# keio-bioinformatics/stem_kernel

Measured on AMD Instinct MI355X. Metric: sequence-pairs/sec (Gram entries/s) at L=200 nt, higher is better.
Workload: dtype f64

## Files before the change

include/stem_kernel.h:

```cpp
#ifndef STEM_KERNEL_H
#define STEM_KERNEL_H

#include <stddef.h>
#include <stdint.h>

#ifdef __cplusplus
extern "C" {
#endif

#define SK_ABI_VERSION 2

typedef enum {
  SK_OK = 0,
  SK_ERR_INVALID = -1,
  SK_ERR_HIP = -2,
  SK_ERR_NO_DEVICE = -3,
  SK_ERR_ALLOC = -4,
  SK_ERR_RANGE = -5,
  SK_ERR_UNSUPPORTED = -6
} sk_status;

typedef enum {
  SK_SU_STEM = 0,
  SK_SI_STEM = 1,
  SK_SU_STR = 2,
  SK_SI_STR = 3,
  SK_SU_STEM_STR = 4,
  SK_SI_STEM_STR = 5,
  SK_LSU_STEM = 6,
  SK_LSU_STEM_STR = 7,
  SK_NAIVE_STR = 8,
  SK_BPLA = 9,
  SK_LA = 10,
  SK_BPLA_SW = 11,
  SK_LA_SW = 12,
  SK_STEM4D = 13
} sk_kernel_kind;

typedef struct {
  int32_t kind;
  uint32_t len_band;
  double beta;
  double loop_gap;
  double stack;
  double covar;
  double alpha;
  double gap;
  double match;
  double mismatch;
  double ext;
  double score_table[16];
  double subst;
  double bp_bound;
  int32_t bp_model;
  uint32_t loop;
  double ali_bound;
  int32_t ali_zerop_fixed;
} sk_kernel_params;

void sk_kernel_params_default(sk_kernel_params *p, int32_t kind);

typedef struct sk_context sk_context;

int sk_open(int device, void *hip_stream, sk_context **ctx);
int sk_close(sk_context *ctx);
const char *sk_strerror(int status);
const char *sk_last_error(const sk_context *ctx);

typedef struct sk_dataset sk_dataset;

int sk_dataset_create(sk_dataset **ds);
int sk_dataset_free(sk_dataset *ds);

int sk_dataset_add(sk_dataset *ds, const char *label, int n_rows,
                   const char *const *rows, const double *const *bpp_rows,
                   float th, int use_bp);
int sk_dataset_add_synthetic(sk_dataset *ds, int32_t n, const char *const *seqs,
                             const char *const *labels, float th, int32_t n_threads);
int sk_dataset_add_synthetic_rows(sk_dataset *ds, int32_t n, int32_t n_rows,
                                  const char *const *rows, const char *const *labels,
                                  float th, int32_t n_threads);
int sk_dataset_add_copy(sk_dataset *dst, const sk_dataset *src, int32_t i);
int sk_dataset_size(const sk_dataset *ds);
int sk_dataset_export(const sk_dataset *ds, int32_t first, int32_t count, uint8_t *buf,
                      size_t cap, size_t *size);
int sk_dataset_import(sk_dataset *ds, const uint8_t *buf, size_t size);
int sk_dataset_pack_digest(sk_dataset *ds, uint64_t *y_hash, uint64_t *x_hash);
const char *sk_dataset_label(const sk_dataset *ds, int i);
int sk_dataset_shape(const sk_dataset *ds, int i, int32_t *n_nodes,
                     int32_t *n_edges, int32_t *n_bpfreq, int32_t *n_roots,
                     int32_t *seq_len);
int sk_dataset_row_traffic(const sk_dataset *ds, int i, int32_t *rows, int32_t *stored,
                           int32_t *slab_reads, int32_t *gamma_reads, int32_t *phi_reads,
                           int32_t *reg_reads, int32_t *y_slots);
int sk_dataset_dag(const sk_dataset *ds, int i, uint32_t *first, uint32_t *last,
                   uint32_t *n_edges, uint32_t *n_bpfreq, float *weight,
                   uint32_t *max_pa, uint32_t *edge_to, uint32_t *edge_gaps,
                   uint32_t *bp_code, float *bp_p, uint32_t *roots,
                   float *pos_weight);

int sk_dataset_profile(const sk_dataset *ds, int i, float *prof5, float *n_seqs);

int sk_dataset_bpla_weights(const sk_dataset *ds, int i, float *p_left,
                            float *p_right, float *p_unpair);

int sk_dataset_upload(sk_context *ctx, sk_dataset *ds);

int sk_gram(sk_context *ctx, sk_dataset *ds, const sk_kernel_params *kp,
            int normalize, double *out);

int sk_pairs_device(sk_context *ctx, sk_dataset *ds, const sk_kernel_params *kp,
                    const int32_t *x, const int32_t *y, int64_t n_pairs,
                    double *out_dev);
int sk_pairs(sk_context *ctx, sk_dataset *ds, const sk_kernel_params *kp,
             const int32_t *x, const int32_t *y, int64_t n_pairs, double *out);

int sk_test_row(sk_context *ctx, sk_dataset *test, int t, sk_dataset *train,
                const int32_t *sv_index, int32_t n_sv,
                const sk_kernel_params *kp, double *out, double *self);

int sk_diagonal(sk_context *ctx, sk_dataset *ds, const int32_t *sv_index,
                int32_t n_sv, const sk_kernel_params *kp, double *out);

int sk_test_matrix(sk_context *ctx, sk_dataset *test, sk_dataset *train,
                   const sk_kernel_params *kp, int norm_test, int normalize,
                   double *out, double *self_out);

int64_t sk_shard_count(int32_t n, int32_t rank, int32_t world);
int sk_shard_cells(int32_t n, int32_t rank, int32_t world, int32_t *x, int32_t *y);
int sk_shard_assemble(int32_t n, int32_t world, const double *gathered, int64_t per_rank,
                      int normalize, double *out);
int sk_comm_unique_id(uint8_t *id, size_t id_bytes);
int sk_comm_init(sk_context *ctx, const uint8_t *id, size_t id_bytes, int32_t rank, int32_t world);
int sk_comm_allgather(sk_context *ctx, const double *send_dev, int64_t count, double *recv_dev);
int sk_gram_sharded(sk_context *ctx, sk_dataset *ds, const sk_kernel_params *kp, int normalize,
                    double *out);

int sk_format_libsvm(const double *matrix, int32_t rows, int32_t cols,
                     const char *const *labels, char *buf, size_t buf_size,
                     size_t *needed);

int sk_fold_synthetic(const char *seq, int32_t n, int32_t no_gu, double *out);

#define SK_FOLD_NO_GU 1
#define SK_FOLD_NO_CLOSING_GU 2
#define SK_FOLD_NO_LONELY_PAIRS 4
int sk_fold_mccaskill(sk_context *ctx, int32_t n, const char *const *seqs, int32_t flags,
                      double *out, double *log_z);
int sk_fold_sample(sk_context *ctx, int32_t n, const char *const *seqs, int32_t flags,
                   int32_t n_samples, uint64_t seed, double *out_bpp, char *out_structs,
                   double *log_z);
double sk_fold_sample_uniform(uint64_t seed, int32_t seq, int32_t sample, int32_t draw);
int sk_fold_alignment(sk_context *ctx, int32_t n_aln, const int32_t *n_rows,
                      const char *const *rows, int32_t flags, double *out, double *log_z);
int sk_dataset_add_consensus(sk_dataset *ds, const char *label, int n_rows,
                             const char *const *rows, const double *bpp, float th);
int sk_dataset_add_alifolded(sk_context *ctx, sk_dataset *ds, int32_t n, int32_t n_rows,
                             const char *const *rows, const char *const *labels, float th,
                             int32_t fold_flags, int32_t n_threads);
int sk_dataset_add_batch(sk_dataset *ds, int32_t n, int32_t n_rows, const char *const *rows,
                         const double *const *bpp_rows, const char *const *labels, float th,
                         int32_t use_bp, int32_t n_threads);
int sk_dataset_add_folded(sk_context *ctx, sk_dataset *ds, int32_t n, int32_t n_rows,
                          const char *const *rows, const char *const *labels, float th,
                          int32_t fold_flags, int32_t n_threads);
int sk_dataset_add_sampled(sk_context *ctx, sk_dataset *ds, int32_t n, int32_t n_rows,
                           const char *const *rows, const char *const *labels, float th,
                           int32_t fold_flags, int32_t n_samples, uint64_t seed, int32_t n_threads);

int sk_bpla_gradients(sk_context *ctx, sk_dataset *xs, sk_dataset *ys, const sk_kernel_params *kp,
                      const int32_t *x, const int32_t *y, int64_t n_pairs, double *value,
                      double *grad);

typedef enum { SK_FMT_FASTA = 0, SK_FMT_CLUSTAL = 1, SK_FMT_MAF = 2 } sk_file_format;
typedef struct sk_seqfile sk_seqfile;
int sk_seqfile_read(const char *path, int32_t format, sk_seqfile **out);
int sk_seqfile_parse(const char *text, size_t len, int32_t format, sk_seqfile **out);
int sk_seqfile_free(sk_seqfile *f);
int64_t sk_seqfile_count(const sk_seqfile *f);
int32_t sk_seqfile_rows(const sk_seqfile *f, int64_t i);
const char *sk_seqfile_row(const sk_seqfile *f, int64_t i, int32_t r);
const char *sk_seqfile_last_error(void);
int sk_random_sequences(uint64_t *state, int32_t n_seqs, int32_t len, char *out);

typedef struct sk_svm_model sk_svm_model;
int sk_svm_model_load(const char *path, sk_svm_model **out);
void sk_svm_model_free(sk_svm_model *m);
int sk_svm_model_info(const sk_svm_model *m, int32_t *svm_type, int32_t *nr_class, int32_t *labels,
                      int32_t *has_probability);
int sk_svm_predict(const sk_svm_model *m, int32_t cnt, const double *row, int32_t n, int32_t probability,
                   double *label, double *values);
const char *sk_svm_last_error(void);

int sk_last_timing(const sk_context *ctx, double *stem_ms, double *string_ms,
                   double *cells, int32_t *launches);
int sk_last_launch_ms(const sk_context *ctx, double *ms_sum, int32_t *n_launches);
int sk_set_async(sk_context *ctx, int32_t on);
int sk_sync_timing(sk_context *ctx);
int sk_last_classes(const sk_context *ctx, uint32_t *stem_maxk_mask, uint32_t *stem4d_mask);
int sk_stem4d_col_shape(int32_t min_len, int32_t max_len, int32_t *nb, int32_t *waves, int32_t *pf);
void sk_ribosum_tables(float *s16, float *p256);
int sk_char2rna(int c);
int sk_experiments(void);

#ifdef __cplusplus
}
#endif
#endif
```

stem_kernel_amd/_lib.py:

```python
from __future__ import annotations

import ctypes as C
import os
import threading

_HERE = os.path.dirname(os.path.abspath(__file__))
LIB_PATH = os.environ.get("SK_LIB_PATH") or os.path.join(_HERE, "libstem_kernel_amd.so")

SK_OK = 0
STATUS = {
    0: "ok", -1: "invalid argument", -2: "HIP runtime error", -3: "no usable gfx950 device",
    -4: "allocation failed", -5: "index out of range", -6: "unsupported",
}

FMT_FASTA, FMT_CLUSTAL, FMT_MAF = range(3)
(SU_STEM, SI_STEM, SU_STR, SI_STR, SU_STEM_STR, SI_STEM_STR, LSU_STEM, LSU_STEM_STR, NAIVE_STR,
 BPLA, LA, BPLA_SW, LA_SW, STEM4D) = range(14)


class KernelParams(C.Structure):
    _fields_ = [
        ("kind", C.c_int32), ("len_band", C.c_uint32), ("beta", C.c_double),
        ("loop_gap", C.c_double), ("stack", C.c_double), ("covar", C.c_double),
        ("alpha", C.c_double), ("gap", C.c_double), ("match", C.c_double),
        ("mismatch", C.c_double), ("ext", C.c_double), ("score_table", C.c_double * 16),
        ("subst", C.c_double), ("bp_bound", C.c_double), ("bp_model", C.c_int32),
        ("loop", C.c_uint32), ("ali_bound", C.c_double), ("ali_zerop_fixed", C.c_int32),
    ]


_P = C.c_void_p
_I32P = C.POINTER(C.c_int32)
_U32P = C.POINTER(C.c_uint32)
_F32P = C.POINTER(C.c_float)
_F64P = C.POINTER(C.c_double)

SIGNATURES = {
    "sk_kernel_params_default": (None, [C.POINTER(KernelParams), C.c_int32]),
    "sk_open": (C.c_int, [C.c_int, _P, C.POINTER(_P)]),
    "sk_close": (C.c_int, [_P]),
    "sk_strerror": (C.c_char_p, [C.c_int]),
    "sk_last_error": (C.c_char_p, [_P]),
    "sk_dataset_create": (C.c_int, [C.POINTER(_P)]),
    "sk_dataset_free": (C.c_int, [_P]),
    "sk_dataset_add": (C.c_int, [_P, C.c_char_p, C.c_int, C.POINTER(C.c_char_p),
                                 C.POINTER(_F64P), C.c_float, C.c_int]),
    "sk_dataset_add_synthetic": (C.c_int, [_P, C.c_int32, C.POINTER(C.c_char_p),
                                           C.POINTER(C.c_char_p), C.c_float, C.c_int32]),
    "sk_dataset_add_synthetic_rows": (C.c_int, [_P, C.c_int32, C.c_int32, C.POINTER(C.c_char_p),
                                                C.POINTER(C.c_char_p), C.c_float, C.c_int32]),
    "sk_dataset_size": (C.c_int, [_P]),
    "sk_dataset_add_copy": (C.c_int, [_P, _P, C.c_int32]),
    "sk_dataset_export": (C.c_int, [_P, C.c_int32, C.c_int32, C.c_void_p, C.c_size_t,
                                    C.POINTER(C.c_size_t)]),
    "sk_dataset_import": (C.c_int, [_P, C.c_void_p, C.c_size_t]),
    "sk_dataset_pack_digest": (C.c_int, [_P, C.POINTER(C.c_uint64), C.POINTER(C.c_uint64)]),
    "sk_dataset_label": (C.c_char_p, [_P, C.c_int]),
    "sk_dataset_shape": (C.c_int, [_P, C.c_int, _I32P, _I32P, _I32P, _I32P, _I32P]),
    "sk_dataset_row_traffic": (C.c_int, [_P, C.c_int, _I32P, _I32P, _I32P, _I32P, _I32P, _I32P, _I32P]),
    "sk_dataset_dag": (C.c_int, [_P, C.c_int, _U32P, _U32P, _U32P, _U32P, _F32P, _U32P,
                                 _U32P, _U32P, _U32P, _F32P, _U32P, _F32P]),
    "sk_dataset_profile": (C.c_int, [_P, C.c_int, _F32P, _F32P]),
    "sk_dataset_bpla_weights": (C.c_int, [_P, C.c_int, _F32P, _F32P, _F32P]),
    "sk_dataset_upload": (C.c_int, [_P, _P]),
    "sk_gram": (C.c_int, [_P, _P, C.POINTER(KernelParams), C.c_int, _F64P]),
    "sk_pairs_device": (C.c_int, [_P, _P, C.POINTER(KernelParams), _I32P, _I32P, C.c_int64,
                                  C.c_void_p]),
    "sk_pairs": (C.c_int, [_P, _P, C.POINTER(KernelParams), _I32P, _I32P, C.c_int64, _F64P]),
    "sk_test_row": (C.c_int, [_P, _P, C.c_int, _P, _I32P, C.c_int32, C.POINTER(KernelParams),
                              _F64P, _F64P]),
    "sk_diagonal": (C.c_int, [_P, _P, _I32P, C.c_int32, C.POINTER(KernelParams), _F64P]),
    "sk_test_matrix": (C.c_int, [_P, _P, _P, C.POINTER(KernelParams), C.c_int, C.c_int, _F64P,
                                 _F64P]),
    "sk_format_libsvm": (C.c_int, [_F64P, C.c_int32, C.c_int32, C.POINTER(C.c_char_p),
                                   C.c_char_p, C.c_size_t, C.POINTER(C.c_size_t)]),
    "sk_fold_synthetic": (C.c_int, [C.c_char_p, C.c_int32, C.c_int32, _F64P]),
    "sk_fold_mccaskill": (C.c_int, [_P, C.c_int32, C.POINTER(C.c_char_p), C.c_int32, _F64P, _F64P]),
    "sk_fold_sample": (C.c_int, [_P, C.c_int32, C.POINTER(C.c_char_p), C.c_int32, C.c_int32, C.c_uint64,
                                 _F64P, C.c_void_p, _F64P]),
    "sk_fold_sample_uniform": (C.c_double, [C.c_uint64, C.c_int32, C.c_int32, C.c_int32]),
    "sk_fold_alignment": (C.c_int, [_P, C.c_int32, _I32P, C.POINTER(C.c_char_p), C.c_int32, _F64P, _F64P]),
    "sk_dataset_add_consensus": (C.c_int, [_P, C.c_char_p, C.c_int, C.POINTER(C.c_char_p), _F64P, C.c_float]),
    "sk_dataset_add_alifolded": (C.c_int, [_P, _P, C.c_int32, C.c_int32, C.POINTER(C.c_char_p),
                                           C.POINTER(C.c_char_p), C.c_float, C.c_int32, C.c_int32]),
    "sk_dataset_add_sampled": (C.c_int, [_P, _P, C.c_int32, C.c_int32, C.POINTER(C.c_char_p),
                                         C.POINTER(C.c_char_p), C.c_float, C.c_int32, C.c_int32,
                                         C.c_uint64, C.c_int32]),
    "sk_dataset_add_batch": (C.c_int, [_P, C.c_int32, C.c_int32, C.POINTER(C.c_char_p),
                                       C.POINTER(_F64P), C.POINTER(C.c_char_p), C.c_float,
                                       C.c_int32, C.c_int32]),
    "sk_dataset_add_folded": (C.c_int, [_P, _P, C.c_int32, C.c_int32, C.POINTER(C.c_char_p),
                                        C.POINTER(C.c_char_p), C.c_float, C.c_int32, C.c_int32]),
    "sk_random_sequences": (C.c_int, [C.POINTER(C.c_uint64), C.c_int32, C.c_int32, C.c_char_p]),
    "sk_last_timing": (C.c_int, [_P, _F64P, _F64P, _F64P, _I32P]),
    "sk_last_launch_ms": (C.c_int, [_P, _F64P, _I32P]),
    "sk_set_async": (C.c_int, [_P, C.c_int32]),
    "sk_sync_timing": (C.c_int, [_P]),
    "sk_shard_count": (C.c_int64, [C.c_int32, C.c_int32, C.c_int32]),
    "sk_shard_cells": (C.c_int, [C.c_int32, C.c_int32, C.c_int32, _I32P, _I32P]),
    "sk_shard_assemble": (C.c_int, [C.c_int32, C.c_int32, _F64P, C.c_int64, C.c_int, _F64P]),
    "sk_comm_unique_id": (C.c_int, [C.c_char_p, C.c_size_t]),
    "sk_comm_init": (C.c_int, [_P, C.c_char_p, C.c_size_t, C.c_int32, C.c_int32]),
    "sk_comm_allgather": (C.c_int, [_P, C.c_void_p, C.c_int64, C.c_void_p]),
    "sk_gram_sharded": (C.c_int, [_P, _P, C.POINTER(KernelParams), C.c_int, _F64P]),
    "sk_last_classes": (C.c_int, [_P, C.POINTER(C.c_uint32), C.POINTER(C.c_uint32)]),
    "sk_stem4d_col_shape": (C.c_int, [C.c_int32, C.c_int32, _I32P, _I32P, _I32P]),
    "sk_ribosum_tables": (None, [_F32P, _F32P]),
    "sk_char2rna": (C.c_int, [C.c_int]),
    "sk_experiments": (C.c_int, []),
    "sk_bpla_gradients": (C.c_int, [_P, _P, _P, C.POINTER(KernelParams), _I32P, _I32P, C.c_int64,
                                    _F64P, _F64P]),
    "sk_seqfile_read": (C.c_int, [C.c_char_p, C.c_int32, C.POINTER(_P)]),
    "sk_seqfile_parse": (C.c_int, [C.c_char_p, C.c_size_t, C.c_int32, C.POINTER(_P)]),
    "sk_seqfile_free": (C.c_int, [_P]),
    "sk_seqfile_count": (C.c_int64, [_P]),
    "sk_seqfile_rows": (C.c_int32, [_P, C.c_int64]),
    "sk_seqfile_row": (C.c_char_p, [_P, C.c_int64, C.c_int32]),
    "sk_seqfile_last_error": (C.c_char_p, []),
    "sk_svm_model_load": (C.c_int, [C.c_char_p, C.POINTER(_P)]),
    "sk_svm_model_free": (None, [_P]),
    "sk_svm_model_info": (C.c_int, [_P, C.POINTER(C.c_int32), C.POINTER(C.c_int32), C.POINTER(C.c_int32),
                                    C.POINTER(C.c_int32)]),
    "sk_svm_predict": (C.c_int, [_P, C.c_int32, C.POINTER(C.c_double), C.c_int32, C.c_int32,
                                 C.POINTER(C.c_double), C.POINTER(C.c_double)]),
    "sk_svm_last_error": (C.c_char_p, []),
}

_lock = threading.Lock()
_lib = None


class StemKernelError(RuntimeError):

    def __init__(self, code, msg=""):
        super().__init__(f"{STATUS.get(code, code)}{': ' + msg if msg else ''}")
        self.code = code


def lib():
    global _lib
    with _lock:
        if _lib is not None:
            return _lib
        if not os.path.exists(LIB_PATH):
            raise StemKernelError(-3, f"{LIB_PATH} not built; run `make` or __graft_entry__.build()")
        try:
            import torch
        except Exception:
            pass
        L = C.CDLL(LIB_PATH)
        for name, (res, args) in SIGNATURES.items():
            f = getattr(L, name)
            f.restype = res
            f.argtypes = args
        _lib = L
        return L


def check(rc, ctx=None):
    if rc != SK_OK:
        msg = ""
        if ctx:
            m = lib().sk_last_error(ctx)
            msg = m.decode() if m else ""
        raise StemKernelError(rc, msg)
    return rc


def default_params(kind=SU_STEM_STR, **over):
    p = KernelParams()
    lib().sk_kernel_params_default(C.byref(p), kind)
    for k, v in over.items():
        if k == "score_table":
            for i, t in enumerate(v):
                p.score_table[i] = float(t)
        else:
            setattr(p, k, v)
    return p
```

stem_kernel_amd/csrc/kernels/dag_stem.hip:

```cpp
#include <hip/hip_runtime.h>

#include <algorithm>

#include "device_set.h"
#include "launch.h"

namespace sk {

__global__ void sk_prep_kernel(DevSet s, DevParamNodes pn, const double* __restrict__ gpow,
                               double gap2) {
  const int e = blockIdx.x * blockDim.x + threadIdx.x;
  if (e >= s.n_examples) return;
  const int nl = s.ex_nl[e];
  const int nb = s.ex_node_base[e], eb = s.ex_edge_base[e];
  for (int k = 0; k < nl; ++k) {
    const uint32_t a = s.nd_a[nb + k];
    const int e0 = a & 0xffff, ne = (a >> 16) & 0xff;
    const double v_s = gap2 * (double)s.nd_w[nb + k];
    double L = 0.0, SL = 0.0;
    if (ne == 0) {
      L += 1.0 * v_s * gpow[s.nd_c[nb + k]];
    } else {
      for (int t = 0; t < ne; ++t) {
        const uint32_t ed = s.ed[eb + e0 + t].x;
// ... 437 lines not shown
          const bool two = na > h + 1;
          const uint32_t c0 = c[h], c1 = two ? c[h + 1] : c[h];
          const double eg0 = w[h], eg1 = two ? w[h + 1] : 0.0;
          add_rows2<MAXK>(S, row_rsrc(child_row(c0, slab, gamtab, phitab, stride), NLy),
                          row_rsrc(child_row(c1, slab, gamtab, phitab, stride), NLy), eg0, eg1, lane);
        }
      }
    }
#ifdef SK_STAMPS
    {
      int nl_ = 0;
      for (int j = 0; j < 4; ++j) nl_ += (j < xne && !(done >> j & 1u)) ? 1 : 0;
      cnt[0] += nl_ + (xne > 4 ? xne - 4 : 0);
    }
#endif
    for (int t = 4; t < xne; t += 2) {
      const uint32_t c0 = xch[chp_r + t];
      const bool two = t + 1 < xne;
      const uint32_t c1 = two ? xch[chp_r + t + 1] : c0;
      const double eg0 = xchw[chp_r + t], eg1 = two ? xchw[chp_r + t + 1] : 0.0;
      add_rows2<MAXK>(S, row_rsrc(child_row(c0, slab, gamtab, phitab, stride), NLy),
                      row_rsrc(child_row(c1, slab, gamtab, phitab, stride), NLy), eg0, eg1, lane);
    }
    STAMP(1);

    if (!combo) {
#pragma unroll
      for (int k = 0; k < MAXK; ++k) R[lane + 64 * k] = lane + 64 * k < qb ? S[k] : 0.0;
    }
    double rowk = 0.0;
    STAMP(2);
#ifdef SK_STAMPS
    cnt[3] += qb > qa ? qb - qa : 0;
#endif
    if (!combo && qa < qb) {
      constexpr int NW = 64 * PW;
      int top = qb - 1, q0 = max(top - NW + 1, qa);
      uint4 nd_n[PW];
      double Pq_n[PW];
#pragma unroll
      for (int j = 0; j < PW; ++j) {
        nd_n[j] = nd_first[j];
        Pq_n[j] = Pq_first[j];
      }
      for (;;) {
        uint4 nd[PW];
        double Pq[PW];
#pragma unroll
        for (int j = 0; j < PW; ++j) {
          nd[j] = nd_n[j];
          Pq[j] = Pq_n[j];
        }
        const int ntop = top - NW, nq0 = max(ntop - NW + 1, qa);
        if (ntop >= qa) {
#pragma unroll
          for (int j = 0; j < PW; ++j) {
            nd_n[j] = Y.nrg[min(nq0 + 64 * j + lane, ntop)];
            Pq_n[j] = yPg[min(nq0 + 64 * j + lane, ntop)];
          }
        }
        double co_v[PW], gl_v[PW];
#pragma unroll
        for (int j = 0; j < PW; ++j) {
          co_v[j] = co[xcode + ((nd[j].y >> 16) & 0xf)];
          gl_v[j] = gp[nd[j].y & 0xffff];
        }
        double Hq[PW];
#pragma unroll
        for (int j = 0; j < PW; ++j) Hq[j] = 0.0;
        if (!xloop) {
          const int ea = __builtin_amdgcn_readfirstlane(nd[0].x & 0xffff);
          const int jt = (top - q0) >> 6;
          uint32_t ndt = nd[0].x;
#pragma unroll
          for (int j = 1; j < PW; ++j) ndt = jt == j ? nd[j].x : ndt;
          const uint32_t at = __builtin_amdgcn_readlane(ndt, (top - q0) & 63);
          const int eb = (int)((at & 0xffff) + ((at >> 16) & 0xff));
          constexpr bool EG = edges_global<MAXK>();
          uint32_t en[SK_MU];
          if constexpr (EG) {
#pragma unroll
            for (int u = 0; u < SK_MU; ++u) en[u] = Y.ed2g[min(ea + 64 * u + lane, eb - 1)];
          }
          for (int f0 = ea; f0 < eb; f0 += 64 * SK_MU) {
            uint32_t e[SK_MU];
            if constexpr (EG) {
#pragma unroll
              for (int u = 0; u < SK_MU; ++u) {
                e[u] = en[u];
                en[u] = Y.ed2g[min(f0 + 64 * (SK_MU + u) + lane, eb - 1)];
              }
            } else {
#pragma unroll
              for (int u = 0; u < SK_MU; ++u) e[u] = Y.ed2[min(f0 + 64 * u + lane, eb - 1)];
            }
            double g[SK_MU], rv[SK_MU];
#pragma unroll
            for (int u = 0; u < SK_MU; ++u) {
              g[u] = gp[e[u] >> 22];
              rv[u] = R[e[u] & 0x7ff];
            }
#pragma unroll
            for (int u = 0; u < SK_MU; ++u) {
              const bool ok = f0 + 64 * u + lane < eb;
              const double w = g[u] * rv[u] * (ok ? 1.0 : 0.0);
              const int h = ok ? (int)((e[u] >> 11) & 0x7ff) - q0 : lane;
              if constexpr (SK_SEGSUM && MAXK <= SK_SEGSUM_MAXK) {
                const int key = ok ? h : -1 - lane;
                const int ql = lane & 3;
                double sw = w;
                {
                  const int ks = __builtin_amdgcn_mov_dpp(key, 0x90, 0xf, 0xf, false);
                  const double ws = __hiloint2double(
                      __builtin_amdgcn_mov_dpp(__double2hiint(sw), 0x90, 0xf, 0xf, false),
                      __builtin_amdgcn_mov_dpp(__double2loint(sw), 0x90, 0xf, 0xf, false));
                  sw += (ql >= 1 && ks == key) ? ws : 0.0;
                }
                {
                  const int ks = __builtin_amdgcn_mov_dpp(key, 0x40, 0xf, 0xf, false);
                  const double ws = __hiloint2double(
                      __builtin_amdgcn_mov_dpp(__double2hiint(sw), 0x40, 0xf, 0xf, false),
                      __builtin_amdgcn_mov_dpp(__double2loint(sw), 0x40, 0xf, 0xf, false));
                  sw += (ql >= 2 && ks == key) ? ws : 0.0;
                }
                const int kn = __builtin_amdgcn_mov_dpp(key, 0xF9, 0xf, 0xf, false);
                if (ok && (ql == 3 || kn != key))
                  __hip_atomic_fetch_add(&hb[h], sw, __ATOMIC_RELAXED, __HIP_MEMORY_SCOPE_WAVEFRONT);
              } else {
                __hip_atomic_fetch_add(&hb[h], w, __ATOMIC_RELAXED, __HIP_MEMORY_SCOPE_WAVEFRONT);
              }
            }
          }
#pragma unroll
          for (int j = 0; j < PW; ++j) {
            Hq[j] = hb[64 * j + lane];
            hb[64 * j + lane] = 0.0;
          }
        }
#pragma unroll
        for (int j = 0; j < PW; ++j) {
          const int q = q0 + 64 * j + lane;
          const bool on = q <= top;
          const uint32_t nda = nd[j].x, ndc = nd[j].y;
          double H = Hq[j];
          if (((nda >> 16) & 0xff) == 0)
            H = (xloop ? xeg0 : xSL) * gl_v[j];
          double vs;
          if (x_one && (ndc >> 24) != 0u) {
            vs = co_v[j] * xpf * (double)__uint_as_float(nd[j].w);
          } else {
            const int qq = on ? q : top;
            vs = H != 0.0 ? match_node_score(co, s, xbb, xb0, xnbf, ys, Y, ys.yn_b[Y.nb + qq] >> 16,
                                             nda >> 24, xwg, gap2 * (double)__uint_as_float(nd[j].z),
                                             x_nbp, (double)ys.yn_nbp[Y.nb + qq], x_nseq)
                          : 0.0;
          }
          const double M = vs * H;
          if (on) {
            R[q] = M;
            rowk += M * Pq[j];
          }
        }
#ifdef SK_STAMPS
        cnt[2] += 1;
#endif
        if (ntop < qa) break;
        top = ntop;
        q0 = nq0;
      }
    }
    STAMP(3);
#pragma unroll
    for (int k = 0; k < MAXK; ++k) {
      const int q = lane + 64 * k;
      if (!combo && 64 * k < qa && q < qa) R[q] = 0.0;
    }
    kacc += xP * rowk;
    wave_sync();
    STAMP(4);

    constexpr int NPF = MAXK == 17 ? SK_NPF17
                        : (MAXK == 16 && (SK_NPF16 == 0 || SK_M16 == 2)) ? 0
                        : ((MAXK <= 12 && SK_NPF12 == 2) || (MAXK == 16 && SK_NPF16 == 2) ||
                           (MAXK == 20 && SK_W20 == 8 && SK_NPF20 == 2)) ? 2 : 1;
    uint32_t nxt_done = 0;
    double egd = 0.0, egt0 = 0.0, egt1 = 0.0;
    double T0[MAXK], T1[MAXK];
#pragma unroll
    for (int k = 0; k < MAXK; ++k) T0[k] = T1[k] = 0.0;
    if (r + 1 < nlx) {
      const int nne = nx.a & 0xff;
      uint32_t pf0 = 0, pf1 = 0;
      int npf = 0;
#pragma unroll
      for (int j = 0; j < 4; ++j) {
        if (j < nne) {
          const uint32_t c = nch[j];
          const double g = ncw[j];
          if ((c & 0xffff) == pslot) {
            egd += g;
            nxt_done |= 1u << j;
          } else if (npf < NPF) {
            if (npf == 0) {
              pf0 = c;
              egt0 = g;
            } else {
              pf1 = c;
              egt1 = g;
            }
            ++npf;
            nxt_done |= 1u << j;
          }
        }
      }
      if (NPF >= 1 && npf >= 1) {
        const __amdgpu_buffer_rsrc_t r0 = row_rsrc(child_row(pf0, slab, gamtab, phitab, stride), NLy);
#pragma unroll
        for (int k = 0; k < MAXK; ++k) T0[k] = row_ld(r0, lane, k);
      }
      if (NPF >= 2 && npf >= 2) {
        const __amdgpu_buffer_rsrc_t r1 = row_rsrc(child_row(pf1, slab, gamtab, phitab, stride), NLy);
#pragma unroll
        for (int k = 0; k < MAXK; ++k) T1[k] = row_ld(r1, lane, k);
      }
    }

    int c0 = 0;
    if (band > 0) c0 = Y.ycs[min(max(xlen - band, 0), Y.lmax + 1)];
    c0 = __builtin_amdgcn_readfirstlane(c0);
#ifdef SK_STAMPS
    cnt[1] += Y.nch - c0;
#endif
    if (!combo && c0 < Y.nch && pslot != 0xffffu) {
      iy_sweep<node_weights<MAXK>(), node_weights_f32<MAXK>()>(Y, R, c0, lane);
      wave_sync();
    }
    STAMP(5);

    constexpr int HD = (MAXK > SK_HALF_D || (m16_wide<MAXK>() && SK_M16_HALFD)) ? (MAXK + 1) / 2 : MAXK;
    if (pslot == 0xffffu) {
#pragma unroll
      for (int k = 0; k < MAXK; ++k) S[k] = egt0 * T0[k] + (NPF >= 2 ? egt1 * T1[k] : 0.0);
    } else if (pslot == 0xfffeu) {
      const double cw = combo ? 1.0 : xwg;
#pragma unroll
      for (int h0 = 0; h0 < MAXK; h0 += HD) {
        double g1[HD];
#pragma unroll
        for (int k = 0; k < HD; ++k) g1[k] = combo ? 0.0 : R[lane + 64 * (h0 + k)];
        SCHED_FENCE();
#pragma unroll
        for (int k = 0; k < HD; ++k)
          S[h0 + k] = egd * (g1[k] + cw * S[h0 + k]) + egt0 * T0[h0 + k] + (NPF >= 2 ? egt1 * T1[h0 + k] : 0.0);
      }
    } else {
#ifdef SK_FULL_STORE
      double* __restrict__ orow = slab + (size_t)pslot * stride + lane;
#else
      const __amdgpu_buffer_rsrc_t orsrc = row_rsrc(slab + (size_t)pslot * stride, NLy);
#endif
      const double cw = combo ? 1.0 : xwg;
#pragma unroll
      for (int h0 = 0; h0 < MAXK; h0 += HD) {
        double g1[HD];
#pragma unroll
        for (int k = 0; k < HD; ++k) g1[k] = combo ? 0.0 : R[lane + 64 * (h0 + k)];
        SCHED_FENCE();
#pragma unroll
        for (int k = 0; k < HD; ++k) {
          const double o = g1[k] + cw * S[h0 + k];
#ifndef SK_XNOSTORE
#ifdef SK_FULL_STORE
          orow[64 * (h0 + k)] = o;
#else
          __builtin_amdgcn_raw_buffer_store_b64(__builtin_bit_cast(u32x2, o), orsrc, lane * 8,
                                                (h0 + k) * 512, SK_ROW_ST_POL);
#endif
#endif
          S[h0 + k] = egd * o + egt0 * T0[h0 + k] + (NPF >= 2 ? egt1 * T1[h0 + k] : 0.0);
        }
      }
    }
    done = nxt_done;
    wave_sync();
    STAMP(6);
  }
#ifdef SK_STAMPS
  if (lane == 0 && P.stamps) {
    for (int i = 0; i < 8; ++i) atomicAdd(&P.stamps[i], tacc[i]);
    atomicAdd(&P.stamps[8], (unsigned long long)nlx);
    atomicAdd(&P.stamps[9], 1ull);
    for (int i = 0; i < 4; ++i) atomicAdd(&P.stamps[10 + i], cnt[i]);
  }
#endif
  for (int off = 32; off > 0; off >>= 1) kacc += __shfl_xor(kacc, off, 64);
  return kacc;
}

template <int MAXK>
struct StemWaves {
  static constexpr int value = MAXK <= 12 ? 12 : MAXK <= 17 ? (SK_M16 ? 12 : SK_W16) : MAXK <= 20 ? SK_W20 : 8;
};

template <int MAXK>
__global__ void __launch_bounds__(64 * StemWaves<MAXK>::value) sk_dag_stem_kernel(StemLaunch P) {
  extern __shared__ __attribute__((aligned(16))) unsigned char smem[];
  const DevSet& s = P.yset;
  const int lane = threadIdx.x & 63, wave = threadIdx.x >> 6;
  const int nwaves = blockDim.x >> 6;
  const int maxnl = P.lds_max_nl;
  constexpr int PW = pass_width<MAXK>();

  lds_f64* co = (lds_f64*)(smem);
  lds_f64* gp = co + 256;
  lds_f64* Rall = gp + P.n_gpow_pad;
  lds_f64* hball = Rall + (size_t)nwaves * maxnl;
  constexpr bool NW = node_weights<MAXK>();
  lds_f64* yew = hball + (size_t)nwaves * 64 * PW;
  lds_u32* ysc = (lds_u32*)(yew + (node_weights_f32<MAXK>() ? (size_t)maxnl / 2
                                   : NW ? (size_t)maxnl : (size_t)P.lds_max_nch * 64));
  lds_u32* yed2 = ysc + (size_t)P.lds_max_nch * 64;
  lds_i32* ylf = (lds_i32*)(yed2 + (edges_global<MAXK>() ? 0 : P.lds_max_edges));
  lds_i32* ycs = ylf + P.lds_max_len_pad;
  lds_i32* ctl = ycs + P.lds_max_len_pad;
  lds_f64* kap = (lds_f64*)(ctl + 4);

  for (int k = threadIdx.x; k < 256; k += blockDim.x) co[k] = P.co_subst[k];
  for (int k = threadIdx.x; k < P.n_gpow; k += blockDim.x) gp[k] = P.gpow[k];

  lds_f64* R = Rall + (size_t)wave * maxnl;
  lds_f64* hb = hball + (size_t)wave * 64 * PW;
  for (int j = 0; j < PW; ++j) hb[64 * j + lane] = 0.0;
  double* slab = P.scratch + (size_t)(blockIdx.x * nwaves + wave) * P.slab_doubles;
  double* gamtab = P.gam_on ? P.gam + (size_t)blockIdx.x * P.gam_doubles : nullptr;
  double* phitab = P.phi_on ? P.phi + (size_t)blockIdx.x * P.phi_doubles : nullptr;
  double* phikap = P.phi_on ? phitab + (size_t)P.xset.n_phi * (64 * MAXK) : nullptr;
  const double gap2 = P.gap2;
  const int band = (int)P.band;

  const int wave_u = __builtin_amdgcn_readfirstlane(wave);
  for (;;) {
    __syncthreads();
    if (threadIdx.x == 0) ctl[0] = atomicAdd(P.item_counter, 1);
    __syncthreads();
    const int it = __builtin_amdgcn_readfirstlane(ctl[0]);
    if (it >= P.n_items) break;
    const int4 item = P.items[it];
    const int y = item.x;
    YView Y;
    Y.nl = s.ex_nl[y];
    Y.nch = s.ex_nch[y];
    Y.nseqs = s.ex_nseqs[y];
    const int nb = s.ex_node_base[y], eb = s.ex_edge_base[y], bb = s.ex_bpf_base[y];
    Y.lmax = Y.nl ? (int)(s.yn_b[nb + Y.nl - 1] & 0xffff) : 0;
    {
      const int ne = s.ex_edge_base[y + 1] - eb;
      const int sb = s.ex_ysc_base[y] * 64, nrec = Y.nch * 64;
      const int nfree = max(maxnl - Y.nl, 1);
      for (int k = threadIdx.x; k < nrec + 128; k += blockDim.x) {
        uint32_t r = k < nrec ? s.ysc[sb + k] : 0u;
        const uint32_t ch = r & 0x7ff, pa = (r >> 11) & 0x7ff;
        const uint32_t zs = (uint32_t)(maxnl - 1 - (k & 63) % nfree);
        if (k >= nrec || ch == pa) r = zs | (zs << 11);
        ysc[k] = r;
        if (!NW) yew[k] = (k >= nrec || ch == pa) ? 0.0 : gap2 * (double)s.yn_w[nb + pa] * gp[r >> 22];
      }
      if (node_weights_f32<MAXK>())
        for (int q = threadIdx.x; q < maxnl; q += blockDim.x) ((lds_f32*)yew)[q] = q < Y.nl ? s.yn_w[nb + q] : 0.0f;
      else if (NW)
        for (int q = threadIdx.x; q < maxnl; q += blockDim.x) yew[q] = q < Y.nl ? gap2 * (double)s.yn_w[nb + q] : 0.0;
      if (!edges_global<MAXK>())
        for (int k = threadIdx.x; k < ne; k += blockDim.x) yed2[k] = s.ye2[eb + k];
      const int cb = s.ex_ycs_base[y];
      for (int v = threadIdx.x; v <= Y.lmax + 1; v += blockDim.x) ycs[v] = s.ycs[cb + v];
    }
    Y.nrg = s.yrec + nb;
    Y.sc = ysc; Y.ew = yew; Y.ed2 = yed2; Y.lfirst = ylf; Y.ycs = ycs; Y.gp = gp;
    Y.ewf = (const lds_f32*)yew; Y.gap2 = gap2;
    Y.ed2g = s.ye2 + eb;
    Y.nb = nb; Y.bb = bb;
    __syncthreads();
    for (int v = threadIdx.x; v <= Y.lmax + 1; v += blockDim.x) {
      int lo = 0, hi = Y.nl;
      while (lo < hi) {
        const int mid = (lo + hi) >> 1;
        if ((int)(s.yn_b[nb + mid] & 0xffff) < v) lo = mid + 1; else hi = mid;
      }
      ylf[v] = lo;
    }
    __syncthreads();

    const bool gam = P.gam_on && s.ex_gapless[y];
    if (gam) {
      const DevSet& xset = P.xset;
      for (int g = wave_u; g < xset.n_gam; g += nwaves) {
        const uint32_t key = xset.gam_key[g];
        const int gcode = (int)(key >> 16) * 16, glen = (int)(key & 0xffff);
        double kp = 0.0;
        for (int k = 0; k < MAXK; ++k) {
          const int q = lane + 64 * k;
          double M = 0.0;
          if (q < Y.nl) {
            const uint4 nd = Y.nrg[q];
            const int ylen = (int)(s.yn_b[nb + q] & 0xffff);
            if (((nd.x >> 16) & 0xff) == 0 && (band == 0 || abs(glen - ylen) <= band)) {
              double vs;
              if ((nd.y >> 24) != 0u) {
                vs = co[gcode + ((nd.y >> 16) & 0xf)] * (double)__uint_as_float(nd.w);
              } else {
                vs = 0.0;
                const int yb0 = (int)(s.yn_b[nb + q] >> 16), ynb = (int)(nd.x >> 24);
                for (int b = 0; b < ynb; ++b)
                  vs += co[gcode + s.bpf_code[bb + yb0 + b]] * (double)s.bpf_p[bb + yb0 + b];
              }
              M = vs * gp[nd.y & 0xffff];
              kp += M * s.yn_P[nb + q];
            }
          }
          R[q] = M;
        }
        for (int off = 32; off > 0; off >>= 1) kp += __shfl_xor(kp, off, 64);
        if (lane == 0) kap[g] = kp;
        wave_sync();
        int c0 = 0;
        if (band > 0) c0 = Y.ycs[min(max(glen - band, 0), Y.lmax + 1)];
        c0 = __builtin_amdgcn_readfirstlane(c0);
        if (c0 < Y.nch) iy_sweep<node_weights<MAXK>(), node_weights_f32<MAXK>()>(Y, R, c0, lane);
        double* grow = gamtab + (size_t)g * (64 * MAXK);
        for (int k = 0; k < MAXK; ++k)
          if (lane + 64 * k < Y.nl) grow[lane + 64 * k] = R[lane + 64 * k];
        wave_sync();
      }
      __syncthreads();

      if (P.phi_on) {
        const DevSet& xset = P.xset;
        const int pb = P.item_phi_off[it], pe = P.item_phi_off[it + 1];
        const int share = (pe - pb + nwaves - 1) / nwaves;
        const int t0 = pb + wave_u * share, t1 = min(pe, t0 + share);
        int gcur = -1;
        double Hr[MAXK];
#pragma unroll
        for (int k = 0; k < MAXK; ++k) Hr[k] = 0.0;
        for (int t = t0; t < t1; ++t) {
          const int idx = __builtin_amdgcn_readfirstlane(P.item_phi[t]);
          const int g = __builtin_amdgcn_readfirstlane((int)xset.phi_g[idx]);
          if (g != gcur) {
            gcur = g;
            const double* __restrict__ grow = gamtab + (size_t)g * (64 * MAXK);
#pragma unroll
            for (int k = 0; k < MAXK; ++k) R[lane + 64 * k] = grow[lane + 64 * k];
            wave_sync();
            for (int k = 0; k < MAXK; ++k) {
              const int q = lane + 64 * k;
              double H = 0.0;
              if (q < Y.nl) {
                const uint32_t na = Y.nrg[q].x;
                const int ne = (int)((na >> 16) & 0xff), e0 = (int)(na & 0xffff);
                for (int e = 0; e < ne; ++e) {
                  const uint32_t rec = edges_global<MAXK>() ? Y.ed2g[e0 + e] : Y.ed2[e0 + e];
                  H += gp[rec >> 22] * R[rec & 0x7ff];
                }
              }
              Hr[k] = H;
            }
            wave_sync();
          }
          const uint32_t al = xset.phi_al[idx];
          const int acode = (int)(al >> 16) * 16, alen = (int)(al & 0xffff);
          double kp = 0.0;
#pragma unroll
          for (int k = 0; k < MAXK; ++k) {
            const int q = lane + 64 * k;
            double M = 0.0;
            if (q < Y.nl) {
              const uint4 nd = Y.nrg[q];
              const int ylen = (int)(s.yn_b[nb + q] & 0xffff);
              if (Hr[k] != 0.0 && (band == 0 || abs(alen - ylen) <= band)) {
                double vs;
                if ((nd.y >> 24) != 0u) {
                  vs = co[acode + ((nd.y >> 16) & 0xf)] * (double)__uint_as_float(nd.w);
                } else {
                  vs = 0.0;
                  const int yb0 = (int)(s.yn_b[nb + q] >> 16), ynb = (int)(nd.x >> 24);
                  for (int b = 0; b < ynb; ++b)
                    vs += co[acode + s.bpf_code[bb + yb0 + b]] * (double)s.bpf_p[bb + yb0 + b];
                }
                M = vs * Hr[k];
                kp += M * s.yn_P[nb + q];
              }
            }
            R[q] = M;
          }
          for (int off = 32; off > 0; off >>= 1) kp += __shfl_xor(kp, off, 64);
          if (lane == 0) phikap[idx] = kp;
          wave_sync();
          int c0 = 0;
          if (band > 0) c0 = Y.ycs[min(max(alen - band, 0), Y.lmax + 1)];
          c0 = __builtin_amdgcn_readfirstlane(c0);
          if (c0 < Y.nch) iy_sweep<node_weights<MAXK>(), node_weights_f32<MAXK>()>(Y, R, c0, lane);
          double* prow = phitab + (size_t)idx * (64 * MAXK);
#pragma unroll
          for (int k = 0; k < MAXK; ++k)
            if (lane + 64 * k < Y.nl) prow[lane + 64 * k] = R[lane + 64 * k];
          wave_sync();
        }
        __syncthreads();
      }
    }

    if (threadIdx.x == 0) ctl[1] = nwaves;
    __syncthreads();
    for (int t = wave_u; t < item.z;) {
      const int x = P.xs[item.y + t];
      const double k = stem_pair<MAXK>(P, Y, R, hb, co, gp, slab, x, lane, gam, gamtab, kap, phitab, phikap);
      if (lane == 0) P.out[P.oidx[item.y + t]] = k;
      int nt = 0;
      if (lane == 0) nt = atomicAdd(reinterpret_cast<int*>(const_cast<int32_t*>((const int32_t*)ctl)) + 1, 1);
      t = __builtin_amdgcn_readlane(nt, 0);
    }
  }
}

hipError_t launch_prep(const DevSet& s, const DevParamNodes& pn, const double* gpow, double gap2,
                       hipStream_t st) {
  const int bs = 64;
  const int grid = (s.n_examples + bs - 1) / bs;
  if (grid == 0) return hipSuccess;
  hipLaunchKernelGGL(sk_prep_kernel, dim3(grid), dim3(bs), 0, st, s, pn, gpow, gap2);
  return hipGetLastError();
}

size_t stem_lds_bytes(const StemLaunch& P, int nwaves) {
  size_t b = 0;
  b += 256 * 8;
  b += (size_t)P.n_gpow_pad * 8;
  b += (size_t)nwaves * P.lds_max_nl * 8;
  b += (size_t)nwaves * 64 * pass_width_of(stem_maxk(P.lds_max_nl)) * 8;
  const int maxk = stem_maxk(P.lds_max_nl);
  if (node_weights_of(maxk))
    b += (size_t)P.lds_max_nch * 64 * 4 + (size_t)P.lds_max_nl * (maxk >= SK_NODEF_MIN ? 4 : 8);
  else
    b += (size_t)P.lds_max_nch * 64 * 12;
  if (stem_maxk(P.lds_max_nl) < SK_EDG_MIN) b += (size_t)P.lds_max_edges * 4;
  b += (size_t)P.lds_max_len_pad * 4 * 2 + 16;
  if (P.gam_on) b += (size_t)P.xset.n_gam * 8;
  return b;
}

#define SK_STEM_CLASSES(X) X(4) X(8) X(12) X(16) X(17) X(20) X(24) X(28) X(32)

static const void* stem_kernel_ptr(int maxk) {
  switch (maxk) {
#define SK_CASE(K) \
  case K: return reinterpret_cast<const void*>(sk_dag_stem_kernel<K>);
    SK_STEM_CLASSES(SK_CASE)
#undef SK_CASE
    default: return nullptr;
  }
}

int stem_maxk(int max_nl) {
  const int s = (std::max(max_nl, 1) + 63) / 64;
  if (SK_K17 && s == 17) return 17;
  const int k = (s + 3) & ~3;
  return k <= 32 ? k : -1;
}

hipError_t launch_stem(const StemLaunch& P, int grid, int nwaves, hipStream_t st) {
  const size_t lds = stem_lds_bytes(P, nwaves);
  const int maxk = stem_maxk(P.lds_max_nl);
  const void* fn = stem_kernel_ptr(maxk);
  if (!fn) return hipErrorInvalidValue;
  hipError_t e = hipFuncSetAttribute(fn, hipFuncAttributeMaxDynamicSharedMemorySize, (int)lds);
  if (e != hipSuccess) return e;
  switch (maxk) {
#define SK_CASE(K)                                                                          \
  case K:                                                                                  \
    hipLaunchKernelGGL(sk_dag_stem_kernel<K>, dim3(grid), dim3(64 * nwaves), lds, st, P); \
    break;
    SK_STEM_CLASSES(SK_CASE)
#undef SK_CASE
    default: return hipErrorInvalidValue;
  }
  return hipGetLastError();
}

hipError_t stem_kernel_attr(int max_nl, int* max_dyn_lds, int* vgprs, int* max_waves) {
  hipFuncAttributes attr;
  const int maxk = stem_maxk(max_nl);
  if (maxk < 0) return hipErrorInvalidValue;
  hipError_t e = hipFuncGetAttributes(&attr, stem_kernel_ptr(maxk));
  if (e != hipSuccess) return e;
  *max_dyn_lds = 163840 - (int)attr.sharedSizeBytes;
  *vgprs = attr.numRegs;
  *max_waves = std::max(1, attr.maxThreadsPerBlock / 64);
  return hipSuccess;
}

}
```

stem_kernel_amd/csrc/kernels/launch.h:

```cpp
#pragma once
#include <hip/hip_runtime.h>

#include <cstddef>
#include <cstdint>

#include "device_set.h"
#include "tri_index.h"

namespace sk {

struct StemLaunch {
  DevSet xset;
  DevSet yset;
  DevParamNodes pn;
  const double* co_subst = nullptr;
  const double* gpow = nullptr;
  int32_t n_gpow = 0, n_gpow_pad = 0;
  double gap2 = 0.0;
  uint32_t band = 0;
  int32_t lds_max_nl = 0, lds_max_edges = 0, lds_max_bpf = 0, lds_max_nch = 0;
  int32_t lds_max_len_pad = 0;
  const int4* items = nullptr;
  int32_t n_items = 0;
  const int32_t* xs = nullptr;
  const int64_t* oidx = nullptr;
  double* out = nullptr;
  int* item_counter = nullptr;
  double* scratch = nullptr;
  int64_t slab_doubles = 0;
  double* gam = nullptr;
  int64_t gam_doubles = 0;
  int32_t gam_on = 0;
  double* phi = nullptr;
  int64_t phi_doubles = 0;
  const int32_t* item_phi_off = nullptr;
  const int32_t* item_phi = nullptr;
  int32_t phi_on = 0;
  unsigned long long* stamps = nullptr;
};

struct StemBigLaunch {
  DevSet xset, yset;
  DevParamNodes pn;
  const double* co_subst = nullptr;
  const double* gpow = nullptr;
  int32_t n_gpow = 0;
  double gap2 = 0.0;
  uint32_t band = 0;
  const int32_t* xs = nullptr;
  const int32_t* ys = nullptr;
  const int64_t* oidx = nullptr;
  int64_t n_pairs = 0;
  double* out = nullptr;
  double* scratch = nullptr;
  int64_t stride = 0;
  int64_t wave_doubles = 0;
};
hipError_t launch_stem_big(const StemBigLaunch& P, int grid, hipStream_t st);
constexpr int kStemBigWaves = 4;

struct StrLaunch {
  DevSet xset, yset;
  const double* st = nullptr;
  const double* gpow = nullptr;
  double gap = 0.0;
  int32_t naive = 0;
  const int32_t* xs = nullptr;
  const int32_t* ys = nullptr;
  int64_t n_pairs = 0;
  double* out = nullptr;
  const int64_t* oidx = nullptr;
  unsigned long long* pair_counter = nullptr;
  int32_t lds_max_len = 0;
};

struct StrPos {
  double v[4];
};
struct StrCode {
  float w;
  int32_t code;
};
struct StrFastLaunch {
  DevSet xset, yset;
  const StrPos* xtab = nullptr;
  const StrPos* ytab = nullptr;
  const double* st = nullptr;
  int32_t onehot = 0;
  const double* gpow = nullptr;
  double gap = 0.0;
  const int32_t* xs = nullptr;
  const int32_t* ys = nullptr;
  const int64_t* oidx = nullptr;
  int64_t n_pairs = 0;
  double* out = nullptr;
  unsigned long long* pair_counter = nullptr;
  int32_t lds_max_len = 0;
};
__host__ __device__ inline size_t str_fast_wave_lds_bytes(int maxlen, bool onehot) {
  return ((size_t)maxlen * (onehot ? sizeof(StrCode) : sizeof(StrPos)) + (size_t)2 * (maxlen + 2) * 8 + 15) &
         ~(size_t)15;
}
constexpr size_t kStrFastLds0 = 16 * 8;
hipError_t launch_str_tab(const float4* prof, const float* pos_w, int64_t n, const double* st, StrPos* xrole,
                          StrPos* yrole, hipStream_t stream);
hipError_t launch_str_code_tab(const float4* prof, const float* pos_w, int64_t n, StrCode* tab,
                               hipStream_t stream);
hipError_t launch_str_fast(const StrFastLaunch& P, int grid, int nwaves, hipStream_t stream);

struct alignas(16) BplaPos {
  double v[4];
  float pr, pl, pu, dyadic;
};
static_assert(sizeof(BplaPos) == 48, "BplaPos is three 16-B loads");

struct BplaLaunch {
  DevSet xset, yset;
  const BplaPos* xtab = nullptr;
  const BplaPos* ytab = nullptr;
  const int64_t* oidx = nullptr;
  const int2* items = nullptr;
  int32_t n_items = 0;
  const double* table = nullptr;
  double alpha = 0.0, beta = 0.0, gap = 0.0, ext = 0.0;
  double beta_gap = 0.0, beta_ext = 0.0;
  int32_t sw = 0;
  int32_t bp = 0;
  const int32_t* xs = nullptr;
  const int32_t* ys = nullptr;
  int64_t n_pairs = 0;
  double* out = nullptr;
  unsigned long long* pair_counter = nullptr;
  int32_t lds_max_len = 0;
  int32_t chunk = 1;
};

struct BplaGradLaunch {
  DevSet xset, yset;
  const double* table = nullptr;
  double alpha = 0.0, beta = 0.0, gap = 0.0, ext = 0.0;
  double beta_gap = 0.0, beta_ext = 0.0;
  const int32_t* xs = nullptr;
  const int32_t* ys = nullptr;
  int64_t n_pairs = 0;
  int32_t n1 = 1, m1 = 1;
  double* scratch = nullptr;
  double* value = nullptr;
  double* grad = nullptr;
  const BplaPos* xtab = nullptr;
  const BplaPos* ytab = nullptr;
  unsigned long long* pair_counter = nullptr;
  const int64_t* oidx = nullptr;
  int32_t lds_max_len = 0;
  int64_t bt_doubles = 0;
};
size_t bpla_grad_pair_bytes(int n1, int m1);
hipError_t launch_bpla_grad(const BplaGradLaunch& P, hipStream_t st);
__host__ __device__ inline int bpla_steps(int lx, int ly) {
  const int lys = ly > 64 ? ly : 64;
  return lx <= 0 || ly <= 0 ? 0 : ((lx + 63) / 64 - 1) * lys + ((lx - 1) & 63) + ly;
}
__host__ __device__ inline size_t bpla_grad_wave_lds_bytes(int maxlen) {
  const size_t b = (size_t)maxlen * sizeof(BplaPos) + (size_t)3 * (maxlen + 2) * 8;
  return (b + 15) & ~(size_t)15;
}
hipError_t launch_bpla_grad_wave(const BplaGradLaunch& P, int grid, int nwaves, hipStream_t st);

__host__ __device__ inline size_t bpla_wave_lds_bytes(int maxlen) {
  const size_t b = (size_t)4 * (maxlen + 2) * 8 + (size_t)maxlen * 32;
  return (b + 15) & ~(size_t)15;
}

struct Stem4dPair {
  int32_t n = 0, m = 0;
  int64_t plane_doubles = 0;
  int64_t scratch_off = 0;
  int64_t x_bp = 0, y_bp = 0;
  int64_t x_chr = 0, y_chr = 0;
  int64_t out_index = 0;
  int64_t band_off = 0;
};

struct Stem4dLaunch {
  const Stem4dPair* pairs = nullptr;
  const int2* items = nullptr;
  int64_t n_items = 0;
  int32_t d1 = 0;
  double* scratch = nullptr;
  const float* bpdiag = nullptr;
  const uint8_t* chars = nullptr;
  const float* bpdiag_y = nullptr;
  const uint8_t* chars_y = nullptr;
  const double* gpow = nullptr;
  double gap = 0.0, stack = 0.0, subst = 0.0;
  float bp_bound = 0.0f;
  double* out = nullptr;
  const int32_t* band_lo = nullptr;
  const int32_t* band_hi = nullptr;
  double* kbound = nullptr;
  int64_t kbound_stride = 0;
  int32_t gsum = 0;
  int32_t col_f = 1;
};

int stem4d_cpl(int m);
hipError_t launch_stem4d(const Stem4dLaunch& P, int cpl, hipStream_t st);
int stem4d_col_w_max(int m);
int stem4d_col_max_n();
int stem4d_col_pf();
int stem4d_col_nb(int cpl);
size_t stem4d_col_lds_bytes(int cpl, int waves, int max_m, int max_n);
int stem4d_col_max_waves(int cpl);
hipError_t launch_stem4d_col(const Stem4dLaunch& P, int64_t n_pairs, int cpl, int waves, int max_m,
                             int max_n, hipStream_t st);

struct PhmmLaunch {
  const Stem4dPair* pairs = nullptr;
  int64_t n_pairs = 0;
  const uint8_t* chars = nullptr;
  const uint8_t* chars_y = nullptr;
  char* scratch = nullptr;
  size_t pair_bytes = 0;
  int32_t n1 = 1, m1 = 1;
  float ali_bound = 0.0f;
  uint32_t band = 0;
  int32_t zerop_fixed = 0;
  int32_t* band_lo = nullptr;
  int32_t* band_hi = nullptr;
};
size_t phmm_pair_bytes(int n1, int m1);
hipError_t launch_phmm(const PhmmLaunch& P, hipStream_t st);

struct FoldSeq {
  int64_t seq_off = 0;
  int64_t work_off = 0;
  int64_t out_off = 0;
  int64_t lp_off = 0;
  int32_t n = 0, n_rows = 1;
};
struct FoldLaunch {
  const FoldSeq* seqs = nullptr;
  const int8_t* codes = nullptr;
  const double* tab = nullptr;
  int32_t o_st = 0, o_hp = 0, o_bu = 0, o_in = 0, o_ni = 0, o_au = 0, o_ml = 0, o_scp = 0;
  double log_sc = 0.0;
  int32_t no_gu = 0, no_closing_gu = 0;
  const uint8_t* lp = nullptr;
  int32_t n_tab = 0, n_tab_pad = 0;
  int32_t n_small = 0;
  int32_t max_n = 0;
  double* work = nullptr;
  double* out = nullptr;
  double* log_z = nullptr;
  int32_t inside_only = 0;
  int32_t o_ali = 0;
  int32_t min_path = 0;
};

constexpr int kFoldTables = 6, kFoldAliTables = 10;
struct FoldWork {
  double* base;
  size_t n;
  int tables;
  __host__ __device__ static size_t doubles(int tables, size_t n) { return (size_t)tables * n * n + 2 * (n + 1); }
  __host__ __device__ double& at(int k, int d, int i) const { return (base + (size_t)k * n * n)[(size_t)d * n + i]; }
  __host__ __device__ double& qb(int d, int i) const { return at(0, d, i); }
  __host__ __device__ double& qm(int d, int i) const { return at(1, d, i); }
  __host__ __device__ double& qm1(int d, int i) const { return at(2, d, i); }
  __host__ __device__ double& hb(int d, int i) const { return at(3, d, i); }
  __host__ __device__ double& hm(int d, int i) const { return at(4, d, i); }
  __host__ __device__ double& hm1(int d, int i) const { return at(5, d, i); }
  __host__ __device__ double& cell(int k, int d, int i) const { return at(kFoldTables + k, d, i); }
  __host__ __device__ double* q5() const { return base + (size_t)tables * n * n; }
  __host__ __device__ double* h5() const { return q5() + n + 1; }
};
inline size_t fold_work_doubles(size_t n) { return FoldWork::doubles(kFoldTables, n); }
inline size_t fold_ali_work_doubles(size_t n) { return FoldWork::doubles(kFoldAliTables, n); }

constexpr int kFoldRingMaxN = 248;
constexpr size_t kFoldLdsMax = 163840 - 256;
enum FoldPath : int32_t { kFoldPathRing = 0, kFoldPathHbm = 1, kFoldPathGtab = 2 };
bool fold_ring(const FoldLaunch& P, int max_n);
bool fold_gtab(const FoldLaunch& P, int max_n);
inline const char* fold_path_name(FoldPath p) {
  return p == kFoldPathRing ? "ring" : p == kFoldPathHbm ? "hbm" : "gtab";
}
FoldPath fold_path(const FoldLaunch& P, int max_n);
size_t fold_lds_bytes(const FoldLaunch& P, int max_n);
hipError_t launch_fold(const FoldLaunch& P, int n_seqs, int max_n, hipStream_t st);

struct FoldSampleLaunch {
  FoldLaunch F;
  uint32_t* cnt = nullptr;
  char* structs = nullptr;
  int32_t* status = nullptr;
  int32_t n_samples = 0;
  int32_t seq_base = 0;
  uint64_t seed = 0;
};
constexpr int32_t kFoldSampleRunaway = 1;
constexpr int32_t kFoldSampleNoWeight = 2;
constexpr int32_t kFoldSampleStack = 3;
size_t fold_sample_lds_bytes(const FoldLaunch& P, int max_n);
hipError_t launch_fold_sample(const FoldSampleLaunch& P, int n_seqs, int max_n, hipStream_t st);

FoldPath fold_ali_path(const FoldLaunch& P, int max_n);
size_t fold_ali_lds_bytes(const FoldLaunch& P, int max_n);
hipError_t launch_fold_ali(const FoldLaunch& P, int n_alns, int max_n, hipStream_t st);

enum CombineMode : int32_t {
  kCombineStem = 0,
  kCombineStr = 1,
  kCombineAdd = 2,
  kCombineLogStem = 3,
  kCombineLogAdd = 4
};

hipError_t launch_prep(const DevSet& s, const DevParamNodes& pn, const double* gpow, double gap2,
                       hipStream_t st);
size_t stem_lds_bytes(const StemLaunch& P, int nwaves);
hipError_t launch_stem(const StemLaunch& P, int grid, int nwaves, hipStream_t st);
hipError_t stem_kernel_attr(int max_nl, int* max_dyn_lds, int* vgprs, int* max_waves);
int stem_maxk(int max_nl);

size_t str_lds_bytes(const StrLaunch& P, int nwaves);
hipError_t launch_str(const StrLaunch& P, int grid, int nwaves, hipStream_t st);

constexpr size_t kBplaExpLds = 1024 * 8;
constexpr int kBplaChunkMax = 16;
#ifndef SK_BPLA_ITEMS_WAVES
#define SK_BPLA_ITEMS_WAVES 12
#endif
constexpr int kBplaItemsWavesMax = SK_BPLA_ITEMS_WAVES;
constexpr size_t kBplaChunkLds = kBplaChunkMax * (16 + 8);
__host__ __device__ inline size_t bpla_items_lds_bytes(int maxlen, int nwaves) {
  return kBplaExpLds + 16 + (size_t)maxlen * sizeof(BplaPos) +
         (size_t)nwaves * (3 * (maxlen + 2) * 8 + kBplaChunkLds);
}
size_t bpla_lds_bytes(const BplaLaunch& P, int nwaves);
hipError_t launch_bpla(const BplaLaunch& P, int grid, int nwaves, hipStream_t st);
hipError_t launch_bpla_tab(const float4* prof, const float4* lru, int64_t n, const double* table,
                           double xscale, BplaPos* xrole, BplaPos* yrole, hipStream_t st);
__host__ __device__ inline size_t bpla_fast_wave_lds_bytes(int maxlen) {
  const size_t b = (size_t)maxlen * sizeof(BplaPos) + (size_t)3 * (maxlen + 2) * 8 + kBplaChunkLds;
  return (b + 15) & ~(size_t)15;
}
hipError_t launch_bpla_fast(const BplaLaunch& P, int grid, int nwaves, hipStream_t st);

hipError_t launch_combine(const double* stem, const double* str, double* out, int64_t n,
                          int32_t mode, double alpha, double beta, hipStream_t st);

}
```

stem_kernel_amd/csrc/sk_api.cpp:

```cpp
#include <hip/hip_runtime.h>

#include <algorithm>
#include <chrono>
#include <cmath>
#include <cstdio>
#include <cstring>
#include <cstdlib>
#include <functional>
#include <memory>
#include <mutex>
#include <new>
#include <numeric>
#include <queue>
#include <sstream>
#include <thread>
#include <type_traits>
#include <atomic>
#include <string>
#include <system_error>
#include <vector>

#include "../../include/stem_kernel.h"
#include "host/fold_host.h"
#include "kernels/fold_ali_model.h"
#include "kernels/fold_rng.h"
#include "host/sk_internal.h"
#include "kernels/device_set.h"
#include "kernels/launch.h"
#include "ribosum85_60.inc"

using sk::DevSet;
using sk::Example;

namespace {

struct DeviceBuffers {
  std::vector<void*> ptrs;
  size_t bytes = 0;
  ~DeviceBuffers() { release(); }
  void release() {
    for (void* p : ptrs) (void)hipFree(p);
    ptrs.clear();
  }
};

template <class V, class T = typename V::value_type>
hipError_t upload(DeviceBuffers& db, const V& v, const T** out) {
  void* p = nullptr;
  const size_t bytes = std::max<size_t>(v.size() * sizeof(T), 16);
  hipError_t e = hipMalloc(&p, bytes);
  if (e != hipSuccess) return e;
  db.ptrs.push_back(p);
  db.bytes += bytes;
  if (!v.empty()) e = hipMemcpy(p, v.data(), v.size() * sizeof(T), hipMemcpyHostToDevice);
  *out = static_cast<const T*>(p);
  return e;
}

float4 bpla_weight(const Example& X, int i) {
  if (!X.has_bp) return make_float4(0.f, 0.f, 1.f, 0.f);
  float pl = 0.0f, pr = 0.0f;
  for (int j = 0; j < i; ++j) pr = (float)((double)pr + X.bpp[sk::tri_index(X.len, j, i)]);
  for (int j = i + 1; j < X.len; ++j) pl = (float)((double)pl + X.bpp[sk::tri_index(X.len, i, j)]);
  float pu = (float)(1.0 - (double)(pl + pr));
  if (pu < 0.0f) pu = 0.0f;
  return make_float4(std::sqrt(pl), std::sqrt(pr), std::sqrt(pu), 0.f);
}

void bpla_weights(const Example& X, std::vector<float4>& out) {
  const int L = X.len;
  const size_t base = out.size();
  out.resize(base + (size_t)std::max(L, 0));
  if (!X.has_bp) {
    for (int i = 0; i < L; ++i) out[base + i] = make_float4(0.f, 0.f, 1.f, 0.f);
    return;
  }
  std::vector<float> pr((size_t)L, 0.0f);
  for (int i = 0; i < L; ++i) {
    float pl = 0.0f;
    if (i + 1 < L) {
      const double* row = X.bpp.data() + sk::tri_index(L, i, i + 1);
      for (int j = i + 1; j < L; ++j) {
        const double b = row[j - i - 1];
        pl = (float)((double)pl + b);
        pr[j] = (float)((double)pr[j] + b);
      }
    }
    float pu = (float)(1.0 - (double)(pl + pr[i]));
    if (pu < 0.0f) pu = 0.0f;
    out[base + i] = make_float4(std::sqrt(pl), std::sqrt(pr[i]), std::sqrt(pu), 0.f);
  }
}

template <class T>
struct NoInitAlloc : std::allocator<T> {
  template <class U>
  struct rebind {
    using other = NoInitAlloc<U>;
  };
  NoInitAlloc() = default;
  template <class U>
  NoInitAlloc(const NoInitAlloc<U>&) noexcept {}
  template <class U>
  void construct(U* p) noexcept {
    ::new ((void*)p) U;
  }
  template <class U, class... A>
  void construct(U* p, A&&... a) {
    ::new ((void*)p) U(std::forward<A>(a)...);
  }
};
template <class T>
using pvec = std::vector<T, NoInitAlloc<T>>;

struct HostPack {
  std::vector<int32_t> ex_nl, ex_node_base, ex_edge_base, ex_bpf_base, ex_lvl_base, ex_nlev,
      ex_len, ex_pos_base, ex_has_w;
  std::vector<uint8_t> ex_dyadic;
  std::vector<uint8_t> ex_str_fast, ex_onehot;
  std::vector<uint8_t> ex_big;
  std::vector<float> ex_nseqs;
  pvec<uint32_t> nd_a, nd_b, nd_c;
  pvec<float> nd_w, nd_nbp;
  pvec<double> nd_P;
  pvec<uint2> ed;
  pvec<uint32_t> bpf_code;
  pvec<float> bpf_p;
  pvec<int32_t> lvl;
  pvec<float4> pos_prof;
  pvec<float> pos_w;
  pvec<uint8_t> pos_chr;
  pvec<float4> pos_lru;
  std::vector<int32_t> ex_nslots, ex_xch_base;
  pvec<sk::XRow> xrow;
  pvec<uint32_t> yn_a, yn_b, yn_c, ye2, ysc;
  pvec<uint4> yrec;
  pvec<float> yn_w, yn_nbp, yn_p0;
  pvec<double> yn_P;
  pvec<int32_t> ycs;
  std::vector<int32_t> ex_ysc_base, ex_nch, ex_ycs_base;
  pvec<uint32_t> xr_node, xr_ch;
  pvec<sk::XRow> xgrow;
  std::vector<uint32_t> gam_key;
  pvec<uint32_t> xg_node, xg_ch, xg_clg, gr_info;
  pvec<float> xg_cpf, gr_pf;
  pvec<double> gr_P;
  std::vector<int32_t> ex_xg_base, ex_nlxg, ex_xgch_base, ex_gr_base, ex_gapless;
  pvec<uint8_t> xg_cty;
  std::vector<uint32_t> phi_al, phi_g;
  pvec<uint32_t> gra_gidx, gra_row, phk_idx;
  std::vector<int32_t> ex_gra_base, ex_phk_base;
  pvec<uint64_t> ex_phi_bits;
  int32_t max_nl = 0, max_edges = 0, max_bpf = 0, max_nlev = 0, max_len = 0, max_slots = 0;
  int32_t max_nch = 0;
};
#define SK_PACK_Y_ARRAYS(X) X(yn_a) X(yn_b) X(yn_c) X(ye2) X(ysc) X(yrec) X(yn_w) X(yn_nbp) X(yn_p0) X(yn_P) \
  X(ycs) X(ex_ysc_base) X(ex_nch) X(ex_ycs_base)
#define SK_PACK_X_ARRAYS(X) X(nd_a) X(nd_b) X(nd_c) X(nd_w) X(nd_nbp) X(nd_P) X(ed) X(bpf_code) X(bpf_p)     \
  X(lvl) X(xr_ch) X(xrow) X(xr_node) X(gr_info) X(gr_pf) X(gr_P) X(xg_ch) X(xg_clg) X(xg_cpf) X(xg_cty)     \
  X(phk_idx) X(gra_gidx) X(gra_row) X(xgrow) X(xg_node) X(pos_prof) X(pos_w) X(pos_chr) X(pos_lru)          \
  X(ex_phi_bits) X(ex_nl) X(ex_node_base) X(ex_edge_base) X(ex_bpf_base) X(ex_lvl_base) X(ex_nlev) X(ex_len) \
  X(ex_pos_base) X(ex_has_w) X(ex_dyadic) X(ex_str_fast) X(ex_onehot) X(ex_big) X(ex_nseqs) X(ex_nslots)    \
  X(ex_xch_base) X(gam_key) X(ex_xg_base) X(ex_nlxg) X(ex_xgch_base) X(ex_gr_base) X(ex_gapless) X(phi_al)   \
  X(phi_g) X(ex_gra_base) X(ex_phk_base)

}

struct Stem4dTables {
  Stem4dTables() = default;
  Stem4dTables(const Stem4dTables&) = delete;
  Stem4dTables& operator=(const Stem4dTables&) = delete;
  ~Stem4dTables() {
    if (device < 0 || buf.ptrs.empty()) return;
    int cur = -1;
    if (hipGetDevice(&cur) != hipSuccess) cur = -1;
    if (hipSetDevice(device) == hipSuccess) (void)hipDeviceSynchronize();
    buf.release();
    if (cur >= 0) (void)hipSetDevice(cur);
  }
  DeviceBuffers buf;
  int device = -1, model = -1;
  unsigned loop = 0;
  size_t n_ex = 0;
  const float* bp = nullptr;
  const uint8_t* ch = nullptr;
  std::vector<int64_t> bp_off, ch_off;
  std::vector<uint8_t> why, acgu;
};

struct sk_dataset {
  std::vector<Example> ex;
  std::vector<std::string> labels;
  int device = -1;
  bool uploaded = false;
  DevSet dev;
  DeviceBuffers buf;
  HostPack pack;
  std::string err;
  double* prep = nullptr;
  double prep_loop_gap = -1.0;
  std::mutex s4_mu;
  std::vector<std::shared_ptr<Stem4dTables>> s4;
};
constexpr size_t kS4Sets = 4;

struct Stem4dBatch {
  sk::Stem4dPair* pairs = nullptr;
  int2* items = nullptr;
  int32_t* band = nullptr;
  size_t cap_pairs = 0, cap_items = 0, cap_band = 0;
};

struct sk_context {
  Stem4dBatch s4d;
  int device = 0;
  hipStream_t stream = nullptr;
  bool own_stream = false;
  int n_cu = 0;
  std::string err;
  double* scratch = nullptr;
  size_t scratch_bytes = 0;
  void* work = nullptr;
  size_t work_bytes = 0;
  hipEvent_t ev0 = nullptr, ev1 = nullptr, ev2 = nullptr, ev3 = nullptr;
  hipStream_t side = nullptr;
  hipEvent_t evf = nullptr, evj = nullptr;
  hipStream_t cls = nullptr;
  hipEvent_t evk = nullptr, evx = nullptr;
  hipStream_t aux = nullptr;
  hipEvent_t eva = nullptr;
  struct TSet {
    hipEvent_t ev[4] = {nullptr, nullptr, nullptr, nullptr};
    std::vector<hipEvent_t> lev;
    size_t lev_used = 0;
    bool pending = false, stem = false, str = false;
    double cells = 0.0;
    int32_t launches = 0;
  };
  static constexpr int kTSets = 4;
  TSet tset[kTSets];
  int tk = 0;
  bool async = false;
  double acc_stem_ms = 0.0, acc_str_ms = 0.0, acc_cells = 0.0, acc_launch_ms = 0.0;
  int32_t acc_launch_n = 0, acc_launches = 0;
  struct Stage {
    std::vector<std::pair<char*, size_t>> blocks;
    size_t blk = 0, off = 0;
    hipEvent_t ev = nullptr;
    bool recorded = false;
    char* dbuf = nullptr;
    size_t dcap = 0;
    hipEvent_t uev = nullptr;
  };
  Stage stage[2];
  hipStream_t cps = nullptr;
  uint64_t ncalls = 0;
  double last_launch_ms_sum = 0.0;
  int32_t last_launch_n = 0;
  double last_stem_ms = 0.0, last_str_ms = 0.0, last_cells = 0.0;
  int32_t last_launches = 0;
  uint32_t last_stem_classes = 0, last_s4d_classes = 0;
  void* comm = nullptr;
};

template <class F>
void run_slices(int n, F&& f) {
  std::vector<std::thread> th;
  std::vector<int> here;
  for (int t = 1; t < n; ++t) {
    try {
      th.emplace_back(f, t);
    } catch (const std::system_error&) {
      here.push_back(t);
    }
  }
  f(0);
  for (int t : here) f(t);
  for (auto& x : th) x.join();
}
int plan_threads(int want) {
  return std::max(1, std::min({want, 16, (int)std::max(1u, std::thread::hardware_concurrency())}));
}
template <class F>
void run_pool(int n, F&& work) {
  std::vector<std::thread> th;
  for (int t = 1; t < n; ++t) {
    try {
      th.emplace_back(work);
    } catch (const std::system_error&) {
      break;
    }
  }
  work();
  for (auto& x : th) x.join();
}

namespace sk {
hipStream_t ctx_stream(sk_context* ctx) { return ctx->stream; }

hipError_t lev_mark(sk_context* ctx, hipStream_t s) {
  sk_context::TSet& T = ctx->tset[ctx->tk];
  if (T.lev_used == T.lev.size()) {
    hipEvent_t e = nullptr;
    const hipError_t r = hipEventCreate(&e);
    if (r != hipSuccess) return r;
    T.lev.push_back(e);
  }
  return hipEventRecord(T.lev[T.lev_used++], s);
}

hipError_t lev_collect(sk_context* ctx) {
  sk_context::TSet& T = ctx->tset[ctx->tk];
  for (size_t i = 0; i + 1 < T.lev_used; i += 2) {
    float ms = 0.f;
    const hipError_t r = hipEventElapsedTime(&ms, T.lev[i], T.lev[i + 1]);
    if (r != hipSuccess) return r;
    ctx->last_launch_ms_sum += ms;
    ++ctx->last_launch_n;
  }
  T.lev_used = 0;
  return hipSuccess;
}

hipError_t tset_resolve(sk_context* ctx, int k) {
  sk_context::TSet& T = ctx->tset[k];
  if (!T.pending) return hipSuccess;
  T.pending = false;
  float ms = 0.f;
  hipError_t r;
  if (T.stem) {
    if ((r = hipEventSynchronize(T.ev[1])) != hipSuccess) return r;
    if ((r = hipEventElapsedTime(&ms, T.ev[0], T.ev[1])) != hipSuccess) return r;
    ctx->acc_stem_ms += ms;
  }
  if (T.str) {
    if ((r = hipEventSynchronize(T.ev[3])) != hipSuccess) return r;
    if ((r = hipEventElapsedTime(&ms, T.ev[2], T.ev[3])) != hipSuccess) return r;
    ctx->acc_str_ms += ms;
  }
  for (size_t i = 0; i + 1 < T.lev_used; i += 2) {
    if ((r = hipEventSynchronize(T.lev[i + 1])) != hipSuccess) return r;
    if ((r = hipEventElapsedTime(&ms, T.lev[i], T.lev[i + 1])) != hipSuccess) return r;
    ctx->acc_launch_ms += ms;
    ++ctx->acc_launch_n;
  }
  T.lev_used = 0;
  ctx->acc_cells += T.cells;
  ctx->acc_launches += T.launches;
  return hipSuccess;
}

hipError_t call_begin(sk_context* ctx) {
  hipError_t r;
  if (ctx->async) {
    const int k = (ctx->tk + 1) % sk_context::kTSets;
    if ((r = tset_resolve(ctx, k)) != hipSuccess) return r;
    ctx->tk = k;
    sk_context::Stage& G = ctx->stage[ctx->ncalls++ & 1];
    if (G.recorded) {
      if ((r = hipEventSynchronize(G.ev)) != hipSuccess) return r;
    } else if (G.blk || G.off) {
      if ((r = hipStreamSynchronize(ctx->stream)) != hipSuccess) return r;
      if (ctx->cps && (r = hipStreamSynchronize(ctx->cps)) != hipSuccess) return r;
    }
    G.recorded = false;
    G.blk = G.off = 0;
  } else {
    ctx->tk = 0;
  }
  sk_context::TSet& T = ctx->tset[ctx->tk];
  for (int i = 0; i < 4; ++i)
    if (!T.ev[i] && (r = hipEventCreate(&T.ev[i])) != hipSuccess) return r;
  T.lev_used = 0;
  T.pending = false;
  ctx->ev0 = T.ev[0];
  ctx->ev1 = T.ev[1];
  ctx->ev2 = T.ev[2];
  ctx->ev3 = T.ev[3];
  return hipSuccess;
}

hipError_t h2d(sk_context* ctx, void* dst, const void* src, size_t bytes, hipStream_t s) {
  if (bytes == 0) return hipSuccess;
  if (!ctx->async) return hipMemcpyAsync(dst, src, bytes, hipMemcpyHostToDevice, s);
  sk_context::Stage& G = ctx->stage[(ctx->ncalls - 1) & 1];
  const size_t need = (bytes + 255) & ~(size_t)255;
  while (G.blk < G.blocks.size() && G.off + need > G.blocks[G.blk].second) {
    ++G.blk;
    G.off = 0;
  }
  if (G.blk == G.blocks.size()) {
    const size_t cap = std::max(need, (size_t)8 << 20);
    void* p = nullptr;
    const hipError_t r = hipHostMalloc(&p, cap, hipHostMallocDefault);
    if (r != hipSuccess) return r;
    G.blocks.push_back({static_cast<char*>(p), cap});
    G.off = 0;
  }
  char* p = G.blocks[G.blk].first + G.off;
  G.off += need;
  std::memcpy(p, src, bytes);
  return hipMemcpyAsync(dst, p, bytes, hipMemcpyHostToDevice, s);
}

hipError_t up_reserve(sk_context* ctx, size_t bytes, char** dst) {
  sk_context::Stage& G = ctx->stage[(ctx->ncalls - 1) & 1];
  hipError_t r;
  if (G.dcap < bytes) {
    if (G.dbuf && (r = hipFree(G.dbuf)) != hipSuccess) return r;
    G.dbuf = nullptr;
    G.dcap = 0;
    const size_t cap = bytes + bytes / 4 + 4096;
    void* p = nullptr;
    if ((r = hipMalloc(&p, cap)) != hipSuccess) return r;
    G.dbuf = static_cast<char*>(p);
    G.dcap = cap;
  }
  *dst = G.dbuf;
  return hipSuccess;
}

hipError_t up_copy(sk_context* ctx, const void* src, size_t bytes, hipStream_t s) {
  sk_context::Stage& G = ctx->stage[(ctx->ncalls - 1) & 1];
  hipError_t r;
  if (!ctx->cps && (r = hipStreamCreateWithFlags(&ctx->cps, hipStreamNonBlocking)) != hipSuccess) return r;
  if (!G.uev && (r = hipEventCreateWithFlags(&G.uev, hipEventDisableTiming)) != hipSuccess) return r;
  if ((r = h2d(ctx, G.dbuf, src, bytes, ctx->cps)) != hipSuccess) return r;
  if ((r = hipEventRecord(G.uev, ctx->cps)) != hipSuccess) return r;
  return hipStreamWaitEvent(s, G.uev, 0);
}

hipError_t call_finish(sk_context* ctx, hipStream_t s, bool stem, bool str) {
  sk_context::TSet& T = ctx->tset[ctx->tk];
  T.stem = stem;
  T.str = str;
  T.cells = ctx->last_cells;
  T.launches = ctx->last_launches;
  hipError_t r;
  if (ctx->async) {
    sk_context::Stage& G = ctx->stage[(ctx->ncalls - 1) & 1];
    if ((r = hipEventRecord(G.ev, s)) != hipSuccess) return r;
    G.recorded = true;
    T.pending = true;
    return hipSuccess;
  }
  if ((r = hipStreamSynchronize(s)) != hipSuccess) return r;
  float ms = 0.f;
  if (stem) {
    if ((r = hipEventElapsedTime(&ms, T.ev[0], T.ev[1])) != hipSuccess) return r;
    ctx->last_stem_ms = ms;
  }
  if (str) {
    if ((r = hipEventElapsedTime(&ms, T.ev[2], T.ev[3])) != hipSuccess) return r;
    ctx->last_str_ms = ms;
  }
  return lev_collect(ctx);
}

void lev_reset(sk_context* ctx) {
  ctx->last_launch_ms_sum = 0.0;
  ctx->last_launch_n = 0;
}
int ctx_device(sk_context* ctx) { return ctx->device; }
void*& ctx_comm(sk_context* ctx) { return ctx->comm; }
void comm_destroy(void* comm);
}

namespace {

int fail(sk_context* ctx, int code, const std::string& msg) {
  if (ctx) ctx->err = msg;
  return code;
}


static void assign_sweep_lanes(const std::vector<int>& take, const std::vector<uint32_t>& er, int nl,
                               uint32_t lanes[64]) {
  const int n = (int)take.size();
  thread_local uint8_t npar[2048];
  int cntp[64];
  for (int i = 0; i < n; ++i) ++npar[(er[take[i]] >> 11) & 0x7ff];
  for (int i = 0; i < n; ++i) cntp[i] = npar[(er[take[i]] >> 11) & 0x7ff];
  for (int i = 0; i < n; ++i) npar[(er[take[i]] >> 11) & 0x7ff] = 0;
  int ord[64];
  {
    int cstart[66] = {0};
    for (int i = 0; i < n; ++i) ++cstart[64 - cntp[i] + 1];
    for (int k = 0; k < 65; ++k) cstart[k + 1] += cstart[k];
    for (int i = 0; i < n; ++i) ord[cstart[64 - cntp[i]]++] = i;
  }
  int fill[4] = {0, 0, 0, 0};
  int at[4][16];
  uint32_t rd[2][32][4];
  int rdn[2][32];
  std::memset(at, 0, sizeof(at));
  std::memset(rdn, 0, sizeof(rdn));
  auto child_load = [&](int h, uint32_t c) {
    const int sl = c & 31;
    for (int t = 0; t < std::min(rdn[h][sl], 4); ++t)
      if (rd[h][sl][t] == c) return rdn[h][sl];
    return rdn[h][sl] + 1;
  };
  auto put = [&](int g, uint32_t r) {
    const uint32_t c = r & 0x7ff, q = (r >> 11) & 0x7ff;
    const int h = g >> 1, sl = c & 31;
    bool seen = false;
    for (int t = 0; t < std::min(rdn[h][sl], 4); ++t) seen |= rd[h][sl][t] == c;
    if (!seen) {
      if (rdn[h][sl] < 4) rd[h][sl][rdn[h][sl]] = c;
      ++rdn[h][sl];
    }
    at[g][q & 15]++;
    lanes[16 * g + fill[g]++] = r;
  };
  for (int oi = 0; oi < n; ++oi) {
    const int i = ord[oi];
    const uint32_t r = er[take[i]];
    const uint32_t c = r & 0x7ff, q = (r >> 11) & 0x7ff;
    int best = -1, bc = 1 << 30;
    for (int g = 0; g < 4; ++g) {
      if (fill[g] == 16) continue;
      const int cost = 4 * (child_load(g >> 1, c) + at[g][q & 15] + 1) + fill[g];
      if (cost < bc) {
        bc = cost;
        best = g;
      }
    }
    put(best, r);
  }
  const int nl1 = std::max(nl, 1);
  for (int g = 0; g < 4; ++g) {
    while (fill[g] < 16) {
      int bs = 0, bc = 1 << 30;
      for (int sl = 0; sl < 32 && sl < nl1; ++sl) {
        const int cost = rdn[g >> 1][sl] + at[g][sl & 15];
        if (cost < bc) {
          bc = cost;
          bs = sl;
        }
      }
      const uint32_t d = (uint32_t)(bs % nl1);
      put(g, d | (d << 11));
    }
  }
}

#define SK_HIP(ctx, expr)                                                              \
  do {                                                                                 \
    hipError_t _e = (expr);                                                            \
    if (_e != hipSuccess)                                                              \
      return fail((ctx), SK_ERR_HIP, std::string(#expr) + ": " + hipGetErrorString(_e)); \
  } while (0)

int pack_dataset(sk_dataset* ds, std::string& err, const std::function<void()>* after_x = nullptr) {
  HostPack& P = ds->pack;
  const bool tstats = std::getenv("SK_HOST_STATS") != nullptr;
  auto tnow = [] { return std::chrono::duration<double, std::milli>(std::chrono::steady_clock::now().time_since_epoch()).count(); };
  const double tp0 = tnow();
  const char* lanes_env = SK_KNOB("SK_SWEEP_LANES");
  const bool sweep_lanes_greedy = !lanes_env || std::atoi(lanes_env) != 0;
  P = HostPack();
  const int n = (int)ds->ex.size();
  auto is_gamma = [&](const Example& X, int v) {
    const uint32_t e0 = X.edge_off[v], e1 = X.edge_off[v + 1];
// ... 1223 lines not shown

static int col_waves(int cpl, int min_m, int max_m, int max_n) {
  static const int w_env = SK_KNOB("SK4C_W") ? std::max(1, std::atoi(SK_KNOB("SK4C_W"))) : 0;
  int W = std::min(w_env ? w_env : sk::stem4d_col_max_waves(cpl), sk::stem4d_col_max_waves(cpl));
  if (min_m != INT32_MAX) W = std::min(W, sk::stem4d_col_w_max(min_m));
  W = std::max(W, 1);
  while (W > 1 && sk::stem4d_col_lds_bytes(cpl, W, max_m, max_n) > 160 * 1024) --W;
  return W;
}

int run_stem4d(sk_context* ctx, sk_dataset* xs_, sk_dataset* ys_, const sk_kernel_params* kp,
               const int32_t* x, const int32_t* y, int64_t n, double* out_dev) {
  if (kp->bp_model < 0 || kp->bp_model > 2 || !(kp->bp_bound >= 0.0))
    return fail(ctx, SK_ERR_INVALID, "4-D stem kernel: bp_model 0..2 and bp_bound >= 0");
  const float ali_bound = (float)kp->ali_bound;
  const bool ali = ali_bound > 0.0f;
  const bool ali_phmm = ali && kp->ali_zerop_fixed;
  std::shared_ptr<const Stem4dTables> tx, ty;
  int rc = stem4d_dataset_tables(ctx, xs_, kp, &tx);
  if (rc) return rc;
  if (ys_ == xs_) ty = tx;
  else if ((rc = stem4d_dataset_tables(ctx, ys_, kp, &ty))) return rc;
  const Stem4dTables& TX = *tx;
  const Stem4dTables& TY = *ty;
  auto usable = [&](const Stem4dTables& T, int e) -> int {
    if (T.why[e] == 1) return fail(ctx, SK_ERR_INVALID, "4-D stem kernel takes single sequences");
    if (T.why[e] == 2) return fail(ctx, SK_ERR_INVALID, "4-D stem kernel with bp_model 0 needs base pairs");
    if (ali && !T.acgu[e])
      return fail(ctx, SK_ERR_INVALID, "4-D stem kernel: alignment constraints need A/C/G/U sequences");
    return SK_OK;
  };
  int max_m = 0, max_n = 0;
  double cells = 0.0;
  for (int64_t k = 0; k < n; ++k) {
    if ((rc = usable(TX, x[k])) || (rc = usable(TY, y[k]))) return rc;
    const double a = xs_->ex[x[k]].len, b = ys_->ex[y[k]].len;
    max_m = std::max(max_m, (int)b);
    max_n = std::max(max_n, (int)a);
    cells += (a + 1) * (a + 2) / 2 * (b + 1) * (b + 2) / 2;
  }
  ctx->last_cells = cells;
  size_t free_b = 0, total_b = 0;
  SK_HIP(ctx, hipMemGetInfo(&free_b, &total_b));
  const double budget = std::min(128e9, 0.5 * (double)free_b);
  std::vector<int64_t> order(n);
  std::iota(order.begin(), order.end(), 0);
  const std::vector<double> gp = gap_powers(kp->gap, std::max(max_m, max_n) + 2);
  rc = ensure_work(ctx, gp.size() * 8 + 4096);
  if (rc) return rc;
  Arena A{static_cast<char*>(ctx->work), 0, ctx->work_bytes};
  double* d_gp = A.take<double>(gp.size());
  hipStream_t S = ctx->stream;
  SK_HIP(ctx, hipMemcpyAsync(d_gp, gp.data(), gp.size() * 8, hipMemcpyHostToDevice, S));
  const int cpl = sk::stem4d_cpl(max_m);
  const bool ktiles = max_m + 1 > 64 * cpl;
  const int64_t kb_stride = ktiles ? 4 * (int64_t)(max_m + 1) : 0;
  const bool banded = ali_phmm || (!ali && kp->len_band > 0);
  const bool gsum = !banded && !SK_KNOB("SK4_NO_GSUM");
  const size_t nst = gsum ? 2 : 4;
  const bool colk_call = gsum && !ktiles && !SK_KNOB("SK4_SPAN") && !SK_KNOB("SK4_NO_PRE");
  const int col_nb = colk_call ? sk::stem4d_col_nb(cpl) : 0;
  auto col_ok = [&](int64_t q) {
    const int m = ys_->ex[y[q]].len;
    return colk_call && xs_->ex[x[q]].len <= sk::stem4d_col_max_n() &&
           (m <= 1 || sk::stem4d_col_w_max(m) >= 1);
  };
  std::stable_sort(order.begin(), order.end(), [&](int64_t a, int64_t b) {
    const bool ca = col_ok(a), cb = col_ok(b);
    if (ca != cb) return ca;
    return xs_->ex[x[a]].len > xs_->ex[x[b]].len;
  });
  double total_ms = 0.0;
  int launches = 0;
  Stem4dBatch& Bt = ctx->s4d;
  for (int64_t b0 = 0; b0 < n;) {
    std::vector<sk::Stem4dPair> prs;
    double bytes = 0.0;
    size_t ring_bytes = 0;
    int64_t b1 = b0;
    int maxn = 0;
    const bool colk = col_ok(order[b0]);
    while (b1 < n && prs.size() < 4096 && col_ok(order[b1]) == colk) {
      const int64_t q = order[b1];
      sk::Stem4dPair p;
      p.n = xs_->ex[x[q]].len;
      p.m = ys_->ex[y[q]].len;
      p.plane_doubles = stem4d_plane_doubles(p.m);
      const size_t rb = colk ? ((size_t)(p.n + col_nb) * (size_t)p.plane_doubles * 8 + 255) & ~(size_t)255
                             : ((size_t)3 * (p.n + 1) * nst * (size_t)p.plane_doubles * 8 +
                                (gsum ? (size_t)(p.n + 1) * 8 : 0) + 255) & ~(size_t)255;
      const double pb = (double)rb + (double)(p.n + 1) * (double)kb_stride * 8.0;
      if (!prs.empty() && bytes + pb > budget) break;
      p.scratch_off = (int64_t)(ring_bytes / 8);
      bytes += pb;
      ring_bytes += rb;
      p.x_bp = TX.bp_off[x[q]];
      p.x_chr = TX.ch_off[x[q]];
      p.y_bp = TY.bp_off[y[q]];
      p.y_chr = TY.ch_off[y[q]];
      p.out_index = q;
      maxn = std::max(maxn, p.n);
      prs.push_back(p);
      ++b1;
    }
    if (colk) {
      int min_m = INT32_MAX;
      for (const auto& p : prs)
        if (p.m >= 2) min_m = std::min(min_m, p.m);
      const int W = col_waves(cpl, min_m, max_m, maxn);
      rc = ensure_scratch(ctx, ring_bytes + 64);
      if (rc) return rc;
      if (Bt.cap_pairs < prs.size()) {
        if (Bt.pairs) {
          SK_HIP(ctx, hipStreamSynchronize(S));
          (void)hipFree(Bt.pairs);
        }
        Bt.cap_pairs = std::max<size_t>(prs.size(), 64);
        SK_HIP(ctx, hipMalloc(&Bt.pairs, Bt.cap_pairs * sizeof(sk::Stem4dPair)));
      }
      SK_HIP(ctx, hipMemcpyAsync(Bt.pairs, prs.data(), prs.size() * sizeof(sk::Stem4dPair),
                                 hipMemcpyHostToDevice, S));
      sk::Stem4dLaunch L;
      L.pairs = Bt.pairs;
      L.scratch = ctx->scratch;
      L.bpdiag = TX.bp;
      L.chars = TX.ch;
      L.bpdiag_y = TY.bp;
      L.chars_y = TY.ch;
      L.gpow = d_gp;
      L.gap = kp->gap;
      L.stack = kp->stack;
      L.subst = kp->subst;
      L.bp_bound = (float)kp->bp_bound;
      L.out = out_dev;
      L.gsum = 3;
      SK_HIP(ctx, hipEventRecord(ctx->ev0, S));
      SK_HIP(ctx, sk::lev_mark(ctx, S));
      SK_HIP(ctx, sk::launch_stem4d_col(L, (int64_t)prs.size(), cpl, W, max_m, maxn, S));
      SK_HIP(ctx, sk::lev_mark(ctx, S));
      ctx->last_s4d_classes |= 1u << ((cpl == 1 ? 0 : cpl == 2 ? 1 : cpl == 4 ? 2 : 3) + 8);
      ++launches;
      SK_HIP(ctx, hipEventRecord(ctx->ev1, S));
      SK_HIP(ctx, hipStreamSynchronize(S));
      SK_HIP(ctx, sk::lev_collect(ctx));
      float ms = 0.f;
      SK_HIP(ctx, hipEventElapsedTime(&ms, ctx->ev0, ctx->ev1));
      total_ms += ms;
      b0 = b1;
      continue;
    }
    std::vector<int32_t> blo, bhi;
    size_t n_band = 0;
    int max_n1 = 1, max_m1 = 1;
    if (ali_phmm) {
      for (auto& p : prs) {
        p.band_off = (int64_t)n_band;
        n_band += (size_t)p.n + 1;
        max_n1 = std::max(max_n1, p.n + 1);
        max_m1 = std::max(max_m1, p.m + 1);
      }
    } else if (!ali && kp->len_band > 0) {
      for (auto& p : prs) {
        p.band_off = (int64_t)blo.size();
        for (int i = 0; i <= p.n; ++i) {
          const unsigned jj = p.n ? (unsigned)((double)i / p.n * p.m + 0.5) : 0u;
          blo.push_back((int32_t)(jj < kp->len_band ? 0u : jj - kp->len_band));
          bhi.push_back((int32_t)(jj + kp->len_band > (unsigned)p.m ? (unsigned)p.m : jj + kp->len_band));
        }
      }
    }
    int nh = SK_KNOB("SK4_STREAMS") ? std::atoi(SK_KNOB("SK4_STREAMS")) : 4;
    if (SK_KNOB("SK_SERIAL_CLASSES") || ktiles) nh = 1;
    nh = std::max(1, std::min({nh, 4, (int)prs.size()}));
    const hipStream_t hs[4] = {S, ctx->cls, ctx->side, ctx->aux};
    std::vector<int2> items;
    std::vector<int64_t> ioff((size_t)(maxn + 1) * nh + 1, 0);
    for (int d1 = 0; d1 <= maxn; ++d1)
      for (int h = 0; h < nh; ++h) {
        ioff[(size_t)d1 * nh + h] = (int64_t)items.size();
        for (size_t p = h; p < prs.size(); p += nh)
          for (int i = 0; i + d1 <= prs[p].n; ++i) items.push_back(make_int2((int)p, i));
      }
    ioff.back() = (int64_t)items.size();
    if (!ali_phmm) n_band = blo.size();
    const size_t phmm_bytes =
        ali_phmm ? prs.size() * sk::phmm_pair_bytes(max_n1, max_m1) : 0;
    const size_t kb_bytes = ktiles ? (size_t)(ioff[nh] - ioff[0]) * (size_t)kb_stride * 8 : 0;
    rc = ensure_scratch(ctx, std::max(ring_bytes + kb_bytes + 64, phmm_bytes));
    if (rc) return rc;
    if (Bt.cap_pairs < prs.size() || Bt.cap_items < items.size()) {
      if (Bt.pairs) (void)hipFree(Bt.pairs);
      if (Bt.items) (void)hipFree(Bt.items);
      Bt.cap_pairs = std::max<size_t>(prs.size(), 64);
      Bt.cap_items = std::max<size_t>(items.size(), 4096);
      SK_HIP(ctx, hipMalloc(&Bt.pairs, Bt.cap_pairs * sizeof(sk::Stem4dPair)));
      SK_HIP(ctx, hipMalloc(&Bt.items, Bt.cap_items * sizeof(int2)));
    }
    SK_HIP(ctx, hipMemcpyAsync(Bt.pairs, prs.data(), prs.size() * sizeof(sk::Stem4dPair),
                               hipMemcpyHostToDevice, S));
    SK_HIP(ctx, hipMemcpyAsync(Bt.items, items.data(), items.size() * sizeof(int2),
                               hipMemcpyHostToDevice, S));
    if (n_band) {
      if (Bt.cap_band < n_band) {
        if (Bt.band) {
          SK_HIP(ctx, hipStreamSynchronize(S));
          (void)hipFree(Bt.band);
        }
        Bt.cap_band = std::max<size_t>(n_band, 4096);
        SK_HIP(ctx, hipMalloc(&Bt.band, 2 * Bt.cap_band * sizeof(int32_t)));
      }
      if (!blo.empty()) {
        SK_HIP(ctx, hipMemcpyAsync(Bt.band, blo.data(), blo.size() * 4, hipMemcpyHostToDevice, S));
        SK_HIP(ctx, hipMemcpyAsync(Bt.band + Bt.cap_band, bhi.data(), bhi.size() * 4,
                                   hipMemcpyHostToDevice, S));
      }
    }
    sk::Stem4dLaunch L;
    L.pairs = Bt.pairs;
    L.scratch = ctx->scratch;
    L.bpdiag = TX.bp;
    L.chars = TX.ch;
    L.bpdiag_y = TY.bp;
    L.chars_y = TY.ch;
    L.gpow = d_gp;
    L.gap = kp->gap;
    L.stack = kp->stack;
    L.subst = kp->subst;
    L.bp_bound = (float)kp->bp_bound;
    L.out = out_dev;
    L.band_lo = n_band ? Bt.band : nullptr;
    L.band_hi = n_band ? Bt.band + Bt.cap_band : nullptr;
    L.kbound = ktiles ? ctx->scratch + ring_bytes / 8 : nullptr;
    L.kbound_stride = kb_stride;
    const bool no_pre = SK_KNOB("SK4_NO_PRE") != nullptr;
    L.gsum = gsum ? (!ktiles && !no_pre ? 2 : 1) : 0;
    SK_HIP(ctx, hipEventRecord(ctx->ev0, S));
    if (ali_phmm) {
      sk::PhmmLaunch H;
      H.pairs = Bt.pairs;
      H.n_pairs = (int64_t)prs.size();
      H.chars = TX.ch;
      H.chars_y = TY.ch;
      H.scratch = reinterpret_cast<char*>(ctx->scratch);
      H.n1 = max_n1;
      H.m1 = max_m1;
      H.pair_bytes = sk::phmm_pair_bytes(max_n1, max_m1);
      H.ali_bound = ali_bound;
      H.band = kp->len_band;
      H.zerop_fixed = kp->ali_zerop_fixed ? 1 : 0;
      H.band_lo = Bt.band;
      H.band_hi = Bt.band + Bt.cap_band;
      SK_HIP(ctx, sk::launch_phmm(H, S));
    }
    if (nh > 1) {
      SK_HIP(ctx, hipEventRecord(ctx->evk, S));
      for (int h = 1; h < nh; ++h) SK_HIP(ctx, hipStreamWaitEvent(hs[h], ctx->evk, 0));
    }
    for (int d1 = 0; d1 <= maxn; ++d1)
      for (int h = 0; h < nh; ++h) {
        const size_t q = (size_t)d1 * nh + h;
        L.d1 = d1;
        L.items = Bt.items + ioff[q];
        L.n_items = ioff[q + 1] - ioff[q];
        if (!L.n_items) continue;
        SK_HIP(ctx, sk::lev_mark(ctx, hs[h]));
        SK_HIP(ctx, sk::launch_stem4d(L, cpl, hs[h]));
        SK_HIP(ctx, sk::lev_mark(ctx, hs[h]));
        ctx->last_s4d_classes |= 1u << ((cpl == 1 ? 0 : cpl == 2 ? 1 : cpl == 4 ? 2 : 3) +
                                        (L.band_lo ? 4 : 0));
        ++launches;
      }
    for (int h = 1; h < nh; ++h) {
      hipEvent_t e = h == 1 ? ctx->evx : h == 2 ? ctx->evj : ctx->eva;
      SK_HIP(ctx, hipEventRecord(e, hs[h]));
      SK_HIP(ctx, hipStreamWaitEvent(S, e, 0));
    }
    SK_HIP(ctx, hipEventRecord(ctx->ev1, S));
    SK_HIP(ctx, hipStreamSynchronize(S));
    SK_HIP(ctx, sk::lev_collect(ctx));
    float ms = 0.f;
    SK_HIP(ctx, hipEventElapsedTime(&ms, ctx->ev0, ctx->ev1));
    total_ms += ms;
    b0 = b1;
  }
  ctx->last_stem_ms = total_ms;
  ctx->last_launches = launches;
  return SK_OK;
}

int run_pairs(sk_context* ctx, sk_dataset* xs_, sk_dataset* ys_, const sk_kernel_params* kp,
              const int32_t* x, const int32_t* y, int64_t n, double* out_dev) {
  if (!ctx || !kp) return fail(ctx, SK_ERR_INVALID, "null argument");
  int rc = check_set(ctx, xs_);
  if (rc) return rc;
  rc = check_set(ctx, ys_);
  if (rc) return rc;
  if (n < 0) return fail(ctx, SK_ERR_INVALID, "negative pair count");
  if (kp->kind < SK_SU_STEM || kp->kind > SK_STEM4D)
    return fail(ctx, SK_ERR_UNSUPPORTED, "unknown kernel kind");
  ctx->last_stem_ms = ctx->last_str_ms = ctx->last_cells = 0.0;
  ctx->last_launches = 0;
  sk::lev_reset(ctx);
  ctx->last_stem_classes = ctx->last_s4d_classes = 0;
  if (n == 0) return SK_OK;
  const int nx = (int)xs_->ex.size(), ny = (int)ys_->ex.size();
  for (int64_t k = 0; k < n; ++k)
    if (x[k] < 0 || x[k] >= nx || y[k] < 0 || y[k] >= ny)
      return fail(ctx, SK_ERR_RANGE, "pair index out of range");
  SK_HIP(ctx, sk::call_begin(ctx));
  if (kind_is_bpla(kp->kind)) return run_bpla(ctx, xs_, ys_, kp, x, y, n, out_dev);
  if (kp->kind == SK_STEM4D) {
    rc = run_stem4d(ctx, xs_, ys_, kp, x, y, n, out_dev);
    if (rc == SK_OK && ctx->async) {
      ctx->acc_stem_ms += ctx->last_stem_ms;
      ctx->acc_cells += ctx->last_cells;
      ctx->acc_launches += ctx->last_launches;
      ctx->acc_launch_ms += ctx->last_launch_ms_sum;
      ctx->acc_launch_n += ctx->last_launch_n;
    }
    return rc;
  }

  const bool stem = kind_has_stem(kp->kind), str = kind_has_str(kp->kind);
  const HostPack& PX = xs_->pack;
  const HostPack& PY = ys_->pack;
  const bool host_stats = std::getenv("SK_HOST_STATS") != nullptr;
  auto now_ms = [] {
    return std::chrono::duration<double, std::milli>(std::chrono::steady_clock::now().time_since_epoch()).count();
  };
  const double th0 = host_stats ? now_ms() : 0.0;
  double th1 = th0, th2 = th0;

  struct StemClass {
    int maxk = 0;
    int max_nl = 0, max_edges = 0, max_bpf = 0, max_nch = 0;
    int nwaves = 1, grid = 1;
    size_t item_off = 0, n_items = 0;
  };
  std::vector<StemClass> classes;
  std::vector<int4> items;
  std::vector<int32_t> ixs;
  std::vector<int64_t> ioidx;
  std::vector<int32_t> big_x, big_y;
  std::vector<int64_t> big_o;
  int big_max_nl = 0;
  const int max_len = std::max(PX.max_len, PY.max_len);
  if (stem) {
    std::vector<int64_t> cnt(ny + 1, 0);
    for (int64_t k = 0; k < n; ++k) cnt[y[k] + 1]++;
    for (int j = 0; j < ny; ++j) cnt[j + 1] += cnt[j];
    std::vector<int64_t> byy(n);
    {
      std::vector<int64_t> pos(cnt.begin(), cnt.end() - 1);
      for (int64_t k = 0; k < n; ++k) byy[pos[y[k]]++] = k;
    }
    {
      std::atomic<int> nextj{0};
      auto work = [&]() {
        std::vector<uint64_t> key;
        std::vector<int64_t> tmp;
        for (int j = nextj.fetch_add(1); j < ny; j = nextj.fetch_add(1)) {
          const int64_t b = cnt[j], e = cnt[j + 1];
          if (e - b < 2) continue;
          key.resize(e - b);
          for (int64_t t = b; t < e; ++t)
            key[t - b] = ((uint64_t)(0xffffffffu - (uint32_t)PX.ex_nl[x[byy[t]]]) << 32) | (uint32_t)(t - b);
          std::sort(key.begin(), key.end());
          tmp.assign(byy.begin() + b, byy.begin() + e);
          for (int64_t t = b; t < e; ++t) byy[t] = tmp[(uint32_t)key[t - b]];
        }
      };
      run_pool(plan_threads(n / 65536 + 1), work);
    }
    ixs.resize(n);
    ioidx.resize(n);
    for (int64_t t = 0; t < n; ++t) {
      ixs[t] = x[byy[t]];
      ioidx[t] = byy[t];
    }
    const bool force_big = [] {
      const char* e = SK_KNOB("SK_FORCE_BIG_Y");
      return e && std::atoi(e) != 0;
    }();
    std::vector<uint8_t> ybig(ny, 0);
    for (int j = 0; j < ny; ++j) ybig[j] = force_big || PY.ex_big[j] ? 1 : 0;
    auto in_class = [&](int j, int maxk) {
      return !ybig[j] && sk::stem_maxk(PY.ex_nl[j] + 1) == maxk;
    };
    {
      std::vector<int64_t> bk;
      for (int j = 0; j < ny; ++j) {
        if (!ybig[j] || cnt[j + 1] == cnt[j]) continue;
        big_max_nl = std::max(big_max_nl, PY.ex_nl[j]);
        for (int64_t t = cnt[j]; t < cnt[j + 1]; ++t) bk.push_back(byy[t]);
      }
      std::stable_sort(bk.begin(), bk.end(), [&](int64_t a, int64_t b) {
        return (double)PX.ex_nl[x[a]] * PY.ex_nl[y[a]] > (double)PX.ex_nl[x[b]] * PY.ex_nl[y[b]];
      });
      for (int64_t k : bk) {
        big_x.push_back(x[k]);
        big_y.push_back(y[k]);
        big_o.push_back(k);
      }
    }
    for (int maxk : {32, 28, 24, 20, 17, 16, 12, 8, 4}) {
      StemClass C;
      C.maxk = maxk;
      bool any = false;
      for (int j = 0; j < ny; ++j) {
        if (cnt[j + 1] == cnt[j] || !in_class(j, maxk)) continue;
        any = true;
        C.max_nl = std::max(C.max_nl, PY.ex_nl[j]);
        C.max_edges = std::max(C.max_edges, PY.ex_edge_base[j + 1] - PY.ex_edge_base[j]);
        C.max_bpf = std::max(C.max_bpf, PY.ex_bpf_base[j + 1] - PY.ex_bpf_base[j]);
        C.max_nch = std::max(C.max_nch, PY.ex_nch[j]);
      }
      if (!any) continue;
      sk::StemLaunch L;
      L.lds_max_nl = 64 * maxk;
      L.lds_max_edges = (C.max_edges + 3) & ~3;
      L.lds_max_bpf = (C.max_bpf + 1 + 3) & ~3;
      L.lds_max_nch = C.max_nch + 2;
      L.lds_max_len_pad = (max_len + 2 + 3) & ~3;
      L.n_gpow = max_len + 2;
      L.n_gpow_pad = (L.n_gpow + 1) & ~1;
      L.xset.n_gam = (int32_t)PX.gam_key.size();
      L.gam_on = L.xset.n_gam > 0;
      int max_dyn = 0, vgprs = 0, max_w = 8;
      SK_HIP(ctx, sk::stem_kernel_attr(L.lds_max_nl, &max_dyn, &vgprs, &max_w));
      const int valloc = ((std::max(vgprs, 1) + 7) / 8) * 8;
      const int waves_cu_vgpr = 4 * std::min(8, 512 / valloc);
      int best = 0, per_cu = 1;
      for (int w = max_w; w >= 1; --w) {
        const size_t lds = sk::stem_lds_bytes(L, w);
        if (lds > (size_t)max_dyn) continue;
        const int pc = std::min<int>((int)(163840 / lds), std::min(32, waves_cu_vgpr) / w);
        if (pc * w > best) {
          best = pc * w;
          C.nwaves = w;
          per_cu = pc;
        }
      }
      if (best == 0) return fail(ctx, SK_ERR_UNSUPPORTED, "y example too large for LDS");
#ifdef SK_STAMPS
      if (const char* fw = SK_KNOB("SK_FORCE_WAVES")) {
        int w = 0, pc = 0;
        if (std::sscanf(fw, "%d,%d", &w, &pc) == 2 && w >= 1 && w <= C.nwaves && pc >= 1) {
          C.nwaves = w;
          per_cu = pc;
        }
      }
#endif
      C.grid = ctx->n_cu * per_cu;
      std::vector<int> ysel;
      double class_cost = 0.0;
      for (int j = 0; j < ny; ++j) {
        if (cnt[j + 1] == cnt[j] || !in_class(j, maxk)) continue;
        ysel.push_back(j);
        for (int64_t t = cnt[j]; t < cnt[j + 1]; ++t)
          class_cost += (double)PX.ex_nl[x[byy[t]]] * (double)PY.ex_nl[j];
      }
      std::stable_sort(ysel.begin(), ysel.end(), [&](int a, int b) {
        return cnt[a + 1] - cnt[a] > cnt[b + 1] - cnt[b];
      });
      double gss_k = 1.5;
      if (const char* e = SK_KNOB("SK_GSS_K")) gss_k = std::max(0.25, std::atof(e));
      const double share = 1.0 / (gss_k * (double)C.grid);
      double remaining = class_cost;
      C.item_off = items.size();
      for (int j : ysel) {
        const double yw = (double)PY.ex_nl[j];
        int64_t b = cnt[j];
        while (b < cnt[j + 1]) {
          const double target = remaining * share;
          int64_t e = b;
          double cost = 0.0;
          while (e < cnt[j + 1] && (e - b < C.nwaves || cost < target)) {
            const int64_t re = std::min<int64_t>(cnt[j + 1], e + C.nwaves);
            for (int64_t t = e; t < re; ++t) cost += (double)PX.ex_nl[x[byy[t]]] * yw;
            e = re;
          }
          items.push_back(make_int4(j, (int)b, (int)(e - b), 0));
          remaining -= cost;
          b = e;
        }
      }
      C.n_items = items.size() - C.item_off;
      C.grid = (int)std::min<int64_t>(C.grid, std::max<int64_t>(1, (int64_t)C.n_items));
      classes.push_back(C);
    }
    double cells = 0.0;
    for (int64_t k = 0; k < n; ++k) cells += (double)PX.ex_nl[x[k]] * (double)PY.ex_nl[y[k]];
    ctx->last_cells = cells;
  }

  if (host_stats) th1 = now_ms();
  std::vector<int32_t> item_phi_off, item_phi;
  const bool phi_on = stem && !PX.phi_al.empty() && !PX.gam_key.empty();
  if (phi_on) {
    const size_t W = (PX.phi_al.size() + 63) / 64;
    const size_t ni = items.size();
    const int T = plan_threads((int)(ni / 512 + 1));
    std::vector<std::vector<int32_t>> tkeys(T), tcnt(T);
    run_slices(T, [&](int t) {
      std::vector<uint64_t> acc(W);
      for (size_t i = ni * t / T; i < ni * (t + 1) / T; ++i) {
        const int4 it = items[i];
        const size_t k0 = tkeys[t].size();
        if (PY.ex_gapless[it.x]) {
          std::fill(acc.begin(), acc.end(), 0ull);
          for (int u = it.y; u < it.y + it.z; ++u) {
            const uint64_t* b = PX.ex_phi_bits.data() + (size_t)ixs[u] * W;
            for (size_t w = 0; w < W; ++w) acc[w] |= b[w];
          }
          for (size_t w = 0; w < W; ++w)
            for (uint64_t m = acc[w]; m; m &= m - 1) tkeys[t].push_back((int32_t)(w * 64 + __builtin_ctzll(m)));
        }
        tcnt[t].push_back((int32_t)(tkeys[t].size() - k0));
      }
    });
    item_phi_off.assign(1, 0);
    for (int t = 0; t < T; ++t) {
      item_phi.insert(item_phi.end(), tkeys[t].begin(), tkeys[t].end());
      for (int32_t c : tcnt[t]) item_phi_off.push_back(item_phi_off.back() + c);
    }
    if (std::getenv("SK_PHI_STATS"))
      std::fprintf(stderr, "[phi] keys=%zu items=%zu item keys=%zu pairs=%lld phi components=%zu rows=%zu\n",
                   PX.phi_al.size(), items.size(), item_phi.size(), (long long)n, PX.phk_idx.size(),
                   PX.xgrow.size());
  }

  if (host_stats) th2 = now_ms();
  std::vector<int32_t> spx, spy;
  std::vector<int64_t> soidx;
  int64_t n_soh = 0, n_sfast = 0;
  const int str_lds_len = (std::max(PY.max_len, 64) + 1) & ~1;
  if (str && kp->kind != SK_NAIVE_STR && !SK_KNOB("SK_STR_GENERAL") &&
      sk::str_fast_wave_lds_bytes(str_lds_len, false) + sk::kStrFastLds0 <= 163840) {
    auto cat = [&](int64_t k) {
      const int a = x[k], b = y[k];
      if (PX.ex_has_w[a] != PY.ex_has_w[b]) return 2;
      if (PX.ex_onehot[a] && PY.ex_onehot[b]) return 0;
      return PX.ex_str_fast[a] && PY.ex_str_fast[b] ? 1 : 2;
    };
    int64_t cnt3[3] = {0, 0, 0};
    for (int64_t k = 0; k < n; ++k) ++cnt3[cat(k)];
    n_soh = cnt3[0];
    n_sfast = cnt3[0] + cnt3[1];
    if (cnt3[0] != n && cnt3[1] != n && cnt3[2] != n) {
      spx.reserve(n);
      spy.reserve(n);
      soidx.reserve(n);
      for (int c = 0; c < 3; ++c)
        for (int64_t k = 0; k < n; ++k)
          if (cat(k) == c) {
            spx.push_back(x[k]);
            spy.push_back(y[k]);
            soidx.push_back(k);
          }
    }
  }
  const size_t n_str_pos = n_sfast ? PX.pos_prof.size() + (ys_ == xs_ ? 0 : PY.pos_prof.size()) : 0;

  const size_t nb = (size_t)n;
  size_t need = 0;
  need += soidx.size() * 8 + n_str_pos * (2 * sizeof(sk::StrPos) + sizeof(sk::StrCode)) + 1024;
  need += (item_phi_off.size() + item_phi.size()) * 4 + 512;
  need += 256 * 8 + 16 * 8 + (size_t)(max_len + 4) * 8 * 2;
  need += 1024;
  need += items.size() * sizeof(int4) + nb * (4 + 8) + nb * 8 * 2 + nb * 4 * 2 + 64 + 8 * 256;
  need += big_x.size() * (4 + 4 + 8) + 3 * 256;
  need += 16 * 256;
  rc = ensure_work(ctx, need);
  if (rc) return rc;
  Arena A{static_cast<char*>(ctx->work), 0, ctx->work_bytes};
  double* d_co = A.take<double>(256);
  double* d_gp_loop = A.take<double>(max_len + 4);
  double* d_st = A.take<double>(16);
  double* d_gp_str = A.take<double>(max_len + 4);
  int4* d_items = A.take<int4>(std::max<size_t>(items.size(), 1));
  int32_t* d_ixs = A.take<int32_t>(std::max<size_t>(nb, 1));
  int64_t* d_oidx = A.take<int64_t>(std::max<size_t>(nb, 1));
  double* d_stem = A.take<double>(nb);
  double* d_str = A.take<double>(nb);
  int32_t* d_px = A.take<int32_t>(nb);
  int32_t* d_py = A.take<int32_t>(nb);
  int* d_ctr = A.take<int>(64);
  int32_t* d_bx = A.take<int32_t>(std::max<size_t>(big_x.size(), 1));
  int32_t* d_by = A.take<int32_t>(std::max<size_t>(big_x.size(), 1));
  int64_t* d_bo = A.take<int64_t>(std::max<size_t>(big_x.size(), 1));
  int32_t* d_iphi_off = A.take<int32_t>(std::max<size_t>(item_phi_off.size(), 1));
  int32_t* d_iphi = A.take<int32_t>(std::max<size_t>(item_phi.size(), 1));
  int64_t* d_soidx = soidx.empty() ? nullptr : A.take<int64_t>(soidx.size());
  sk::StrPos* d_stab = (n_sfast > n_soh) ? A.take<sk::StrPos>(2 * n_str_pos) : nullptr;
  sk::StrCode* d_ctab = n_soh ? A.take<sk::StrCode>(n_str_pos) : nullptr;

  std::vector<double> co(256), st(16);
  const bool subst = kind_subst(kp->kind);
  for (int k = 0; k < 256; ++k)
    co[k] = subst ? std::exp(SK_RIBOSUM_P[k] * kp->beta)
                  : ((k >> 4) == (k & 15) ? kp->stack : kp->covar);
  for (int k = 0; k < 16; ++k)
    st[k] = subst ? std::exp(SK_RIBOSUM_S[k] * kp->alpha)
                  : ((k >> 2) == (k & 3) ? kp->match : kp->mismatch);
  const std::vector<double> gl = gap_powers(kp->loop_gap, max_len + 4);
  const std::vector<double> gs = gap_powers(kp->gap, max_len + 4);
  hipStream_t S = ctx->stream;
  SK_HIP(ctx, sk::h2d(ctx, d_co, co.data(), 256 * 8, S));
  SK_HIP(ctx, sk::h2d(ctx, d_st, st.data(), 16 * 8, S));
  SK_HIP(ctx, sk::h2d(ctx, d_gp_loop, gl.data(), gl.size() * 8, S));
  SK_HIP(ctx, sk::h2d(ctx, d_gp_str, gs.data(), gs.size() * 8, S));
  SK_HIP(ctx, hipMemsetAsync(d_ctr, 0, 64 * sizeof(int), S));

  double* stem_out = (combine_mode(kp->kind) == sk::kCombineStem) ? out_dev : d_stem;
  double* str_out = (combine_mode(kp->kind) == sk::kCombineStr) ? out_dev : d_str;

  const bool side = stem && str;
  if (str) {
    SK_HIP(ctx, sk::h2d(ctx, d_px, spx.empty() ? x : spx.data(), nb * 4, S));
    SK_HIP(ctx, sk::h2d(ctx, d_py, spy.empty() ? y : spy.data(), nb * 4, S));
    if (d_soidx)
      SK_HIP(ctx, sk::h2d(ctx, d_soidx, soidx.data(), soidx.size() * 8, S));
    if (side) {
      SK_HIP(ctx, hipEventRecord(ctx->evf, S));
      SK_HIP(ctx, hipStreamWaitEvent(ctx->side, ctx->evf, 0));
    }
  }
  if (stem) {
    SK_HIP(ctx, sk::h2d(ctx, d_items, items.data(), items.size() * sizeof(int4), S));
    SK_HIP(ctx, sk::h2d(ctx, d_ixs, ixs.data(), nb * 4, S));
    SK_HIP(ctx, sk::h2d(ctx, d_oidx, ioidx.data(), nb * 8, S));
    if (phi_on) {
      SK_HIP(ctx, sk::h2d(ctx, d_iphi_off, item_phi_off.data(), item_phi_off.size() * 4, S));
      if (!item_phi.empty())
        SK_HIP(ctx, sk::h2d(ctx, d_iphi, item_phi.data(), item_phi.size() * 4, S));
    }
    const double gap2 = kp->loop_gap * kp->loop_gap;
    const size_t nnd = std::max<size_t>(PX.nd_a.size(), 1);
    const size_t nxc = std::max<size_t>(PX.xr_ch.size(), 1), nxg = std::max<size_t>(PX.xgrow.size(), 1),
                 nxgc = std::max<size_t>(PX.xg_ch.size(), 1),
                 ngh = std::max<size_t>(PX.ex_nl.size() * PX.gam_key.size(), 1),
                 nphk = std::max<size_t>(PX.phk_idx.size(), 1);
    if (!xs_->prep) {
      void* p = nullptr;
      SK_HIP(ctx, hipMalloc(&p, (3 * nnd + nxc + nxg + nxgc + ngh + nphk) * sizeof(double)));
      xs_->prep = static_cast<double*>(p);
      xs_->buf.ptrs.push_back(p);
      xs_->prep_loop_gap = -1.0;
    }
    sk::DevParamNodes pn;
    pn.nd_L = xs_->prep;
    pn.nd_SL = xs_->prep + nnd;
    pn.xr_SL = xs_->prep + 2 * nnd;
    pn.xr_chw = xs_->prep + 3 * nnd;
    pn.xg_SL = pn.xr_chw + nxc;
    pn.xg_chw = pn.xg_SL + nxg;
    pn.gam_h = pn.xg_chw + nxgc;
    pn.phk_w = pn.gam_h + ngh;
    if (!(xs_->prep_loop_gap == kp->loop_gap)) {
      SK_HIP(ctx, sk::launch_prep(xs_->dev, pn, d_gp_loop, gap2, S));
      xs_->prep_loop_gap = kp->loop_gap;
    }
    const bool two_streams = classes.size() > 1 && !SK_KNOB("SK_SERIAL_CLASSES");
    size_t scratch_need = 0, scratch_x = 0;
    for (size_t c = 0; c < classes.size(); ++c) {
      const StemClass& C = classes[c];
      const int64_t slab = (int64_t)(PX.max_slots + 1) * 64 * C.maxk;
      const int64_t gtab = (int64_t)PX.gam_key.size() * 64 * C.maxk;
      const int64_t ptab = phi_on ? (int64_t)PX.phi_al.size() * (64 * C.maxk + 1) : 0;
      const size_t b = (size_t)C.grid * (C.nwaves * slab + gtab + ptab) * sizeof(double);
      size_t& r = (two_streams && (c & 1)) ? scratch_x : scratch_need;
      r = std::max(r, b);
    }
    const int64_t big_stride = ((int64_t)std::max(big_max_nl, 1) + 63) / 64 * 64;
    const int64_t big_wave = (int64_t)(PX.max_slots + 2) * big_stride;
    int big_grid = 0;
    if (!big_x.empty()) {
      size_t free_b = 0, total_b = 0;
      SK_HIP(ctx, hipMemGetInfo(&free_b, &total_b));
      const size_t budget = std::max<size_t>(std::min<size_t>(free_b / 2, (size_t)32 << 30),
                                             (size_t)big_wave * 8 * sk::kStemBigWaves);
      const int64_t by_mem = (int64_t)(budget / ((size_t)big_wave * 8 * sk::kStemBigWaves));
      const int64_t by_pairs = ((int64_t)big_x.size() + sk::kStemBigWaves - 1) / sk::kStemBigWaves;
      big_grid = (int)std::max<int64_t>(1, std::min<int64_t>({by_mem, by_pairs, (int64_t)ctx->n_cu * 8}));
      scratch_need = std::max(scratch_need,
                              (size_t)big_grid * sk::kStemBigWaves * (size_t)big_wave * sizeof(double));
    }
    scratch_need = (scratch_need + 255) / 256 * 256;
    rc = ensure_scratch(ctx, std::max<size_t>(scratch_need + scratch_x, 64));
    if (rc) return rc;
    double* scratch_cls = ctx->scratch + scratch_need / sizeof(double);
#ifdef SK_STAMPS
    unsigned long long* d_stamps = nullptr;
    SK_HIP(ctx, hipMalloc(&d_stamps, 16 * sizeof(unsigned long long)));
    SK_HIP(ctx, hipMemsetAsync(d_stamps, 0, 16 * sizeof(unsigned long long), S));
#endif
    if (host_stats)
      std::fprintf(stderr, "[host] pairs=%lld plan %.2f ms, phi keys %.2f ms, uploads+prep %.2f ms\n",
                   (long long)n, th1 - th0, th2 - th1, now_ms() - th2);
    SK_HIP(ctx, hipEventRecord(ctx->ev0, S));
    if (two_streams) {
      SK_HIP(ctx, hipEventRecord(ctx->evk, S));
      SK_HIP(ctx, hipStreamWaitEvent(ctx->cls, ctx->evk, 0));
    }
    for (size_t c = 0; c < classes.size(); ++c) {
      const StemClass& C = classes[c];
      const bool on_cls = two_streams && (c & 1);
      sk::StemLaunch SL;
      SL.xset = xs_->dev;
      SL.yset = ys_->dev;
      SL.pn = pn;
      SL.co_subst = d_co;
      SL.gpow = d_gp_loop;
      SL.n_gpow = max_len + 2;
      SL.n_gpow_pad = (SL.n_gpow + 1) & ~1;
      SL.gap2 = gap2;
      SL.band = kp->len_band;
      SL.lds_max_nl = 64 * C.maxk;
      SL.lds_max_edges = (C.max_edges + 3) & ~3;
      SL.lds_max_bpf = (C.max_bpf + 1 + 3) & ~3;
      SL.lds_max_nch = C.max_nch + 2;
      SL.lds_max_len_pad = (max_len + 2 + 3) & ~3;
      SL.items = d_items + C.item_off;
      SL.n_items = (int32_t)C.n_items;
      SL.xs = d_ixs;
      SL.oidx = d_oidx;
      SL.out = stem_out;
      SL.item_counter = d_ctr + 16 + (int)c;
      SL.slab_doubles = (int64_t)(PX.max_slots + 1) * SL.lds_max_nl;
      SL.scratch = on_cls ? scratch_cls : ctx->scratch;
      SL.gam_on = !PX.gam_key.empty();
      SL.gam_doubles = (int64_t)PX.gam_key.size() * SL.lds_max_nl;
      SL.gam = SL.scratch + (size_t)C.grid * C.nwaves * SL.slab_doubles;
      SL.phi_on = phi_on ? 1 : 0;
      SL.phi_doubles = phi_on ? (int64_t)PX.phi_al.size() * (SL.lds_max_nl + 1) : 0;
      SL.phi = SL.gam + (size_t)C.grid * SL.gam_doubles;
      SL.item_phi_off = d_iphi_off + C.item_off;
      SL.item_phi = d_iphi;
#ifdef SK_STAMPS
      SL.stamps = d_stamps;
#endif
      SK_HIP(ctx, sk::lev_mark(ctx, on_cls ? ctx->cls : S));
      SK_HIP(ctx, sk::launch_stem(SL, C.grid, C.nwaves, on_cls ? ctx->cls : S));
      SK_HIP(ctx, sk::lev_mark(ctx, on_cls ? ctx->cls : S));
      ctx->last_stem_classes |= 1u << (C.maxk % 4 ? C.maxk : C.maxk / 4);
    }
    if (two_streams) {
      SK_HIP(ctx, hipEventRecord(ctx->evx, ctx->cls));
      SK_HIP(ctx, hipStreamWaitEvent(S, ctx->evx, 0));
    }
    if (!big_x.empty()) {
      const size_t nbig = big_x.size();
      SK_HIP(ctx, sk::h2d(ctx, d_bx, big_x.data(), nbig * 4, S));
      SK_HIP(ctx, sk::h2d(ctx, d_by, big_y.data(), nbig * 4, S));
      SK_HIP(ctx, sk::h2d(ctx, d_bo, big_o.data(), nbig * 8, S));
      sk::StemBigLaunch BL;
      BL.xset = xs_->dev;
      BL.yset = ys_->dev;
      BL.pn = pn;
      BL.co_subst = d_co;
      BL.gpow = d_gp_loop;
      BL.n_gpow = max_len + 2;
      BL.gap2 = gap2;
      BL.band = kp->len_band;
      BL.xs = d_bx;
      BL.ys = d_by;
      BL.oidx = d_bo;
      BL.n_pairs = (int64_t)nbig;
      BL.out = stem_out;
      BL.scratch = ctx->scratch;
      BL.stride = big_stride;
      BL.wave_doubles = big_wave;
      SK_HIP(ctx, sk::lev_mark(ctx, S));
      SK_HIP(ctx, sk::launch_stem_big(BL, big_grid, S));
      SK_HIP(ctx, sk::lev_mark(ctx, S));
      ctx->last_stem_classes |= 1u;
    }
    SK_HIP(ctx, hipEventRecord(ctx->ev1, S));
#ifdef SK_STAMPS
    {
      unsigned long long h[16];
      SK_HIP(ctx, hipMemcpyAsync(h, d_stamps, sizeof(h), hipMemcpyDeviceToHost, S));
      SK_HIP(ctx, hipStreamSynchronize(S));
      (void)hipFree(d_stamps);
      const double rows = (double)h[8];
      std::fprintf(stderr, "[stamps] classes=%zu pairs=%llu rows=%.0f cycles/row:", classes.size(),
                   h[9], rows);
      const char* nm[7] = {"hdr", "A", "Rfill", "passes", "zero", "sweep", "store"};
      for (int i = 0; i < 7; ++i) std::fprintf(stderr, " %s=%.0f", nm[i], h[i] / rows);
      std::fprintf(stderr, "\n[stamps] per row: A-loaded rows=%.3f swept chunks=%.2f match passes=%.2f band nodes=%.1f\n",
                   h[10] / rows, h[11] / rows, h[12] / rows, h[13] / rows);
      for (const StemClass& C : classes)
        std::fprintf(stderr, "[stamps] class maxk=%d max_nl=%d max_edges=%d max_nch=%d waves/wg=%d grid=%d items=%zu\n",
                     C.maxk, C.max_nl, C.max_edges, C.max_nch, C.nwaves, C.grid, C.n_items);
    }
#endif
    ctx->last_launches = (int32_t)classes.size() + (big_x.empty() ? 0 : 1);
  }
  if (str) {
    const hipStream_t SS = side ? ctx->side : S;
    sk::StrLaunch T;
    T.xset = xs_->dev;
    T.yset = ys_->dev;
    T.st = d_st;
    T.gpow = d_gp_str;
    T.gap = kp->gap;
    T.naive = kp->kind == SK_NAIVE_STR ? 1 : 0;
    T.xs = d_px + n_sfast;
    T.ys = d_py + n_sfast;
    T.oidx = d_soidx ? d_soidx + n_sfast : nullptr;
    T.n_pairs = n - n_sfast;
    T.out = str_out;
    T.pair_counter = reinterpret_cast<unsigned long long*>(d_ctr + 8);
    T.lds_max_len = (std::max(PY.max_len, 1) + 1) & ~1;
    int w = 4;
    while (w > 1 && sk::str_lds_bytes(T, w) > 65536) w /= 2;
    const size_t lds = sk::str_lds_bytes(T, w);
    if (lds > 163840) return fail(ctx, SK_ERR_UNSUPPORTED, "sequence too long for string kernel LDS");
    const int per_cu = std::max(1, std::min<int>((int)(163840 / lds), 8));
    const int64_t g = std::max<int64_t>(1, std::min<int64_t>((int64_t)ctx->n_cu * per_cu, (n - n_sfast + w - 1) / w));
    SK_HIP(ctx, hipEventRecord(ctx->ev2, SS));
    for (int oh = 1; oh >= 0; --oh) {
      const int64_t b = oh ? 0 : n_soh, e = oh ? n_soh : n_sfast;
      if (e <= b) continue;
      const size_t npx = PX.pos_prof.size(), npy = PY.pos_prof.size();
      const void *tx, *ty;
      if (oh) {
        SK_HIP(ctx, sk::launch_str_code_tab(xs_->dev.pos_prof, xs_->dev.pos_w, (int64_t)npx, d_ctab, SS));
        if (ys_ != xs_)
          SK_HIP(ctx, sk::launch_str_code_tab(ys_->dev.pos_prof, ys_->dev.pos_w, (int64_t)npy, d_ctab + npx, SS));
        tx = d_ctab;
        ty = ys_ != xs_ ? d_ctab + npx : d_ctab;
      } else {
        SK_HIP(ctx, sk::launch_str_tab(xs_->dev.pos_prof, xs_->dev.pos_w, (int64_t)npx, d_st, d_stab,
                                       d_stab + npx, SS));
        tx = d_stab;
        ty = d_stab + npx;
        if (ys_ != xs_) {
          SK_HIP(ctx, sk::launch_str_tab(ys_->dev.pos_prof, ys_->dev.pos_w, (int64_t)npy, d_st, d_stab + 2 * npx,
                                         d_stab + 2 * npx + npy, SS));
          ty = d_stab + 2 * npx + npy;
        }
      }
      sk::StrFastLaunch F;
      F.xset = xs_->dev;
      F.yset = ys_->dev;
      F.xtab = static_cast<const sk::StrPos*>(tx);
      F.ytab = static_cast<const sk::StrPos*>(ty);
      F.st = d_st;
      F.onehot = oh;
      F.gpow = d_gp_str;
      F.gap = kp->gap;
      F.xs = d_px + b;
      F.ys = d_py + b;
      F.oidx = d_soidx ? d_soidx + b : nullptr;
      F.n_pairs = e - b;
      F.out = str_out;
      F.lds_max_len = (std::max(PY.max_len, 64) + 1) & ~1;
      const size_t wl = sk::str_fast_wave_lds_bytes(F.lds_max_len, oh != 0);
      if (wl + sk::kStrFastLds0 > 163840) return fail(ctx, SK_ERR_UNSUPPORTED, "sequence too long for string kernel LDS");
      const int per_cu_w = (int)std::max<size_t>(1, std::min<size_t>(16, (163840 - sk::kStrFastLds0) / wl));
      const int fw = std::min(4, per_cu_w);
      const int64_t fg = std::min<int64_t>((int64_t)ctx->n_cu * std::max(1, per_cu_w / fw), (e - b + fw - 1) / fw);
      SK_HIP(ctx, sk::launch_str_fast(F, (int)fg, fw, SS));
    }
    if (n_sfast < n) SK_HIP(ctx, sk::launch_str(T, (int)g, w, SS));
    SK_HIP(ctx, hipEventRecord(ctx->ev3, SS));
    if (side) {
      SK_HIP(ctx, hipEventRecord(ctx->evj, ctx->side));
      SK_HIP(ctx, hipStreamWaitEvent(S, ctx->evj, 0));
    }
  }
  const int32_t mode = combine_mode(kp->kind);
  if (mode != sk::kCombineStem && mode != sk::kCombineStr)
    SK_HIP(ctx, sk::launch_combine(d_stem, d_str, out_dev, n, mode, kp->alpha, kp->beta, S));
  SK_HIP(ctx, sk::call_finish(ctx, S, stem, str));
  return SK_OK;
}

int bpla_gradients(sk_context* ctx, sk_dataset* xs_, sk_dataset* ys_, const sk_kernel_params* kp,
                   const int32_t* x, const int32_t* y, int64_t n, double* value, double* grad) {
  if (!ctx || !xs_ || !ys_ || !kp || (n > 0 && (!x || !y || !value || !grad)))
    return fail(ctx, SK_ERR_INVALID, "null argument");
  int rc = check_set(ctx, xs_);
  if (rc) return rc;
  rc = check_set(ctx, ys_);
  if (rc) return rc;
  if (n <= 0) return n < 0 ? fail(ctx, SK_ERR_INVALID, "negative pair count") : SK_OK;
  SK_HIP(ctx, sk::call_begin(ctx));
  for (int64_t k = 0; k < n; ++k) {
    if (x[k] < 0 || x[k] >= (int)xs_->ex.size() || y[k] < 0 || y[k] >= (int)ys_->ex.size())
      return fail(ctx, SK_ERR_INVALID, "pair index out of range");
    if (!xs_->ex[x[k]].has_bp || !ys_->ex[y[k]].has_bp)
      return fail(ctx, SK_ERR_INVALID, "BPLA gradients need examples built with use_bp");
  }
  size_t free_b = 0, total_b = 0;
  SK_HIP(ctx, hipMemGetInfo(&free_b, &total_b));
  const double budget = std::min(96e9, 0.6 * (double)free_b);
  rc = ensure_work(ctx, 16 * 8 + 4096);
  if (rc) return rc;
  double* d_tb = static_cast<double*>(ctx->work);
  hipStream_t S = ctx->stream;
  SK_HIP(ctx, hipMemcpyAsync(d_tb, kp->score_table, 16 * 8, hipMemcpyHostToDevice, S));
  struct DevBuf {
    void* p = nullptr;
    ~DevBuf() {
      if (p) (void)hipFree(p);
    }
  } xy_buf, out_buf;
  SK_HIP(ctx, hipMalloc(&xy_buf.p, (size_t)2 * n * sizeof(int32_t)));
  SK_HIP(ctx, hipMalloc(&out_buf.p, (size_t)10 * n * sizeof(double)));
  int32_t* d_xy = static_cast<int32_t*>(xy_buf.p);
  double* d_out = static_cast<double*>(out_buf.p);
  SK_HIP(ctx, hipMemcpyAsync(d_xy, x, (size_t)n * 4, hipMemcpyHostToDevice, S));
  SK_HIP(ctx, hipMemcpyAsync(d_xy + n, y, (size_t)n * 4, hipMemcpyHostToDevice, S));
  double total_ms = 0.0;
  const HostPack& PX = xs_->pack;
  const HostPack& PY = ys_->pack;
  std::vector<int32_t> wx, wy, gx, gy;
  std::vector<int64_t> wo, go;
  const bool general_only = SK_KNOB("SK_BPLA_GENERAL") != nullptr;
  for (int64_t k = 0; k < n; ++k) {
    if (!general_only && PX.ex_dyadic[x[k]] && PY.ex_dyadic[y[k]]) {
      wx.push_back(x[k]);
      wy.push_back(y[k]);
      wo.push_back(k);
    } else {
      gx.push_back(x[k]);
      gy.push_back(y[k]);
      go.push_back(k);
    }
  }
  if (!wx.empty()) {
    const size_t nw = wx.size();
    const size_t npx = PX.pos_prof.size(), npy = ys_ == xs_ ? 0 : PY.pos_prof.size();
    const size_t ntab = 2 * (npx + npy);
    int tmax = 1, maxlen = 64;
    for (size_t k = 0; k < nw; ++k) {
      tmax = std::max(tmax, sk::bpla_steps(xs_->ex[wx[k]].len, ys_->ex[wy[k]].len));
      maxlen = std::max(maxlen, ys_->ex[wy[k]].len);
    }
    maxlen = (maxlen + 1) & ~1;
    const size_t wl = sk::bpla_grad_wave_lds_bytes(maxlen);
    if (wl + sk::kBplaExpLds > 163840)
      return fail(ctx, SK_ERR_UNSUPPORTED, "sequence too long for the BPLA gradient kernel LDS");
    const int per_cu_w = (int)std::max<size_t>(1, std::min<size_t>(16, (163840 - 2 * sk::kBplaExpLds) / wl));
    const int wpb = std::min(4, per_cu_w);
    const int64_t bt = (int64_t)3 * 64 * tmax;
    int64_t grid = (int64_t)ctx->n_cu * std::max(1, per_cu_w / wpb);
    grid = std::min<int64_t>(grid, std::max<int64_t>(1, ((int64_t)nw + wpb - 1) / wpb));
    grid = std::min<int64_t>(grid, std::max<int64_t>(1, (int64_t)(budget / (8.0 * bt * wpb))));
    DevBuf tab_buf, idx_buf;
    SK_HIP(ctx, hipMalloc(&tab_buf.p, ntab * sizeof(sk::BplaPos) + 64));
    SK_HIP(ctx, hipMalloc(&idx_buf.p, nw * (4 + 4 + 8) + 64));
    int32_t* d_wx = static_cast<int32_t*>(idx_buf.p);
    int32_t* d_wy = d_wx + nw;
    int64_t* d_wo = reinterpret_cast<int64_t*>(static_cast<char*>(idx_buf.p) + ((nw * 8 + 15) & ~size_t(15)));
    unsigned long long* d_cnt = reinterpret_cast<unsigned long long*>(d_tb + 16);
    SK_HIP(ctx, hipMemcpyAsync(d_wx, wx.data(), nw * 4, hipMemcpyHostToDevice, S));
    SK_HIP(ctx, hipMemcpyAsync(d_wy, wy.data(), nw * 4, hipMemcpyHostToDevice, S));
    SK_HIP(ctx, hipMemcpyAsync(d_wo, wo.data(), nw * 8, hipMemcpyHostToDevice, S));
    SK_HIP(ctx, hipMemsetAsync(d_cnt, 0, 8, S));
    sk::BplaPos* tabs = static_cast<sk::BplaPos*>(tab_buf.p);
    sk::BplaPos* tx = tabs;
    sk::BplaPos* ty = tabs + npx;
    SK_HIP(ctx, sk::launch_bpla_tab(xs_->dev.pos_prof, xs_->dev.pos_lru, (int64_t)npx, d_tb, 1.0, tx,
                                    tabs + npx, S));
    if (npy) {
      ty = tabs + 2 * npx + npy;
      SK_HIP(ctx, sk::launch_bpla_tab(ys_->dev.pos_prof, ys_->dev.pos_lru, (int64_t)npy, d_tb, 1.0,
                                      tabs + 2 * npx, ty, S));
    }
    rc = ensure_scratch(ctx, (size_t)grid * wpb * (size_t)bt * 8 + 64);
    if (rc) return rc;
    sk::BplaGradLaunch W;
    W.xset = xs_->dev;
    W.yset = ys_->dev;
    W.table = d_tb;
    W.alpha = kp->alpha;
    W.beta = kp->beta;
    W.gap = kp->gap;
    W.ext = kp->ext;
    W.beta_gap = std::exp(kp->beta * kp->gap);
    W.beta_ext = std::exp(kp->beta * kp->ext);
    W.xs = d_wx;
    W.ys = d_wy;
    W.n_pairs = (int64_t)nw;
    W.scratch = ctx->scratch;
    W.value = d_out;
    W.grad = d_out + n;
    W.xtab = tx;
    W.ytab = ty;
    W.pair_counter = d_cnt;
    W.oidx = d_wo;
    W.lds_max_len = maxlen;
    W.bt_doubles = bt;
    SK_HIP(ctx, hipEventRecord(ctx->ev0, S));
    SK_HIP(ctx, sk::launch_bpla_grad_wave(W, (int)grid, wpb, S));
    SK_HIP(ctx, hipEventRecord(ctx->ev1, S));
    SK_HIP(ctx, hipStreamSynchronize(S));
    float ms = 0.f;
    SK_HIP(ctx, hipEventElapsedTime(&ms, ctx->ev0, ctx->ev1));
    total_ms += ms;
  }
  if (!wx.empty() && !gx.empty()) {
    SK_HIP(ctx, hipMemcpyAsync(d_xy, gx.data(), gx.size() * 4, hipMemcpyHostToDevice, S));
    SK_HIP(ctx, hipMemcpyAsync(d_xy + n, gy.data(), gy.size() * 4, hipMemcpyHostToDevice, S));
  }
  const int64_t ng = wx.empty() ? n : (int64_t)gx.size();
  const int32_t* hx = wx.empty() ? x : gx.data();
  const int32_t* hy = wx.empty() ? y : gy.data();
  double* g_out = wx.empty() ? d_out : d_out + 5 * n;
  for (int64_t b0 = 0; b0 < ng && rc == SK_OK;) {
    int n1 = 1, m1 = 1;
    int64_t b1 = b0;
    while (b1 < ng) {
      const int a1 = std::max(n1, xs_->ex[hx[b1]].len + 1), c1 = std::max(m1, ys_->ex[hy[b1]].len + 1);
      if (b1 > b0 && (double)(b1 - b0 + 1) * sk::bpla_grad_pair_bytes(a1, c1) > budget) break;
      n1 = a1, m1 = c1, ++b1;
    }
    const int64_t cnt = b1 - b0;
    rc = ensure_scratch(ctx, (size_t)cnt * sk::bpla_grad_pair_bytes(n1, m1) + 64);
    if (rc) break;
    sk::BplaGradLaunch G;
    G.xset = xs_->dev;
    G.yset = ys_->dev;
    G.table = d_tb;
    G.alpha = kp->alpha;
    G.beta = kp->beta;
    G.gap = kp->gap;
    G.ext = kp->ext;
    G.beta_gap = std::exp(kp->beta * kp->gap);
    G.beta_ext = std::exp(kp->beta * kp->ext);
    G.xs = d_xy + b0;
    G.ys = d_xy + n + b0;
    G.n_pairs = cnt;
    G.n1 = n1;
    G.m1 = m1;
    G.scratch = ctx->scratch;
    G.value = g_out + b0;
    G.grad = g_out + ng + 4 * b0;
    SK_HIP(ctx, hipEventRecord(ctx->ev0, S));
    SK_HIP(ctx, sk::launch_bpla_grad(G, S));
    SK_HIP(ctx, hipEventRecord(ctx->ev1, S));
    SK_HIP(ctx, hipStreamSynchronize(S));
    float ms = 0.f;
    SK_HIP(ctx, hipEventElapsedTime(&ms, ctx->ev0, ctx->ev1));
// ... 975 lines not shown
    const size_t need = sq.size() * sizeof(sk::FoldSeq) + codes.size() + lp.size() + tab.size() * 8 +
                        (outn + nb) * 8 + strn + 10 * 256;
    int rc = ensure_work(ctx, need);
    if (rc) return rc;
    rc = ensure_scratch(ctx, std::max<size_t>(work * 8, 64));
    if (rc) return rc;
    Arena A{static_cast<char*>(ctx->work), 0, ctx->work_bytes};
    sk::FoldSeq* d_sq = A.take<sk::FoldSeq>(sq.size());
    int8_t* d_codes = A.take<int8_t>(std::max<size_t>(codes.size(), 1));
    double* d_tab = A.take<double>(tab.size());
    double* d_out = A.take<double>(std::max<size_t>(outn, 1));
    double* d_lz = A.take<double>(nb);
    uint8_t* d_lp = no_lp ? A.take<uint8_t>(std::max<size_t>(lp.size(), 1)) : nullptr;
    if (no_lp && !lp.empty())
      SK_HIP(ctx, hipMemcpyAsync(d_lp, lp.data(), lp.size(), hipMemcpyHostToDevice, S));
    SK_HIP(ctx, hipMemcpyAsync(d_sq, sq.data(), sq.size() * sizeof(sk::FoldSeq), hipMemcpyHostToDevice, S));
    if (!codes.empty())
      SK_HIP(ctx, hipMemcpyAsync(d_codes, codes.data(), codes.size(), hipMemcpyHostToDevice, S));
    SK_HIP(ctx, hipMemcpyAsync(d_tab, tab.data(), tab.size() * 8, hipMemcpyHostToDevice, S));
    SK_HIP(ctx, hipMemsetAsync(ctx->scratch, 0, work * 8, S));
    SK_HIP(ctx, hipMemsetAsync(d_out, 0, std::max<size_t>(outn, 1) * 8, S));
    char* d_str = want_str ? A.take<char>(std::max<size_t>(strn, 1)) : nullptr;
    int32_t* d_status = sm ? A.take<int32_t>(1) : nullptr;
    if (want_str && strn) SK_HIP(ctx, hipMemsetAsync(d_str, '.', strn, S));
    if (sm) SK_HIP(ctx, hipMemsetAsync(d_status, 0, sizeof(int32_t), S));
    L.seqs = d_sq;
    L.codes = d_codes;
    L.tab = d_tab;
    L.lp = d_lp;
    L.work = ctx->scratch;
    L.out = d_out;
    L.log_z = d_lz;
    if (stats)
      std::fprintf(stderr, "[sk] fold batch: %d items, longest %d, path %s\n", nb, bmax,
                   sk::fold_path_name(K.path(L, bmax)));
    SK_HIP(ctx, K.launch(L, nb, bmax, S));
    std::vector<double> lz(nb);
    std::vector<uint32_t> cnt;
    int32_t status = 0;
    if (sm) {
      sk::FoldSampleLaunch SL;
      SL.F = L;
      SL.cnt = reinterpret_cast<uint32_t*>(d_out);
      SL.structs = d_str;
      SL.status = d_status;
      SL.n_samples = sm->n_samples;
      SL.seq_base = b0;
      SL.seed = sm->seed;
      SK_HIP(ctx, sk::launch_fold_sample(SL, nb, bmax, S));
      if (out && outn) {
        cnt.resize(outn);
        SK_HIP(ctx, hipMemcpyAsync(cnt.data(), d_out, outn * 4, hipMemcpyDeviceToHost, S));
      }
      if (strn) SK_HIP(ctx, hipMemcpyAsync(sm->structs + str_host, d_str, strn, hipMemcpyDeviceToHost, S));
      SK_HIP(ctx, hipMemcpyAsync(&status, d_status, sizeof(int32_t), hipMemcpyDeviceToHost, S));
    } else if (outn) {
      SK_HIP(ctx, hipMemcpyAsync(out + out_host, d_out, outn * 8, hipMemcpyDeviceToHost, S));
    }
    SK_HIP(ctx, hipMemcpyAsync(lz.data(), d_lz, nb * 8, hipMemcpyDeviceToHost, S));
    SK_HIP(ctx, hipStreamSynchronize(S));
    for (int k = 0; k < nb; ++k) {
      if (!std::isfinite(lz[k])) return fail(ctx, SK_ERR_UNSUPPORTED, K.out_of_range);
      if (log_z) log_z[b0 + k] = lz[k];
    }
    if (status == sk::kFoldSampleRunaway)
      return fail(ctx, SK_ERR_HIP, "fold sampling: a walk made more than 2 n + 2 decisions");
    if (status == sk::kFoldSampleNoWeight)
      return fail(ctx, SK_ERR_HIP, "fold sampling: a decision's candidates sum to 0 or a non-finite value");
    if (status != 0) return fail(ctx, SK_ERR_HIP, "fold sampling: more open segments than the stack holds");
    for (size_t a = 0; a < cnt.size(); ++a) out[out_host + a] = (double)cnt[a] / (double)ns;
    out_host += outn;
    str_host += strn;
    b0 = b1;
  }
  if (stats) std::fprintf(stderr, "[sk] fold: %d items in %d batches\n", (int)n, n_batches);
  return SK_OK;
}

}

int sk_fold_mccaskill(sk_context* ctx, int32_t n, const char* const* seqs, int32_t flags,
                      double* out, double* log_z) {
  if (!ctx || n < 0 || (n > 0 && (!seqs || !out))) return fail(ctx, SK_ERR_INVALID, "null argument");
  if (flags & ~(SK_FOLD_NO_GU | SK_FOLD_NO_CLOSING_GU | SK_FOLD_NO_LONELY_PAIRS))
    return fail(ctx, SK_ERR_UNSUPPORTED, "fold: unknown flag");
  return fold_batches(ctx, kFoldPlain, n, nullptr, seqs, flags, out, log_z, nullptr);
}

int sk_fold_sample(sk_context* ctx, int32_t n, const char* const* seqs, int32_t flags,
                   int32_t n_samples, uint64_t seed, double* out_bpp, char* out_structs, double* log_z) {
  if (!ctx || n < 0 || (n > 0 && !seqs)) return fail(ctx, SK_ERR_INVALID, "null argument");
  if (n_samples < 1) return fail(ctx, SK_ERR_INVALID, "fold sampling: n_samples must be at least 1");
  if (!out_bpp && !out_structs) return fail(ctx, SK_ERR_INVALID, "fold sampling: no output asked for");
  if (flags & ~(SK_FOLD_NO_GU | SK_FOLD_NO_CLOSING_GU | SK_FOLD_NO_LONELY_PAIRS))
    return fail(ctx, SK_ERR_UNSUPPORTED, "fold: unknown flag");
  FoldSampling sm;
  sm.n_samples = n_samples;
  sm.seed = seed;
  sm.structs = out_structs;
  return fold_batches(ctx, kFoldPlain, n, nullptr, seqs, flags, out_bpp, log_z, &sm);
}

double sk_fold_sample_uniform(uint64_t seed, int32_t seq, int32_t sample, int32_t draw) {
  return sk::rng_uniform(sk::rng_stream(seed, seq, sample), draw);
}

int sk_fold_alignment(sk_context* ctx, int32_t n_aln, const int32_t* n_rows, const char* const* rows,
                      int32_t flags, double* out, double* log_z) {
  if (!ctx || n_aln < 0 || (n_aln > 0 && (!n_rows || !rows || !out))) return fail(ctx, SK_ERR_INVALID, "null argument");
  if (flags & ~(SK_FOLD_NO_GU | SK_FOLD_NO_CLOSING_GU | SK_FOLD_NO_LONELY_PAIRS))
    return fail(ctx, SK_ERR_UNSUPPORTED, "fold: unknown flag");
  if (flags & SK_FOLD_NO_CLOSING_GU)
    return fail(ctx, SK_ERR_UNSUPPORTED,
                "consensus fold: --noClosingGU has no per-column meaning when the rows differ");
  size_t r = 0;
  for (int32_t k = 0, len = 0; k < n_aln; ++k) {
    if (n_rows[k] < 1) return fail(ctx, SK_ERR_INVALID, "consensus fold: an alignment needs at least one row");
    if (n_rows[k] > sk::kAliMaxRows) return fail(ctx, SK_ERR_UNSUPPORTED, "consensus fold: too many rows");
    for (int32_t a = 0; a < n_rows[k]; ++a, ++r) {
      if (!rows[r]) return fail(ctx, SK_ERR_INVALID, "null row");
      const int m = (int)std::strlen(rows[r]);
      if (a == 0) len = m;
      else if (m != len) return fail(ctx, SK_ERR_INVALID, "consensus fold: rows of unequal length");
    }
  }
  return fold_batches(ctx, kFoldAli, n_aln, n_rows, rows, flags, out, log_z, nullptr);
}

namespace {
int add_examples_threaded(sk_dataset* ds, int32_t n, int32_t n_rows, const char* const* rows,
                          const double* const* bpp_rows, const char* const* labels, float th,
                          int use_bp, int32_t n_threads, bool consensus = false) {
  const size_t base = ds->ex.size();
  try {
    ds->ex.resize(base + n);
    for (int32_t i = 0; i < n; ++i) ds->labels.emplace_back(labels && labels[i] ? labels[i] : "+1");
  } catch (const std::bad_alloc&) {
    return SK_ERR_ALLOC;
  }
  int nt = n_threads > 0 ? n_threads : (int)std::thread::hardware_concurrency();
  nt = std::max(1, std::min(nt, std::max<int32_t>(n, 1)));
  std::atomic<int32_t> next(0), status(SK_OK);
  auto work = [&]() {
    for (;;) {
      const int32_t i = next.fetch_add(1);
      if (i >= n || status.load() != SK_OK) return;
      try {
        sk::build_example(ds->ex[base + i], n_rows, rows + (size_t)i * n_rows,
                          use_bp ? bpp_rows + (size_t)i * (consensus ? 1 : n_rows) : nullptr, th, use_bp != 0,
                          consensus);
      } catch (...) {
        status.store(SK_ERR_INVALID);
      }
    }
  };
  run_pool(nt, work);
  if (status.load() != SK_OK) {
    ds->ex.resize(base);
    ds->labels.resize(base);
  }
  return status.load();
}
}

int sk_dataset_add_batch(sk_dataset* ds, int32_t n, int32_t n_rows, const char* const* rows,
                         const double* const* bpp_rows, const char* const* labels, float th,
                         int32_t use_bp, int32_t n_threads) {
  if (!ds || n < 0 || n_rows < 1 || (n > 0 && (!rows || (use_bp && !bpp_rows)))) return SK_ERR_INVALID;
  if (ds->uploaded) return SK_ERR_INVALID;
  return add_examples_threaded(ds, n, n_rows, rows, bpp_rows, labels, th, use_bp, n_threads);
}

namespace {
int add_folded(sk_context* ctx, sk_dataset* ds, int32_t n, int32_t n_rows, const char* const* rows,
               const char* const* labels, float th, int32_t fold_flags, int32_t n_samples, uint64_t seed,
               int32_t n_threads) {
  if (!ctx || !ds || n < 0 || n_rows < 1 || (n > 0 && !rows)) return fail(ctx, SK_ERR_INVALID, "null argument");
  if (ds->uploaded) return fail(ctx, SK_ERR_INVALID, "dataset already uploaded");
  const size_t nr = (size_t)n * n_rows;
  std::vector<std::string> erased(nr);
  std::vector<const char*> eptr(nr);
  std::vector<size_t> off(nr + 1, 0);
  for (size_t r = 0; r < nr; ++r) {
    if (!rows[r]) return fail(ctx, SK_ERR_INVALID, "null row");
    for (const char* p = rows[r]; *p; ++p)
      if (*p != '-') erased[r].push_back((char)std::tolower((unsigned char)*p));
    eptr[r] = erased[r].c_str();
    const size_t m = erased[r].size();
    off[r + 1] = off[r] + (m > 1 ? m * (m - 1) / 2 : 0);
  }
  std::vector<double> bpp(std::max<size_t>(off[nr], 1));
  int rc = n_samples > 0 ? sk_fold_sample(ctx, (int32_t)nr, eptr.data(), fold_flags, n_samples, seed, bpp.data(),
                                          nullptr, nullptr)
                         : sk_fold_mccaskill(ctx, (int32_t)nr, eptr.data(), fold_flags, bpp.data(), nullptr);
  if (rc) return rc;
  std::vector<const double*> bptr(nr);
  for (size_t r = 0; r < nr; ++r) bptr[r] = bpp.data() + off[r];
  rc = add_examples_threaded(ds, n, n_rows, rows, bptr.data(), labels, th, 1, n_threads);
  return rc ? fail(ctx, rc, "example build failed") : SK_OK;
}
}

int sk_dataset_add_folded(sk_context* ctx, sk_dataset* ds, int32_t n, int32_t n_rows,
                          const char* const* rows, const char* const* labels, float th,
                          int32_t fold_flags, int32_t n_threads) {
  return add_folded(ctx, ds, n, n_rows, rows, labels, th, fold_flags, 0, 0, n_threads);
}

int sk_dataset_add_sampled(sk_context* ctx, sk_dataset* ds, int32_t n, int32_t n_rows,
                           const char* const* rows, const char* const* labels, float th,
                           int32_t fold_flags, int32_t n_samples, uint64_t seed, int32_t n_threads) {
  if (n_samples < 1) return fail(ctx, SK_ERR_INVALID, "fold sampling: n_samples must be at least 1");
  return add_folded(ctx, ds, n, n_rows, rows, labels, th, fold_flags, n_samples, seed, n_threads);
}

int sk_dataset_add_alifolded(sk_context* ctx, sk_dataset* ds, int32_t n, int32_t n_rows,
                             const char* const* rows, const char* const* labels, float th,
                             int32_t fold_flags, int32_t n_threads) {
  if (!ctx || !ds || n < 0 || n_rows < 1 || (n > 0 && !rows)) return fail(ctx, SK_ERR_INVALID, "null argument");
  if (ds->uploaded) return fail(ctx, SK_ERR_INVALID, "dataset already uploaded");
  std::vector<size_t> off((size_t)n + 1, 0);
  for (int32_t i = 0; i < n; ++i) {
    if (!rows[(size_t)i * n_rows]) return fail(ctx, SK_ERR_INVALID, "null row");
    const size_t m = std::strlen(rows[(size_t)i * n_rows]);
    off[i + 1] = off[i] + (m > 1 ? m * (m - 1) / 2 : 0);
  }
  std::vector<double> bpp(std::max<size_t>(off[n], 1));
  const std::vector<int32_t> nr((size_t)n, n_rows);
  int rc = sk_fold_alignment(ctx, n, nr.data(), rows, fold_flags, bpp.data(), nullptr);
  if (rc) return rc;
  std::vector<const double*> bptr((size_t)n);
  for (int32_t i = 0; i < n; ++i) bptr[i] = bpp.data() + off[i];
  rc = add_examples_threaded(ds, n, n_rows, rows, bptr.data(), labels, th, 1, n_threads, true);
  return rc ? fail(ctx, rc, "example build failed") : SK_OK;
}

int sk_random_sequences(uint64_t* state, int32_t n_seqs, int32_t len, char* out) {
  if (!state || !out || n_seqs < 0 || len < 0) return SK_ERR_INVALID;
  for (int32_t s = 0; s < n_seqs; ++s) sk::random_sequence(*state, len, out + (size_t)s * (len + 1));
  return SK_OK;
}

int sk_last_timing(const sk_context* ctx, double* stem_ms, double* string_ms, double* cells,
                   int32_t* launches) {
  if (!ctx) return SK_ERR_INVALID;
  if (stem_ms) *stem_ms = ctx->last_stem_ms;
  if (string_ms) *string_ms = ctx->last_str_ms;
  if (cells) *cells = ctx->last_cells;
  if (launches) *launches = ctx->last_launches;
  return SK_OK;
}

int sk_set_async(sk_context* ctx, int32_t on) {
  if (!ctx) return SK_ERR_INVALID;
  if (ctx->async && !on) {
    const int rc = sk_sync_timing(ctx);
    if (rc) return rc;
  }
  ctx->async = on != 0;
  return SK_OK;
}

int sk_sync_timing(sk_context* ctx) {
  if (!ctx) return SK_ERR_INVALID;
  if (!ctx->async) return SK_OK;
  for (int k = 0; k < sk_context::kTSets; ++k)
    if (sk::tset_resolve(ctx, k) != hipSuccess) return fail(ctx, SK_ERR_HIP, "sk_sync_timing: event");
  ctx->last_stem_ms = ctx->acc_stem_ms;
  ctx->last_str_ms = ctx->acc_str_ms;
  ctx->last_cells = ctx->acc_cells;
  ctx->last_launches = ctx->acc_launches;
  ctx->last_launch_ms_sum = ctx->acc_launch_ms;
  ctx->last_launch_n = ctx->acc_launch_n;
  ctx->acc_stem_ms = ctx->acc_str_ms = ctx->acc_cells = ctx->acc_launch_ms = 0.0;
  ctx->acc_launch_n = ctx->acc_launches = 0;
  return SK_OK;
}

int sk_last_launch_ms(const sk_context* ctx, double* ms_sum, int32_t* n_launches) {
  if (!ctx) return SK_ERR_INVALID;
  if (ms_sum) *ms_sum = ctx->last_launch_ms_sum;
  if (n_launches) *n_launches = ctx->last_launch_n;
  return SK_OK;
}

int sk_stem4d_col_shape(int32_t min_len, int32_t max_len, int32_t* nb, int32_t* waves, int32_t* pf) {
  if (max_len < 0 || min_len > max_len) return SK_ERR_INVALID;
  const int cpl = sk::stem4d_cpl(max_len);
  const bool runs = max_len + 1 <= 64 * cpl && max_len <= sk::stem4d_col_max_n() &&
                    (min_len <= 1 || sk::stem4d_col_w_max(min_len) >= 1);
  if (nb) *nb = sk::stem4d_col_nb(cpl);
  if (waves) *waves = runs ? col_waves(cpl, min_len >= 2 ? min_len : INT32_MAX, max_len, max_len) : 0;
  if (pf) *pf = sk::stem4d_col_pf();
  return SK_OK;
}

int sk_last_classes(const sk_context* ctx, uint32_t* stem_maxk_mask, uint32_t* stem4d_mask) {
  if (!ctx) return SK_ERR_INVALID;
  if (stem_maxk_mask) *stem_maxk_mask = ctx->last_stem_classes;
  if (stem4d_mask) *stem4d_mask = ctx->last_s4d_classes;
  return SK_OK;
}

void sk_ribosum_tables(float* s16, float* p256) {
  if (s16) std::memcpy(s16, SK_RIBOSUM_S, sizeof(SK_RIBOSUM_S));
  if (p256) std::memcpy(p256, SK_RIBOSUM_P, sizeof(SK_RIBOSUM_P));
}

int sk_char2rna(int c) { return sk::char2rna(c); }

int sk_experiments(void) {
#ifdef SK_EXPERIMENTS
  return 1;
#else
  return 0;
#endif
}

}
```

stem_kernel_amd/kernel_matrix.py:

```python
from __future__ import annotations

import ctypes as C
import sys
from typing import Iterable, List, Optional, Sequence

import numpy as np

from . import _lib
from ._lib import SK_OK, KernelParams, StemKernelError, check, lib

__all__ = [
    "fold", "random_sequences", "Dataset", "Context", "KernelMatrix",
    "SuStemKernel", "SiStemKernel", "StringKernel", "SuStemStrKernel", "StemStrKernel",
    "SiStemStrKernel", "LSuStemKernel", "LSuStemStrKernel", "NaiveStringKernel",
    "StemKernelError", "SVMModel",
]


_FORMATS = {"fa": _lib.FMT_FASTA, "fasta": _lib.FMT_FASTA, "aln": _lib.FMT_CLUSTAL,
            "clustal": _lib.FMT_CLUSTAL, "maf": _lib.FMT_MAF}


def _seqfile_rows(h) -> List[List[str]]:
    L = lib()
# ... 279 lines not shown
            ctx._chk(lib().sk_dataset_add_sampled(ctx.handle, ds._h, n, nr, rarr, larr, C.c_float(th),
                                                  flags, n_samples, seed, threads))
        elif consensus:
            ctx._chk(lib().sk_dataset_add_alifolded(ctx.handle, ds._h, n, nr, rarr, larr, C.c_float(th),
                                                    flags, threads))
        else:
            ctx._chk(lib().sk_dataset_add_folded(ctx.handle, ds._h, n, nr, rarr, larr, C.c_float(th),
                                                 flags, threads))
        return ds

    def __len__(self):
        return lib().sk_dataset_size(self._h)

    def export(self, first: int = 0, count: Optional[int] = None) -> bytearray:
        count = len(self) - first if count is None else count
        need = C.c_size_t()
        check(lib().sk_dataset_export(self._h, first, count, None, 0, C.byref(need)))
        out = bytearray(need.value)
        buf = (C.c_char * max(need.value, 1)).from_buffer(out) if need.value else None
        check(lib().sk_dataset_export(self._h, first, count, buf, need.value, C.byref(need)))
        return out

    def import_bytes(self, data) -> "Dataset":
        n = len(data)
        if isinstance(data, bytearray) and n:
            data = (C.c_char * n).from_buffer(data)
        check(lib().sk_dataset_import(self._h, data, n))
        return self

    def pack_digest(self):
        hy, hx = C.c_uint64(), C.c_uint64()
        check(lib().sk_dataset_pack_digest(self._h, C.byref(hy), C.byref(hx)))
        return hy.value, hx.value

    def profile(self, i: int):
        L = self.shape(i)[4]
        out = np.zeros((max(L, 1), 5), np.float32)
        ns = C.c_float()
        check(lib().sk_dataset_profile(self._h, i, out.ctypes.data_as(C.POINTER(C.c_float)),
                                       C.byref(ns)))
        return out[:L], ns.value

    def bpla_weights(self, i: int):
        L = self.shape(i)[4]
        a = [np.zeros(max(L, 1), np.float32) for _ in range(3)]
        check(lib().sk_dataset_bpla_weights(self._h, i, *(v.ctypes.data_as(C.POINTER(C.c_float))
                                                           for v in a)))
        return [v[:L] for v in a]

    def label(self, i: int) -> str:
        return lib().sk_dataset_label(self._h, i).decode()

    def shape(self, i: int):
        v = [C.c_int32() for _ in range(5)]
        check(lib().sk_dataset_shape(self._h, i, *[C.byref(a) for a in v]))
        return tuple(a.value for a in v)

    def row_traffic(self, i: int) -> dict:
        v = [C.c_int32() for _ in range(7)]
        check(lib().sk_dataset_row_traffic(self._h, i, *[C.byref(a) for a in v]))
        return dict(zip(("rows", "stored", "slab_reads", "gamma_reads", "phi_reads", "reg_reads",
                         "y_slots"), (a.value for a in v)))

    def dag(self, i: int) -> dict:
        nn, ne, nb, nr, L = self.shape(i)
        u = lambda k: np.zeros(max(k, 1), np.uint32)
        f = lambda k: np.zeros(max(k, 1), np.float32)
        d = dict(first=u(nn), last=u(nn), n_edges=u(nn), n_bpfreq=u(nn), weight=f(nn),
                 max_pa=u(nn), edge_to=u(ne), edge_gaps=u(ne), bp_code=u(nb), bp_p=f(nb),
                 roots=u(nr), pos_weight=f(L))
        ptr = lambda a: a.ctypes.data_as(C.POINTER(C.c_uint32 if a.dtype == np.uint32 else C.c_float))
        check(lib().sk_dataset_dag(self._h, i, *[ptr(d[k]) for k in
                                                 ("first", "last", "n_edges", "n_bpfreq", "weight",
                                                  "max_pa", "edge_to", "edge_gaps", "bp_code",
                                                  "bp_p", "roots", "pos_weight")]))
        sizes = dict(first=nn, last=nn, n_edges=nn, n_bpfreq=nn, weight=nn, max_pa=nn,
                     edge_to=ne, edge_gaps=ne, bp_code=nb, bp_p=nb, roots=nr, pos_weight=L)
        return {k: v[: sizes[k]] for k, v in d.items()}


class Context:

    def __init__(self, device: int = 0, stream: Optional[int] = None):
        self._h = C.c_void_p()
        check(lib().sk_open(device, C.c_void_p(stream) if stream else None, C.byref(self._h)))
        self.device = device

    def close(self):
        if self._h is not None and self._h.value:
            lib().sk_close(self._h)
            self._h = None

    def __del__(self):
        try:
            self.close()
        except Exception:
            pass

    @property
    def handle(self):
        return self._h

    def _chk(self, rc):
        return check(rc, self._h)

    def fold(self, seqs: Sequence[str], no_gu: bool = False, no_closing_gu: bool = False,
             log_z: bool = False, no_lonely_pairs: bool = False):
        seqs = list(seqs)
        n = len(seqs)
        sizes = [len(s) * (len(s) - 1) // 2 for s in seqs]
        out = np.zeros(max(sum(sizes), 1))
        lz = np.zeros(max(n, 1))
        sarr = (C.c_char_p * max(n, 1))(*[s.encode() for s in seqs])
        flags = (1 if no_gu else 0) | (2 if no_closing_gu else 0) | (4 if no_lonely_pairs else 0)
        self._chk(lib().sk_fold_mccaskill(self._h, n, sarr, flags,
                                          out.ctypes.data_as(C.POINTER(C.c_double)),
                                          lz.ctypes.data_as(C.POINTER(C.c_double))))
        res, o = [], 0
        for z in sizes:
            res.append(out[o:o + z].copy())
            o += z
        return (res, lz[:n]) if log_z else res

    def fold_alignment(self, alns: Sequence[Sequence[str]], no_gu: bool = False,
                       no_lonely_pairs: bool = False, with_log_z: bool = False):
        alns = [[a] if isinstance(a, str) else list(a) for a in alns]
        n = len(alns)
        sizes = [len(a[0]) * (len(a[0]) - 1) // 2 if a else 0 for a in alns]
        out = np.zeros(max(sum(sizes), 1))
        lz = np.zeros(max(n, 1))
        flat = [r.encode() for a in alns for r in a]
        rarr = (C.c_char_p * max(len(flat), 1))(*flat)
        nrow = np.array([len(a) for a in alns] or [0], dtype=np.int32)
        flags = (1 if no_gu else 0) | (4 if no_lonely_pairs else 0)
        self._chk(lib().sk_fold_alignment(self._h, n, nrow.ctypes.data_as(C.POINTER(C.c_int32)), rarr, flags,
                                          out.ctypes.data_as(C.POINTER(C.c_double)),
                                          lz.ctypes.data_as(C.POINTER(C.c_double))))
        res, o = [], 0
        for z in sizes:
            res.append(out[o:o + z].copy())
            o += z
        return (res, lz[:n]) if with_log_z else res

    def fold_sample(self, seqs: Sequence[str], n_samples: int, seed: int = 0, no_gu: bool = False,
                    no_closing_gu: bool = False, no_lonely_pairs: bool = False,
                    structures: bool = False, log_z: bool = False):
        seqs = list(seqs)
        n = len(seqs)
        sizes = [len(s) * (len(s) - 1) // 2 for s in seqs]
        out = np.zeros(max(sum(sizes), 1))
        lz = np.zeros(max(n, 1))
        sarr = (C.c_char_p * max(n, 1))(*[s.encode() for s in seqs])
        flags = (1 if no_gu else 0) | (2 if no_closing_gu else 0) | (4 if no_lonely_pairs else 0)
        sbuf = None
        if structures:
            sbuf = np.zeros(max(sum(len(s) for s in seqs) * max(n_samples, 0), 1), np.uint8)
        self._chk(lib().sk_fold_sample(self._h, n, sarr, flags, n_samples, seed,
                                       out.ctypes.data_as(C.POINTER(C.c_double)),
                                       sbuf.ctypes.data if structures else None,
                                       lz.ctypes.data_as(C.POINTER(C.c_double))))
        res, o = [], 0
        for z in sizes:
            res.append(out[o:o + z].copy())
            o += z
        ret = [res]
        if structures:
            raw, strs, o = sbuf.tobytes(), [], 0
            for s in seqs:
                m = len(s)
                strs.append([raw[o + k * m:o + (k + 1) * m].decode("ascii") for k in range(n_samples)])
                o += m * n_samples
            ret.append(strs)
        if log_z:
            ret.append(lz[:n])
        return ret[0] if len(ret) == 1 else tuple(ret)

    def upload(self, ds: Dataset):
        self._chk(lib().sk_dataset_upload(self._h, ds.handle))

    def gram(self, ds: Dataset, kernel: _Kernel, normalize: bool = False) -> np.ndarray:
        self.upload(ds)
        n = len(ds)
        out = np.zeros((n, n), dtype=np.float64)
        self._chk(lib().sk_gram(self._h, ds.handle, C.byref(kernel.params), int(normalize),
                                out.ctypes.data_as(C.POINTER(C.c_double))))
        return out

    def pairs(self, ds: Dataset, kernel: _Kernel, x, y) -> np.ndarray:
        self.upload(ds)
        x = np.ascontiguousarray(x, dtype=np.int32)
        y = np.ascontiguousarray(y, dtype=np.int32)
        out = np.zeros(x.size, dtype=np.float64)
        self._chk(lib().sk_pairs(self._h, ds.handle, C.byref(kernel.params),
                                 x.ctypes.data_as(C.POINTER(C.c_int32)),
                                 y.ctypes.data_as(C.POINTER(C.c_int32)), x.size,
                                 out.ctypes.data_as(C.POINTER(C.c_double))))
        return out

    def bpla_gradients(self, ds: Dataset, kernel: "BPLAKernel", x, y, ys: Optional[Dataset] = None):
        ys = ds if ys is None else ys
        self.upload(ds)
        self.upload(ys)
        x = np.ascontiguousarray(x, dtype=np.int32)
        y = np.ascontiguousarray(y, dtype=np.int32)
        val = np.zeros(x.size, dtype=np.float64)
        grad = np.zeros((x.size, 4), dtype=np.float64)
        self._chk(lib().sk_bpla_gradients(self._h, ds.handle, ys.handle, C.byref(kernel.params),
                                          x.ctypes.data_as(C.POINTER(C.c_int32)),
                                          y.ctypes.data_as(C.POINTER(C.c_int32)), x.size,
                                          val.ctypes.data_as(C.POINTER(C.c_double)),
                                          grad.ctypes.data_as(C.POINTER(C.c_double))))
        return val, grad

    def bpla_gradient_gram(self, ds: Dataset, kernel: "BPLAKernel", normalize: bool = False):
        from .shard import assemble_gradients
        n = len(ds)
        iu, ju = np.triu_indices(n)
        val, grad = self.bpla_gradients(ds, kernel, iu, ju)
        return assemble_gradients(iu, ju, val, grad, n, normalize)

    def comm_init(self, uid: bytes, rank: int, world: int) -> None:
        self._chk(lib().sk_comm_init(self._h, uid, len(uid), rank, world))

    def allgather(self, send_ptr: int, count: int, recv_ptr: int) -> None:
        self._chk(lib().sk_comm_allgather(self._h, send_ptr, count, recv_ptr))

    def gram_sharded(self, ds: Dataset, kernel: _Kernel, normalize: bool = False) -> np.ndarray:
        self.upload(ds)
        n = len(ds)
        out = np.zeros((n, n), dtype=np.float64)
        self._chk(lib().sk_gram_sharded(self._h, ds.handle, C.byref(kernel.params),
                                        int(normalize), out.ctypes.data_as(C.POINTER(C.c_double))))
        return out

    def pairs_device(self, ds: Dataset, kernel: _Kernel, x, y, out_ptr: int) -> None:
        self.upload(ds)
        x = np.ascontiguousarray(x, dtype=np.int32)
        y = np.ascontiguousarray(y, dtype=np.int32)
        self._chk(lib().sk_pairs_device(self._h, ds.handle, C.byref(kernel.params),
                                        x.ctypes.data_as(C.POINTER(C.c_int32)),
                                        y.ctypes.data_as(C.POINTER(C.c_int32)), x.size,
                                        C.c_void_p(out_ptr)))

    def test_row(self, test: Dataset, t: int, train: Dataset, kernel: _Kernel,
                 sv_index=None, self_value: bool = False):
        self.upload(test)
        self.upload(train)
        out = np.zeros(len(train), dtype=np.float64)
        sv = None if sv_index is None else np.ascontiguousarray(sv_index, dtype=np.int32)
        sf = C.c_double(0.0)
        self._chk(lib().sk_test_row(self._h, test.handle, t, train.handle,
                                    None if sv is None else sv.ctypes.data_as(C.POINTER(C.c_int32)),
                                    0 if sv is None else sv.size, C.byref(kernel.params),
                                    out.ctypes.data_as(C.POINTER(C.c_double)),
                                    C.byref(sf) if self_value else None))
        return (out, sf.value) if self_value else out

    def diagonal(self, ds: Dataset, kernel: _Kernel, sv_index=None) -> np.ndarray:
        self.upload(ds)
        out = np.zeros(len(ds), dtype=np.float64)
        sv = None if sv_index is None else np.ascontiguousarray(sv_index, dtype=np.int32)
        self._chk(lib().sk_diagonal(self._h, ds.handle,
                                    None if sv is None else sv.ctypes.data_as(C.POINTER(C.c_int32)),
                                    0 if sv is None else sv.size, C.byref(kernel.params),
                                    out.ctypes.data_as(C.POINTER(C.c_double))))
        return out

    def test_matrix(self, test: Dataset, train: Dataset, kernel: _Kernel, norm_test=False,
                    normalize=False):
        self.upload(test)
        self.upload(train)
        out = np.zeros((len(test), len(train)), dtype=np.float64)
        self_ = np.zeros(len(test), dtype=np.float64)
        self._chk(lib().sk_test_matrix(self._h, test.handle, train.handle, C.byref(kernel.params),
                                       int(norm_test), int(normalize),
                                       out.ctypes.data_as(C.POINTER(C.c_double)),
                                       self_.ctypes.data_as(C.POINTER(C.c_double))))
        return out, self_

    def last_timing(self):
        a, b, c, d = C.c_double(), C.c_double(), C.c_double(), C.c_int32()
        self._chk(lib().sk_last_timing(self._h, C.byref(a), C.byref(b), C.byref(c), C.byref(d)))
        return dict(stem_ms=a.value, string_ms=b.value, cells=c.value, launches=d.value)

    def set_async(self, on: bool = True) -> None:
        self._chk(lib().sk_set_async(self._h, 1 if on else 0))

    def sync_timing(self) -> None:
        self._chk(lib().sk_sync_timing(self._h))

    def last_launch_ms(self):
        a, b = C.c_double(), C.c_int32()
        self._chk(lib().sk_last_launch_ms(self._h, C.byref(a), C.byref(b)))
        return dict(ms_sum=a.value, launches=b.value)

    def last_classes(self):
        a, b = C.c_uint32(), C.c_uint32()
        self._chk(lib().sk_last_classes(self._h, C.byref(a), C.byref(b)))
        maxk = sorted((4 * k if k <= 8 else k) for k in range(32) if a.value >> k & 1)
        s4d = sorted({(1 << (k & 3), bool(k & 4)) for k in range(12) if b.value >> k & 1})
        col = sorted(1 << (k & 3) for k in range(8, 12) if b.value >> k & 1)
        return dict(stem_maxk=maxk, stem4d=s4d, stem4d_col=col)


def stem4d_col_shape(min_len: int, max_len: int) -> dict:
    v = [C.c_int32() for _ in range(3)]
    check(lib().sk_stem4d_col_shape(int(min_len), int(max_len), *[C.byref(a) for a in v]))
    return dict(nb=v[0].value, waves=v[1].value, pf=v[2].value)


def format_libsvm(matrix: np.ndarray, labels: Sequence[str]) -> str:
    m = np.ascontiguousarray(matrix, dtype=np.float64)
    rows, cols = m.shape
    larr = (C.c_char_p * rows)(*[l.encode() for l in labels])
    need = C.c_size_t()
    check(lib().sk_format_libsvm(m.ctypes.data_as(C.POINTER(C.c_double)), rows, cols, larr, None,
                                 0, C.byref(need)))
    buf = C.create_string_buffer(need.value)
    check(lib().sk_format_libsvm(m.ctypes.data_as(C.POINTER(C.c_double)), rows, cols, larr, buf,
                                 need.value, C.byref(need)))
    return buf.value.decode()


class SVMModel:

    def __init__(self, path: str):
        h = C.c_void_p()
        rc = lib().sk_svm_model_load(str(path).encode(), C.byref(h))
        if rc != SK_OK:
            raise StemKernelError(rc, lib().sk_svm_last_error().decode())
        self._h = h
        t, k, p = C.c_int32(), C.c_int32(), C.c_int32()
        check(lib().sk_svm_model_info(self._h, C.byref(t), C.byref(k), None, C.byref(p)))
        self.svm_type, self.nr_class, self.has_probability = t.value, k.value, bool(p.value)
        labels = (C.c_int32 * max(k.value, 1))()
        check(lib().sk_svm_model_info(self._h, None, None, labels, None))
        self.labels = [labels[i] for i in range(k.value)]

    def __del__(self):
        h = getattr(self, "_h", None)
        if h:
            lib().sk_svm_model_free(h)
            self._h = None

    def predict(self, row, cnt: int = 1, probability: bool = True):
        r = np.ascontiguousarray(row, dtype=np.float64)
        nv = max(self.nr_class * (self.nr_class - 1) // 2, self.nr_class, 1)
        vals = np.zeros(nv, dtype=np.float64)
        label = C.c_double()
        rc = lib().sk_svm_predict(self._h, int(cnt), r.ctypes.data_as(C.POINTER(C.c_double)), r.size,
                                  int(probability), C.byref(label), vals.ctypes.data_as(C.POINTER(C.c_double)))
        if rc != SK_OK:
            raise StemKernelError(rc, lib().sk_svm_last_error().decode())
        if probability and self.svm_type in (0, 1):
            return label.value, vals[: self.nr_class]
        return label.value, vals[: max(self.nr_class * (self.nr_class - 1) // 2, 1)]


class KernelMatrix:

    def __init__(self, ctx: Optional[Context] = None):
        self.ctx = ctx if ctx is not None else Context(0)
        self.matrix = np.zeros((0, 0))
        self.self_ = np.zeros(0)
        self.label: List[str] = []

    def calculate(self, train: Dataset, kernel: _Kernel, normalize: bool = False, n_th: int = 1):
        self.matrix = self.ctx.gram(train, kernel, normalize)
        self.label = [train.label(i) for i in range(len(train))]
        return 0.0

    def calculate_test(self, test: Dataset, train: Dataset, kernel: _Kernel, norm_test=False,
                       normalize=False, n_th: int = 1):
        self.matrix, self.self_ = self.ctx.test_matrix(test, train, kernel, norm_test, normalize)
        self.label = [test.label(i) for i in range(len(test))]
        return 0.0

    @staticmethod
    def calculate_row(ctx: Context, data: Dataset, t: int, train: Dataset, kernel: _Kernel,
                      sv_index=None, want_self=False):
        return ctx.test_row(data, t, train, kernel, sv_index, want_self)

    @staticmethod
    def diagonal(ctx: Context, train: Dataset, kernel: _Kernel, sv_index=None):
        return ctx.diagonal(train, kernel, sv_index)

    def __call__(self, i, j=None):
        return self.self_[i] if j is None else self.matrix[i, j]

    def print(self, out=sys.stdout):
        out.write(format_libsvm(self.matrix, self.label))

    def save(self, path: str) -> None:
        text = format_libsvm(self.matrix, self.label).encode()
        if path.endswith(".gz"):
            import gzip
            with gzip.open(path, "wb") as f:
                f.write(text)
        elif path.endswith(".bz2"):
            import bz2
            with bz2.open(path, "wb") as f:
                f.write(text)
        else:
            try:
                with open(path, "wb") as f:
                    f.write(text)
            except OSError as e:
                raise StemKernelError(-1, f"{path}: cannot open for writing") from e
```

Before: 219,500.

## Precompute per-y gamma tables once in a separate kernel and share across work items

Adds a pre-pass kernel that builds, for every gapless y example in a stem class, its gamma rows and kappa values into a shared global table indexed by slot. Stem work items then copy kappa from that table instead of recomputing the gamma sweep per item, which removes redundant work when one y is split across several items or blocks. In exchange it needs extra scratch memory, sized against a budget with a fallback to per-block recomputation. It also adds an extra launch and a stream dependency before the main stem kernels.

Measured after the change: 226,100, median of 6. 3.0% higher.

```diff
diff --git a/include/stem_kernel.h b/include/stem_kernel.h
--- a/include/stem_kernel.h
+++ b/include/stem_kernel.h
@@ -198,6 +198,7 @@
 int sk_set_async(sk_context *ctx, int32_t on);
 int sk_sync_timing(sk_context *ctx);
 int sk_last_classes(const sk_context *ctx, uint32_t *stem_maxk_mask, uint32_t *stem4d_mask);
+int32_t sk_last_gamma_shared(const sk_context *ctx);
 int sk_stem4d_col_shape(int32_t min_len, int32_t max_len, int32_t *nb, int32_t *waves, int32_t *pf);
 void sk_ribosum_tables(float *s16, float *p256);
 int sk_char2rna(int c);
diff --git a/stem_kernel_amd/_lib.py b/stem_kernel_amd/_lib.py
--- a/stem_kernel_amd/_lib.py
+++ b/stem_kernel_amd/_lib.py
@@ -104,6 +104,7 @@
     "sk_comm_allgather": (C.c_int, [_P, C.c_void_p, C.c_int64, C.c_void_p]),
     "sk_gram_sharded": (C.c_int, [_P, _P, C.POINTER(KernelParams), C.c_int, _F64P]),
     "sk_last_classes": (C.c_int, [_P, C.POINTER(C.c_uint32), C.POINTER(C.c_uint32)]),
+    "sk_last_gamma_shared": (C.c_int32, [_P]),
     "sk_stem4d_col_shape": (C.c_int, [C.c_int32, C.c_int32, _I32P, _I32P, _I32P]),
     "sk_ribosum_tables": (None, [_F32P, _F32P]),
     "sk_char2rna": (C.c_int, [C.c_int]),
diff --git a/stem_kernel_amd/csrc/kernels/dag_stem.hip b/stem_kernel_amd/csrc/kernels/dag_stem.hip
--- a/stem_kernel_amd/csrc/kernels/dag_stem.hip
+++ b/stem_kernel_amd/csrc/kernels/dag_stem.hip
@@ -763,52 +763,55 @@
   static constexpr int value = MAXK <= 12 ? 12 : MAXK <= 17 ? (SK_M16 ? 12 : SK_W16) : MAXK <= 20 ? SK_W20 : 8;
 };
 
+struct StemLds {
+  lds_f64* co;
+  lds_f64* gp;
+  lds_f64* Rall;
+  lds_f64* hball;
+  lds_f64* yew;
+  lds_u32* ysc;
+  lds_u32* yed2;
+  lds_i32* ylf;
+  lds_i32* ycs;
+  lds_i32* ctl;
+  lds_f64* kap;
+};
+
 template <int MAXK>
-__global__ void __launch_bounds__(64 * StemWaves<MAXK>::value) sk_dag_stem_kernel(StemLaunch P) {
+__device__ __forceinline__ StemLds stem_lds_carve(const StemLaunch& P, int nwaves) {
   extern __shared__ __attribute__((aligned(16))) unsigned char smem[];
-  const DevSet& s = P.yset;
-  const int lane = threadIdx.x & 63, wave = threadIdx.x >> 6;
-  const int nwaves = blockDim.x >> 6;
   const int maxnl = P.lds_max_nl;
   constexpr int PW = pass_width<MAXK>();
-
-  lds_f64* co = (lds_f64*)(smem);
-  lds_f64* gp = co + 256;
-  lds_f64* Rall = gp + P.n_gpow_pad;
-  lds_f64* hball = Rall + (size_t)nwaves * maxnl;
   constexpr bool NW = node_weights<MAXK>();
-  lds_f64* yew = hball + (size_t)nwaves * 64 * PW;
-  lds_u32* ysc = (lds_u32*)(yew + (node_weights_f32<MAXK>() ? (size_t)maxnl / 2
-                                   : NW ? (size_t)maxnl : (size_t)P.lds_max_nch * 64));
-  lds_u32* yed2 = ysc + (size_t)P.lds_max_nch * 64;
-  lds_i32* ylf = (lds_i32*)(yed2 + (edges_global<MAXK>() ? 0 : P.lds_max_edges));
-  lds_i32* ycs = ylf + P.lds_max_len_pad;
-  lds_i32* ctl = ycs + P.lds_max_len_pad;
-  lds_f64* kap = (lds_f64*)(ctl + 4);
-
-  for (int k = threadIdx.x; k < 256; k += blockDim.x) co[k] = P.co_subst[k];
-  for (int k = threadIdx.x; k < P.n_gpow; k += blockDim.x) gp[k] = P.gpow[k];
-
-  lds_f64* R = Rall + (size_t)wave * maxnl;
-  lds_f64* hb = hball + (size_t)wave * 64 * PW;
-  for (int j = 0; j < PW; ++j) hb[64 * j + lane] = 0.0;
-  double* slab = P.scratch + (size_t)(blockIdx.x * nwaves + wave) * P.slab_doubles;
-  double* gamtab = P.gam_on ? P.gam + (size_t)blockIdx.x * P.gam_doubles : nullptr;
-  double* phitab = P.phi_on ? P.phi + (size_t)blockIdx.x * P.phi_doubles : nullptr;
-  double* phikap = P.phi_on ? phitab + (size_t)P.xset.n_phi * (64 * MAXK) : nullptr;
+  StemLds L;
+  L.co = (lds_f64*)(smem);
+  L.gp = L.co + 256;
+  L.Rall = L.gp + P.n_gpow_pad;
+  L.hball = L.Rall + (size_t)nwaves * maxnl;
+  L.yew = L.hball + (size_t)nwaves * 64 * PW;
+  L.ysc = (lds_u32*)(L.yew + (node_weights_f32<MAXK>() ? (size_t)maxnl / 2
+                              : NW ? (size_t)maxnl : (size_t)P.lds_max_nch * 64));
+  L.yed2 = L.ysc + (size_t)P.lds_max_nch * 64;
+  L.ylf = (lds_i32*)(L.yed2 + (edges_global<MAXK>() ? 0 : P.lds_max_edges));
+  L.ycs = L.ylf + P.lds_max_len_pad;
+  L.ctl = L.ycs + P.lds_max_len_pad;
+  L.kap = (lds_f64*)(L.ctl + 4);
+  return L;
+}
+
+template <int MAXK>
+__device__ __forceinline__ void stage_y(const StemLaunch& P, const StemLds& L, int y, YView& Y) {
+  const DevSet& s = P.yset;
+  constexpr bool NW = node_weights<MAXK>();
+  const int maxnl = P.lds_max_nl;
   const double gap2 = P.gap2;
-  const int band = (int)P.band;
-
-  const int wave_u = __builtin_amdgcn_readfirstlane(wave);
-  for (;;) {
-    __syncthreads();
-    if (threadIdx.x == 0) ctl[0] = atomicAdd(P.item_counter, 1);
-    __syncthreads();
-    const int it = __builtin_amdgcn_readfirstlane(ctl[0]);
-    if (it >= P.n_items) break;
-    const int4 item = P.items[it];
-    const int y = item.x;
-    YView Y;
+  lds_f64* gp = L.gp;
+  lds_f64* yew = L.yew;
+  lds_u32* ysc = L.ysc;
+  lds_u32* yed2 = L.yed2;
+  lds_i32* ylf = L.ylf;
+  lds_i32* ycs = L.ycs;
+  {
     Y.nl = s.ex_nl[y];
     Y.nch = s.ex_nch[y];
     Y.nseqs = s.ex_nseqs[y];
@@ -850,47 +853,124 @@
       ylf[v] = lo;
     }
     __syncthreads();
+  }
+}
+
+template <int MAXK, typename KapPtr>
+__device__ __forceinline__ void gamma_rows(const StemLaunch& P, const YView& Y, lds_f64* R, const lds_f64* co,
+                                           const lds_f64* gp, double* gamtab, KapPtr kap, int wave_u,
+                                           int nwaves, int lane) {
+  const DevSet& s = P.yset;
+  const DevSet& xset = P.xset;
+  const int band = (int)P.band;
+  const int nb = Y.nb, bb = Y.bb;
+  for (int g = wave_u; g < xset.n_gam; g += nwaves) {
+    const uint32_t key = xset.gam_key[g];
+    const int gcode = (int)(key >> 16) * 16, glen = (int)(key & 0xffff);
+    double kp = 0.0;
+    for (int k = 0; k < MAXK; ++k) {
+      const int q = lane + 64 * k;
+      double M = 0.0;
+      if (q < Y.nl) {
+        const uint4 nd = Y.nrg[q];
+        const int ylen = (int)(s.yn_b[nb + q] & 0xffff);
+        if (((nd.x >> 16) & 0xff) == 0 && (band == 0 || abs(glen - ylen) <= band)) {
+          double vs;
+          if ((nd.y >> 24) != 0u) {
+            vs = co[gcode + ((nd.y >> 16) & 0xf)] * (double)__uint_as_float(nd.w);
+          } else {
+            vs = 0.0;
+            const int yb0 = (int)(s.yn_b[nb + q] >> 16), ynb = (int)(nd.x >> 24);
+            for (int b = 0; b < ynb; ++b)
+              vs += co[gcode + s.bpf_code[bb + yb0 + b]] * (double)s.bpf_p[bb + yb0 + b];
+          }
+          M = vs * gp[nd.y & 0xffff];
+          kp += M * s.yn_P[nb + q];
+        }
+      }
+      R[q] = M;
+    }
+    for (int off = 32; off > 0; off >>= 1) kp += __shfl_xor(kp, off, 64);
+    if (lane == 0) kap[g] = kp;
+    wave_sync();
+    int c0 = 0;
+    if (band > 0) c0 = Y.ycs[min(max(glen - band, 0), Y.lmax + 1)];
+    c0 = __builtin_amdgcn_readfirstlane(c0);
+    if (c0 < Y.nch) iy_sweep<node_weights<MAXK>(), node_weights_f32<MAXK>()>(Y, R, c0, lane);
+    double* grow = gamtab + (size_t)g * (64 * MAXK);
+    for (int k = 0; k < MAXK; ++k)
+      if (lane + 64 * k < Y.nl) grow[lane + 64 * k] = R[lane + 64 * k];
+    wave_sync();
+  }
+}
+
+template <int MAXK>
+__global__ void __launch_bounds__(64 * StemWaves<MAXK>::value) sk_gamma_table_kernel(StemLaunch P) {
+  const int lane = threadIdx.x & 63, wave = threadIdx.x >> 6;
+  const int nwaves = blockDim.x >> 6;
+  const int slot = blockIdx.x;
+  if (slot >= P.n_slots) return;
+  const StemLds L = stem_lds_carve<MAXK>(P, nwaves);
+  for (int k = threadIdx.x; k < 256; k += blockDim.x) L.co[k] = P.co_subst[k];
+  for (int k = threadIdx.x; k < P.n_gpow; k += blockDim.x) L.gp[k] = P.gpow[k];
+  lds_f64* R = L.Rall + (size_t)wave * P.lds_max_nl;
+  const int wave_u = __builtin_amdgcn_readfirstlane(wave);
+  __syncthreads();
+  YView Y;
+  stage_y<MAXK>(P, L, P.slot_y[slot], Y);
+  gamma_rows<MAXK>(P, Y, R, L.co, L.gp, P.gam + (size_t)slot * P.gam_doubles,
+                   P.kap_y + (size_t)slot * P.xset.n_gam, wave_u, nwaves, lane);
+}
+
+template <int MAXK>
+__global__ void __launch_bounds__(64 * StemWaves<MAXK>::value) sk_dag_stem_kernel(StemLaunch P) {
+  const DevSet& s = P.yset;
+  const int lane = threadIdx.x & 63, wave = threadIdx.x >> 6;
+  const int nwaves = blockDim.x >> 6;
+  const int maxnl = P.lds_max_nl;
+  constexpr int PW = pass_width<MAXK>();
+
+  const StemLds L = stem_lds_carve<MAXK>(P, nwaves);
+  lds_f64* co = L.co;
+  lds_f64* gp = L.gp;
+  lds_i32* ctl = L.ctl;
+  lds_f64* kap = L.kap;
+
+  for (int k = threadIdx.x; k < 256; k += blockDim.x) co[k] = P.co_subst[k];
+  for (int k = threadIdx.x; k < P.n_gpow; k += blockDim.x) gp[k] = P.gpow[k];
+
+  lds_f64* R = L.Rall + (size_t)wave * maxnl;
+  lds_f64* hb = L.hball + (size_t)wave * 64 * PW;
+  for (int j = 0; j < PW; ++j) hb[64 * j + lane] = 0.0;
+  double* slab = P.scratch + (size_t)(blockIdx.x * nwaves + wave) * P.slab_doubles;
+  double* phitab = P.phi_on ? P.phi + (size_t)blockIdx.x * P.phi_doubles : nullptr;
+  double* phikap = P.phi_on ? phitab + (size_t)P.xset.n_phi * (64 * MAXK) : nullptr;
+  const int band = (int)P.band;
+
+  const int wave_u = __builtin_amdgcn_readfirstlane(wave);
+  for (;;) {
+    __syncthreads();
+    if (threadIdx.x == 0) ctl[0] = atomicAdd(P.item_counter, 1);
+    __syncthreads();
+    const int it = __builtin_amdgcn_readfirstlane(ctl[0]);
+    if (it >= P.n_items) break;
+    const int4 item = P.items[it];
+    const int y = item.x;
+    YView Y;
+    stage_y<MAXK>(P, L, y, Y);
+    const int nb = Y.nb, bb = Y.bb;
 
     const bool gam = P.gam_on && s.ex_gapless[y];
+    double* gamtab = nullptr;
     if (gam) {
       const DevSet& xset = P.xset;
-      for (int g = wave_u; g < xset.n_gam; g += nwaves) {
-        const uint32_t key = xset.gam_key[g];
-        const int gcode = (int)(key >> 16) * 16, glen = (int)(key & 0xffff);
-        double kp = 0.0;
-        for (int k = 0; k < MAXK; ++k) {
-          const int q = lane + 64 * k;
-          double M = 0.0;
-          if (q < Y.nl) {
-            const uint4 nd = Y.nrg[q];
-            const int ylen = (int)(s.yn_b[nb + q] & 0xffff);
-            if (((nd.x >> 16) & 0xff) == 0 && (band == 0 || abs(glen - ylen) <= band)) {
-              double vs;
-              if ((nd.y >> 24) != 0u) {
-                vs = co[gcode + ((nd.y >> 16) & 0xf)] * (double)__uint_as_float(nd.w);
-              } else {
-                vs = 0.0;
-                const int yb0 = (int)(s.yn_b[nb + q] >> 16), ynb = (int)(nd.x >> 24);
-                for (int b = 0; b < ynb; ++b)
-                  vs += co[gcode + s.bpf_code[bb + yb0 + b]] * (double)s.bpf_p[bb + yb0 + b];
-              }
-              M = vs * gp[nd.y & 0xffff];
-              kp += M * s.yn_P[nb + q];
-            }
-          }
-          R[q] = M;
-        }
-        for (int off = 32; off > 0; off >>= 1) kp += __shfl_xor(kp, off, 64);
-        if (lane == 0) kap[g] = kp;
-        wave_sync();
-        int c0 = 0;
-        if (band > 0) c0 = Y.ycs[min(max(glen - band, 0), Y.lmax + 1)];
-        c0 = __builtin_amdgcn_readfirstlane(c0);
-        if (c0 < Y.nch) iy_sweep<node_weights<MAXK>(), node_weights_f32<MAXK>()>(Y, R, c0, lane);
-        double* grow = gamtab + (size_t)g * (64 * MAXK);
-        for (int k = 0; k < MAXK; ++k)
-          if (lane + 64 * k < Y.nl) grow[lane + 64 * k] = R[lane + 64 * k];
-        wave_sync();
+      if (P.gam_shared) {
+        gamtab = P.gam + (size_t)item.w * P.gam_doubles;
+        const double* __restrict__ ky = P.kap_y + (size_t)item.w * xset.n_gam;
+        for (int g = threadIdx.x; g < xset.n_gam; g += blockDim.x) kap[g] = ky[g];
+      } else {
+        gamtab = P.gam + (size_t)blockIdx.x * P.gam_doubles;
+        gamma_rows<MAXK>(P, Y, R, co, gp, gamtab, kap, wave_u, nwaves, lane);
       }
       __syncthreads();
 
@@ -1047,6 +1127,26 @@
   return hipGetLastError();
 }
 
+hipError_t launch_gamma_tables(const StemLaunch& P, int nwaves, hipStream_t st) {
+  if (!P.gam_shared || P.n_slots <= 0) return hipSuccess;
+  const size_t lds = stem_lds_bytes(P, nwaves);
+  const int maxk = stem_maxk(P.lds_max_nl);
+  switch (maxk) {
+#define SK_CASE(K)                                                                                  \
+  case K: {                                                                                        \
+    hipError_t e = hipFuncSetAttribute(reinterpret_cast<const void*>(sk_gamma_table_kernel<K>),    \
+                                       hipFuncAttributeMaxDynamicSharedMemorySize, (int)lds);      \
+    if (e != hipSuccess) return e;                                                                 \
+    hipLaunchKernelGGL(sk_gamma_table_kernel<K>, dim3(P.n_slots), dim3(64 * nwaves), lds, st, P); \
+    break;                                                                                         \
+  }
+    SK_STEM_CLASSES(SK_CASE)
+#undef SK_CASE
+    default: return hipErrorInvalidValue;
+  }
+  return hipGetLastError();
+}
+
 hipError_t stem_kernel_attr(int max_nl, int* max_dyn_lds, int* vgprs, int* max_waves) {
   hipFuncAttributes attr;
   const int maxk = stem_maxk(max_nl);
diff --git a/stem_kernel_amd/csrc/kernels/launch.h b/stem_kernel_amd/csrc/kernels/launch.h
--- a/stem_kernel_amd/csrc/kernels/launch.h
+++ b/stem_kernel_amd/csrc/kernels/launch.h
@@ -31,6 +31,10 @@
   double* gam = nullptr;
   int64_t gam_doubles = 0;
   int32_t gam_on = 0;
+  int32_t gam_shared = 0;
+  double* kap_y = nullptr;
+  const int32_t* slot_y = nullptr;
+  int32_t n_slots = 0;
   double* phi = nullptr;
   int64_t phi_doubles = 0;
   const int32_t* item_phi_off = nullptr;
@@ -320,6 +324,7 @@
                        hipStream_t st);
 size_t stem_lds_bytes(const StemLaunch& P, int nwaves);
 hipError_t launch_stem(const StemLaunch& P, int grid, int nwaves, hipStream_t st);
+hipError_t launch_gamma_tables(const StemLaunch& P, int nwaves, hipStream_t st);
 hipError_t stem_kernel_attr(int max_nl, int* max_dyn_lds, int* vgprs, int* max_waves);
 int stem_maxk(int max_nl);
 
diff --git a/stem_kernel_amd/csrc/sk_api.cpp b/stem_kernel_amd/csrc/sk_api.cpp
--- a/stem_kernel_amd/csrc/sk_api.cpp
+++ b/stem_kernel_amd/csrc/sk_api.cpp
@@ -260,6 +260,7 @@
   double last_stem_ms = 0.0, last_str_ms = 0.0, last_cells = 0.0;
   int32_t last_launches = 0;
   uint32_t last_stem_classes = 0, last_s4d_classes = 0;
+  int32_t last_gamma_shared = 0;
   void* comm = nullptr;
 };
 
@@ -2089,6 +2090,7 @@
   ctx->last_launches = 0;
   sk::lev_reset(ctx);
   ctx->last_stem_classes = ctx->last_s4d_classes = 0;
+  ctx->last_gamma_shared = 0;
   if (n == 0) return SK_OK;
   const int nx = (int)xs_->ex.size(), ny = (int)ys_->ex.size();
   for (int64_t k = 0; k < n; ++k)
@@ -2123,9 +2125,13 @@
     int max_nl = 0, max_edges = 0, max_bpf = 0, max_nch = 0;
     int nwaves = 1, grid = 1;
     size_t item_off = 0, n_items = 0;
+    size_t slot_off = 0, n_slots = 0;
+    bool gam_shared = false;
+    size_t tab_off = 0;
   };
   std::vector<StemClass> classes;
   std::vector<int4> items;
+  std::vector<int32_t> slot_y;
   std::vector<int32_t> ixs;
   std::vector<int64_t> ioidx;
   std::vector<int32_t> big_x, big_y;
@@ -2193,6 +2199,7 @@
     for (int maxk : {32, 28, 24, 20, 17, 16, 12, 8, 4}) {
       StemClass C;
       C.maxk = maxk;
+      C.slot_off = slot_y.size();
       bool any = false;
       for (int j = 0; j < ny; ++j) {
         if (cnt[j + 1] == cnt[j] || !in_class(j, maxk)) continue;
@@ -2257,6 +2264,11 @@
       C.item_off = items.size();
       for (int j : ysel) {
         const double yw = (double)PY.ex_nl[j];
+        int slot = -1;
+        if (L.gam_on && PY.ex_gapless[j]) {
+          slot = (int)(slot_y.size() - C.slot_off);
+          slot_y.push_back(j);
+        }
         int64_t b = cnt[j];
         while (b < cnt[j + 1]) {
           const double target = remaining * share;
@@ -2267,11 +2279,12 @@
             for (int64_t t = e; t < re; ++t) cost += (double)PX.ex_nl[x[byy[t]]] * yw;
             e = re;
           }
-          items.push_back(make_int4(j, (int)b, (int)(e - b), 0));
+          items.push_back(make_int4(j, (int)b, (int)(e - b), slot));
           remaining -= cost;
           b = e;
         }
       }
+      C.n_slots = slot_y.size() - C.slot_off;
       C.n_items = items.size() - C.item_off;
       C.grid = (int)std::min<int64_t>(C.grid, std::max<int64_t>(1, (int64_t)C.n_items));
       classes.push_back(C);
@@ -2356,6 +2369,7 @@
   need += 256 * 8 + 16 * 8 + (size_t)(max_len + 4) * 8 * 2;
   need += 1024;
   need += items.size() * sizeof(int4) + nb * (4 + 8) + nb * 8 * 2 + nb * 4 * 2 + 64 + 8 * 256;
+  need += slot_y.size() * 4 + 256;
   need += big_x.size() * (4 + 4 + 8) + 3 * 256;
   need += 16 * 256;
   rc = ensure_work(ctx, need);
@@ -2373,6 +2387,7 @@
   int32_t* d_px = A.take<int32_t>(nb);
   int32_t* d_py = A.take<int32_t>(nb);
   int* d_ctr = A.take<int>(64);
+  int32_t* d_sloty = A.take<int32_t>(std::max<size_t>(slot_y.size(), 1));
   int32_t* d_bx = A.take<int32_t>(std::max<size_t>(big_x.size(), 1));
   int32_t* d_by = A.take<int32_t>(std::max<size_t>(big_x.size(), 1));
   int64_t* d_bo = A.take<int64_t>(std::max<size_t>(big_x.size(), 1));
@@ -2417,6 +2432,7 @@
     SK_HIP(ctx, sk::h2d(ctx, d_items, items.data(), items.size() * sizeof(int4), S));
     SK_HIP(ctx, sk::h2d(ctx, d_ixs, ixs.data(), nb * 4, S));
     SK_HIP(ctx, sk::h2d(ctx, d_oidx, ioidx.data(), nb * 8, S));
+    SK_HIP(ctx, sk::h2d(ctx, d_sloty, slot_y.data(), slot_y.size() * 4, S));
     if (phi_on) {
       SK_HIP(ctx, sk::h2d(ctx, d_iphi_off, item_phi_off.data(), item_phi_off.size() * 4, S));
       if (!item_phi.empty())
@@ -2450,14 +2466,33 @@
     }
     const bool two_streams = classes.size() > 1 && !SK_KNOB("SK_SERIAL_CLASSES");
     size_t scratch_need = 0, scratch_x = 0;
-    for (size_t c = 0; c < classes.size(); ++c) {
-      const StemClass& C = classes[c];
-      const int64_t slab = (int64_t)(PX.max_slots + 1) * 64 * C.maxk;
-      const int64_t gtab = (int64_t)PX.gam_key.size() * 64 * C.maxk;
-      const int64_t ptab = phi_on ? (int64_t)PX.phi_al.size() * (64 * C.maxk + 1) : 0;
-      const size_t b = (size_t)C.grid * (C.nwaves * slab + gtab + ptab) * sizeof(double);
-      size_t& r = (two_streams && (c & 1)) ? scratch_x : scratch_need;
-      r = std::max(r, b);
+    size_t tab_total = 0;
+    auto size_classes = [&](size_t gam_budget) {
+      scratch_need = scratch_x = tab_total = 0;
+      for (size_t c = 0; c < classes.size(); ++c) {
+        StemClass& C = classes[c];
+        const int64_t slab = (int64_t)(PX.max_slots + 1) * 64 * C.maxk;
+        const int64_t gtab1 = (int64_t)PX.gam_key.size() * 64 * C.maxk;
+        const size_t shared_b = C.n_slots * (size_t)(gtab1 + (int64_t)PX.gam_key.size()) * sizeof(double);
+        C.gam_shared = C.n_slots > 0 && tab_total + shared_b <= gam_budget;
+        if (C.gam_shared) {
+          C.tab_off = tab_total / sizeof(double);
+          tab_total += shared_b;
+        }
+        const int64_t ptab = phi_on ? (int64_t)PX.phi_al.size() * (64 * C.maxk + 1) : 0;
+        const size_t b = (size_t)C.grid * (C.nwaves * slab + ptab + (C.gam_shared ? 0 : gtab1)) * sizeof(double);
+        size_t& r = (two_streams && (c & 1)) ? scratch_x : scratch_need;
+        r = std::max(r, b);
+      }
+    };
+    const bool any_slots = !PX.gam_key.empty() && !slot_y.empty();
+    size_classes(any_slots ? SIZE_MAX : 0);
+    if (const char* e = SK_KNOB("SK_GAM_TABLE_MB")) {
+      size_classes((size_t)std::max(0.0, std::atof(e) * 1048576.0));
+    } else if (tab_total > 0 && scratch_need + scratch_x + tab_total + 512 > ctx->scratch_bytes) {
+      size_t free_b = 0, total_b = 0;
+      SK_HIP(ctx, hipMemGetInfo(&free_b, &total_b));
+      size_classes(std::min<size_t>((free_b + ctx->scratch_bytes) / 4, (size_t)8 << 30));
     }
     const int64_t big_stride = ((int64_t)std::max(big_max_nl, 1) + 63) / 64 * 64;
     const int64_t big_wave = (int64_t)(PX.max_slots + 2) * big_stride;
@@ -2473,10 +2508,21 @@
       scratch_need = std::max(scratch_need,
                               (size_t)big_grid * sk::kStemBigWaves * (size_t)big_wave * sizeof(double));
     }
-    scratch_need = (scratch_need + 255) / 256 * 256;
-    rc = ensure_scratch(ctx, std::max<size_t>(scratch_need + scratch_x, 64));
+    const size_t big_need = scratch_need;
+    auto get_scratch = [&]() {
+      scratch_need = (std::max(scratch_need, big_need) + 255) / 256 * 256;
+      scratch_x = (scratch_x + 255) / 256 * 256;
+      return ensure_scratch(ctx, std::max<size_t>(scratch_need + scratch_x + tab_total, 64));
+    };
+    rc = get_scratch();
+    if (rc && tab_total > 0) {
+      (void)hipGetLastError();
+      size_classes(0);
+      rc = get_scratch();
+    }
     if (rc) return rc;
     double* scratch_cls = ctx->scratch + scratch_need / sizeof(double);
+    double* scratch_tab = scratch_cls + scratch_x / sizeof(double);
 #ifdef SK_STAMPS
     unsigned long long* d_stamps = nullptr;
     SK_HIP(ctx, hipMalloc(&d_stamps, 16 * sizeof(unsigned long long)));
@@ -2486,14 +2532,11 @@
       std::fprintf(stderr, "[host] pairs=%lld plan %.2f ms, phi keys %.2f ms, uploads+prep %.2f ms\n",
                    (long long)n, th1 - th0, th2 - th1, now_ms() - th2);
     SK_HIP(ctx, hipEventRecord(ctx->ev0, S));
-    if (two_streams) {
-      SK_HIP(ctx, hipEventRecord(ctx->evk, S));
-      SK_HIP(ctx, hipStreamWaitEvent(ctx->cls, ctx->evk, 0));
-    }
+    std::vector<sk::StemLaunch> launches(classes.size());
     for (size_t c = 0; c < classes.size(); ++c) {
       const StemClass& C = classes[c];
       const bool on_cls = two_streams && (c & 1);
-      sk::StemLaunch SL;
+      sk::StemLaunch& SL = launches[c];
       SL.xset = xs_->dev;
       SL.yset = ys_->dev;
       SL.pn = pn;
@@ -2518,18 +2561,37 @@
       SL.scratch = on_cls ? scratch_cls : ctx->scratch;
       SL.gam_on = !PX.gam_key.empty();
       SL.gam_doubles = (int64_t)PX.gam_key.size() * SL.lds_max_nl;
-      SL.gam = SL.scratch + (size_t)C.grid * C.nwaves * SL.slab_doubles;
+      double* wg_tab = SL.scratch + (size_t)C.grid * C.nwaves * SL.slab_doubles;
+      SL.gam_shared = C.gam_shared ? 1 : 0;
+      SL.n_slots = C.gam_shared ? (int32_t)C.n_slots : 0;
+      SL.slot_y = d_sloty + C.slot_off;
+      SL.gam = C.gam_shared ? scratch_tab + C.tab_off : wg_tab;
+      SL.kap_y = SL.gam + C.n_slots * (size_t)SL.gam_doubles;
       SL.phi_on = phi_on ? 1 : 0;
       SL.phi_doubles = phi_on ? (int64_t)PX.phi_al.size() * (SL.lds_max_nl + 1) : 0;
-      SL.phi = SL.gam + (size_t)C.grid * SL.gam_doubles;
+      SL.phi = wg_tab + (C.gam_shared ? 0 : (size_t)C.grid * SL.gam_doubles);
       SL.item_phi_off = d_iphi_off + C.item_off;
       SL.item_phi = d_iphi;
 #ifdef SK_STAMPS
       SL.stamps = d_stamps;
 #endif
+    }
+    bool any_tables = false;
+    for (size_t c = 0; c < classes.size(); ++c) {
+      SK_HIP(ctx, sk::launch_gamma_tables(launches[c], classes[c].nwaves, S));
+      any_tables = any_tables || classes[c].gam_shared;
+    }
+    if (two_streams || (side && any_tables)) SK_HIP(ctx, hipEventRecord(ctx->evk, S));
+    if (two_streams) SK_HIP(ctx, hipStreamWaitEvent(ctx->cls, ctx->evk, 0));
+    if (side && any_tables) SK_HIP(ctx, hipStreamWaitEvent(ctx->side, ctx->evk, 0));
+    for (size_t c = 0; c < classes.size(); ++c) {
+      const StemClass& C = classes[c];
+      const bool on_cls = two_streams && (c & 1);
+      const sk::StemLaunch& SL = launches[c];
       SK_HIP(ctx, sk::lev_mark(ctx, on_cls ? ctx->cls : S));
       SK_HIP(ctx, sk::launch_stem(SL, C.grid, C.nwaves, on_cls ? ctx->cls : S));
       SK_HIP(ctx, sk::lev_mark(ctx, on_cls ? ctx->cls : S));
+      if (C.gam_shared) ++ctx->last_gamma_shared;
       ctx->last_stem_classes |= 1u << (C.maxk % 4 ? C.maxk : C.maxk / 4);
     }
     if (two_streams) {
@@ -4111,6 +4173,8 @@
   return SK_OK;
 }
 
+int32_t sk_last_gamma_shared(const sk_context* ctx) { return ctx ? ctx->last_gamma_shared : 0; }
+
 void sk_ribosum_tables(float* s16, float* p256) {
   if (s16) std::memcpy(s16, SK_RIBOSUM_S, sizeof(SK_RIBOSUM_S));
   if (p256) std::memcpy(p256, SK_RIBOSUM_P, sizeof(SK_RIBOSUM_P));
diff --git a/stem_kernel_amd/kernel_matrix.py b/stem_kernel_amd/kernel_matrix.py
--- a/stem_kernel_amd/kernel_matrix.py
+++ b/stem_kernel_amd/kernel_matrix.py
@@ -605,6 +605,9 @@
         col = sorted(1 << (k & 3) for k in range(8, 12) if b.value >> k & 1)
         return dict(stem_maxk=maxk, stem4d=s4d, stem4d_col=col)
 
+    def last_gamma_shared(self) -> int:
+        return int(lib().sk_last_gamma_shared(self._h))
+
 
 def stem4d_col_shape(min_len: int, max_len: int) -> dict:
     v = [C.c_int32() for _ in range(3)]
```
